# szlhl1040/Vehicles-Dispatch-Simulator

Hardware: AMD Instinct MI355X
Metric: env-steps x replicas / sec (192-cluster, 10k vehicles) (higher is better)
Workload: dtype int32

## Files before the change

include/vds_debug.h:

```cpp
#ifndef VDS_DEBUG_H
#define VDS_DEBUG_H

#include "vds.h"

#ifdef __cplusplus
extern "C" {
#endif

int vds_debug_dense(vds_handle *h, int32_t lanes_per_replica, int32_t tab, int32_t keys, int32_t force_slow);

int vds_debug_ablate(vds_handle *h, int32_t flags);

int vds_debug_read_prof(vds_handle *h, uint64_t *out32);

int vds_debug_read_span(vds_handle *h, uint64_t *out1024, int32_t reset);

int vds_debug_read_err(vds_handle *h, int32_t *out16);

int vds_debug_check_guards(vds_handle *h);

int vds_debug_poke_guard(vds_handle *h);

int vds_debug_graph_pool_size(void);

int vds_debug_tick_forms(vds_handle *h, uint8_t *out, int32_t cap, int32_t *n_out);

int vds_selftest_dpp(vds_handle *h, const int32_t *in, int32_t *out_wave, int32_t *out_rowmin, int32_t *out_rowsum,
                     int32_t *out_rowscan, int32_t nwaves);

#ifdef __cplusplus
}
#endif
#endif
```

vehicles_dispatch_simulator_amd/_lib.py:

```python
from __future__ import annotations

import ctypes as C
import os
import sys
import subprocess

_HERE = os.path.dirname(os.path.abspath(__file__))
def _lib_path():
    name = os.environ.get("VDS_LIB", "libvds.so")
    if os.path.isabs(name):
        return name
    for d in (_HERE, os.path.join(os.path.dirname(_HERE), "build")):
        if os.path.exists(os.path.join(d, name)):
            return os.path.join(d, name)
    return os.path.join(_HERE, name)


LIB_PATH = _lib_path()
CSRC = os.path.join(_HERE, "csrc")

NUM_COUNTERS = 8
COUNTER_NAMES = ("order_num", "reject_num", "matched", "wait_sum", "dispatch_num", "dispatch_cost", "sum_order_value", "evals")


class VdsConfig(C.Structure):
    _fields_ = [
        ("struct_size", C.c_int32), ("device", C.c_int32), ("replicas", C.c_int32), ("vehicles", C.c_int32),
        ("tick_minutes", C.c_int32), ("neighbor_can_server", C.c_int32), ("pickup_reject_threshold", C.c_int64),
        ("idle_cap", C.c_int32), ("ring_cap", C.c_int32), ("ring_ticks", C.c_int32), ("far_cap", C.c_int32),
        ("force_generic", C.c_int32),
    ]


_VP, _I32, _I64 = C.c_void_p, C.c_int32, C.c_int64
SYMBOLS = {
    "vds_version": (_I32, []),
    "vds_build_id": (C.c_char_p, []),
    "vds_config_init": (None, [C.POINTER(VdsConfig)]),
    "vds_create": (C.c_int, [C.POINTER(VdsConfig), C.POINTER(_VP)]),
    "vds_destroy": (C.c_int, [_VP]),
    "vds_last_error": (C.c_char_p, [_VP]),
    "vds_set_stream": (C.c_int, [_VP, _VP]),
    "vds_load_static": (C.c_int, [_VP, _VP, _I32, _VP, _I32, _VP, _VP, _I32]),
    "vds_load_orders": (C.c_int, [_VP, _VP, _VP, _VP, _I32]),
    "vds_load_order_days": (C.c_int, [_VP, _I32, _VP, _VP, _VP, _VP, _VP]),
    "vds_load_orders_strided": (C.c_int, [_VP, _VP, _VP, _VP, _I32, _I64]),
    "vds_replica_ticks": (C.c_int, [_VP, _I32, C.POINTER(_I32), C.POINTER(_I32)]),
    "vds_set_idle_cap": (C.c_int, [_VP, _I32]),
    "vds_idle_cap": (C.c_int, [_VP]),
    "vds_num_ticks": (C.c_int, [_VP, C.POINTER(_I32)]),
    "vds_reset": (C.c_int, [_VP, _VP]),
    "vds_reset_again": (C.c_int, [_VP]),
    "vds_reset_random": (C.c_int, [_VP, _VP]),
    "vds_step": (C.c_int, [_VP]),
    "vds_apply_dispatch": (C.c_int, [_VP, _I32, _VP, _VP, _VP, _VP]),
    "vds_apply_dispatch_ex": (C.c_int, [_VP, _I32, _VP, _VP, _VP, _VP, _VP, _VP]),
    "vds_apply_dispatch_device": (C.c_int, [_VP, _I32, _VP]),
    "vds_advance": (C.c_int, [_VP]),
    "vds_run": (C.c_int, [_VP, _I32]),
    "vds_set_run_groups": (C.c_int, [_VP, _I32, _I32]),
    "vds_get_run_groups": (C.c_int, [_VP]),
    "vds_sync": (C.c_int, [_VP]),
    "vds_clock": (C.c_int, [_VP, C.POINTER(_I32), C.POINTER(_I32)]),
    "vds_read_obs": (C.c_int, [_VP, _VP, _VP, _VP, _VP, _VP]),
    "vds_obs_device": (C.c_int, [_VP, C.POINTER(_VP)]),
    "vds_obs_device_planes": (C.c_int, [_VP, _I32, C.POINTER(_VP)]),
    "vds_obs_inplace": (C.c_int, [_VP, _I32, C.POINTER(_VP), C.POINTER(C.c_int64), C.POINTER(C.c_int64)]),
    "vds_run_hooked_invalidate": (C.c_int, [_VP]),
    "vds_supply_inplace": (C.c_int, [_VP, C.POINTER(_VP), C.POINTER(C.c_int64), C.POINTER(C.c_int64), C.POINTER(C.c_int64), C.POINTER(_VP), C.POINTER(_I32)]),
    "vds_counters_device": (C.c_int, [_VP, C.POINTER(_VP)]),
    "vds_outcomes_device": (C.c_int, [_VP, C.POINTER(_VP)]),
    "vds_read_outcomes": (C.c_int, [_VP, _VP, _VP, _VP, _VP]),
    "vds_read_counters": (C.c_int, [_VP, _VP]),
    "vds_reduce_counters": (C.c_int, [_VP, _VP, C.POINTER(_VP)]),
    "vds_reduce_counters_into": (C.c_int, [_VP, _VP]),
    "vds_profile_enable": (C.c_int, [_VP, _I32]),
    "vds_run_hooked": (C.c_int, [_VP, _I32, _I32, _I32, _VP, _VP]),
    "vds_set_replica_days": (C.c_int, [_VP, _VP]),
    "vds_profile_read": (C.c_int, [_VP, _VP, _I32, C.POINTER(_I32)]),
    "vds_read_orders": (C.c_int, [_VP, _I32, _I32, _VP, _VP, _VP]),
    "vds_read_lists": (C.c_int, [_VP, _I32] + [_VP] * 8),
    "vds_read_vehicles": (C.c_int, [_VP, _I32] + [_VP] * 5),
    "vds_read_work": (C.c_int, [_VP, _VP]),
    "vds_py_random_nodes": (C.c_int, [C.c_uint64, _I32, _I32, _VP, _VP]),
    "vds_cluster_cost_sums": (C.c_int, [_I32, _VP, _I32, _VP, _I32, _VP, _VP]),
    "vds_cluster_cost_sums_error": (C.c_char_p, []),
    "vds_main_kernel": (C.c_char_p, [_VP]),
    "vds_dfs_sequences": (C.c_int, [_VP, _VP, _I32, _I32, _VP, _VP, C.c_int64]),
}
TEST_SYMBOLS = {"vds_debug_read_span": (C.c_int, [_VP, _VP, _I32]), "vds_debug_read_err": (C.c_int, [_VP, _VP]), "vds_debug_graph_pool_size": (C.c_int, []), "vds_debug_tick_forms": (C.c_int, [_VP, _VP, _I32, _VP]), "vds_debug_check_guards": (C.c_int, [_VP]), "vds_debug_poke_guard": (C.c_int, [_VP]), "vds_debug_dense": (C.c_int, [_VP, _I32, _I32, _I32, _I32]), "vds_debug_ablate": (C.c_int, [_VP, _I32]), "vds_debug_read_prof": (C.c_int, [_VP, _VP]), "vds_selftest_dpp": (C.c_int, [_VP, _VP, _VP, _VP, _VP, _VP, _I32])}

_lib = None


def build(force: bool = False) -> str:
    srcs = [os.path.join(CSRC, f) for f in os.listdir(CSRC) if f.endswith((".hip", ".h"))]
    srcs.append(os.path.join(os.path.dirname(_HERE), "include", "vds.h"))
    srcs.append(os.path.join(os.path.dirname(_HERE), "include", "vds_debug.h"))
    stale = (not os.path.exists(LIB_PATH)) or any(os.path.getmtime(s) > os.path.getmtime(LIB_PATH) for s in srcs)
    if force or stale:
        subprocess.check_call(["make", "-s", "-C", CSRC])
    return LIB_PATH


def load():
    global _lib
    if _lib is None:
        if not os.path.exists(LIB_PATH):
            try:
                build(force=True)
            except Exception as e:
                raise RuntimeError("libvds.so is not built (%s) and building it failed (%s): run "
                                   "`make -C vehicles_dispatch_simulator_amd/csrc`; there is no CPU fallback" % (LIB_PATH, e))
        if "torch" not in sys.modules and not os.environ.get("VDS_NO_TORCH_PRELOAD"):
            try:
                import torch
            except ImportError:
                pass
        lib = C.CDLL(LIB_PATH)
        for name, (res, args) in {**SYMBOLS, **TEST_SYMBOLS}.items():
            if os.environ.get("VDS_LIB") and not hasattr(lib, name):
                print("vehicles_dispatch_simulator_amd: %s (VDS_LIB) does not export %s" % (LIB_PATH, name), file=sys.stderr)
                continue
            fn = getattr(lib, name)
            fn.restype = res
            fn.argtypes = args
        _lib = lib
    return _lib
```

vehicles_dispatch_simulator_amd/csrc/vds_api.hip:

```cpp
#include "../../include/vds.h"
#include "../../include/vds_debug.h"
#include "vds_device.h"

#include <algorithm>
#include <unordered_map>
#include <atomic>
#include <chrono>
#include <thread>
#include <cstdarg>
#include <cstdio>
#include <cstdlib>
#include <cstring>
#include <exception>
#include <map>
#include <mutex>
#include <new>
#include <string>
#include <vector>
#include <execinfo.h>
#include <signal.h>
#include <unistd.h>

namespace vds {
void launch_reset(const Static &, const State &, const int *, hipStream_t);
bool reset_uses_image(const Static &);
void launch_reset_capture(const Static &, const State &, unsigned *, int *, hipStream_t);
void launch_reset_image(const Static &, const State &, const unsigned *, const int *, hipStream_t);
void launch_py_random_nodes(const unsigned long long *, int, int, int, int, const int *, int *, int *, hipStream_t);
void launch_start_nodes_check(const int *, int, int, int, int, const int *, int *, unsigned long long *, hipStream_t);
void launch_tick_main(const Static &, const State &, int, int, hipStream_t);
void launch_tick_work(const Static &, const State &, int, hipStream_t);
void launch_update_only(const Static &, const State &, int, hipStream_t);
void launch_match_dfs(const Static &, const State &, int, hipStream_t);
void launch_tick_replica2(const Static &, const State &, int, hipStream_t);
void launch_tick_hybrid(const Static &, const State &, int, int, hipStream_t);
void emit_tick_rows(const Emit &, const Static &, const State &, int, int, int, int);
void emit_hybrid_rows(const Emit &, const Static &, const State &, int, int, int, int);
void emit_hybrid_walk(const Emit &, const Static &, const State &, int, int, int);
void launch_build_vis(const Static &, const int *, unsigned *, unsigned char *, long long, hipStream_t);
size_t dfs_walk_lds(const Static &);
int dfs_walk_pool(const Static &);
void launch_dispatch(const Static &, const State &, int, int, const int *, const int *, const int *, const int *,
                     const int *, const int *, const int *, const int *, hipStream_t);
void launch_dispatch_dense(const Static &, const State &, int, int, const int *, int, hipStream_t);
void launch_pack_obs(const Static &, const State &, int, int, int, int *, hipStream_t);
void launch_reduce_counters(const Static &, const State &, long long *, long long *, hipStream_t);
void launch_selftest_dpp(const int *, int *, int *, int *, int *, int, hipStream_t);
void set_ablate_tick(int, hipStream_t);
void read_prof_tick(unsigned long long *, hipStream_t);
void set_ablate_dfs(int, hipStream_t);
void read_prof_dfs(unsigned long long *, hipStream_t);
void set_ablate_dense(int, hipStream_t);
void read_prof_dense(unsigned long long *, hipStream_t);
void read_span_dense(unsigned long long *, int, hipStream_t);
void emit_tick_dense(const Emit &, const Static &, const State &, int, int, int);
void emit_dense_flush(const Emit &, const Static &, const State &, int, int);
void emit_pack_obs(const Emit &, const Static &, const State &, int, int, int, int *, int, int);
void emit_dispatch_dense(const Emit &, const Static &, const State &, int, int, const int *, int, int, int);
void emit_slot_outcomes(const Emit &, const Static &, const State &, int, int, long long *, int, int);
void launch_slot_outcomes(const Static &, const State &, int, int, long long *, hipStream_t);
}

using namespace vds;

static thread_local std::string g_create_error;

struct DayHost {
    int O = 0;
    int T = 0, now0 = 0, q_base = 0, Oq = 0;
    std::vector<int> so_id;
    std::vector<int> q_value;
    std::vector<int> q_of;
    std::vector<int> o_tick;
    std::vector<long long> value_upto;
    long long value_all = 0;
};

template <typename T>
struct NoInitAlloc {
    using value_type = T;
    NoInitAlloc() = default;
    template <class U> NoInitAlloc(const NoInitAlloc<U> &) {}
    T *allocate(size_t n) { return static_cast<T *>(::operator new(n * sizeof(T))); }
    void deallocate(T *p, size_t) { ::operator delete(p); }
    template <class U, class... A> void construct(U *p, A &&...a) {
        if constexpr (sizeof...(A) == 0) ::new ((void *)p) U; else ::new ((void *)p) U(std::forward<A>(a)...);
    }
    bool operator==(const NoInitAlloc &) const { return true; }
    bool operator!=(const NoInitAlloc &) const { return false; }
};
template <typename T> using hvec = std::vector<T, NoInitAlloc<T>>;

struct PinnedPool {
    std::mutex mu;
    std::vector<std::pair<void *, size_t>> idle;
    std::unordered_map<void *, std::pair<size_t, bool>> live;
    size_t idle_bytes = 0;
    void *get(size_t bytes) {
        bytes = (bytes + 65535) & ~(size_t)65535;
        std::lock_guard<std::mutex> lk(mu);
        int best = -1;
        for (int i = 0; i < (int)idle.size(); ++i)
            if (idle[i].second >= bytes && idle[i].second <= bytes + bytes / 2 + (1u << 20) && (best < 0 || idle[i].second < idle[best].second)) best = i;
        if (best >= 0) {
            void *p = idle[best].first; const size_t b = idle[best].second;
            idle.erase(idle.begin() + best); idle_bytes -= b;
            live[p] = {b, true};
            return p;
        }
        void *p = nullptr;
        if (hipHostMalloc(&p, bytes, hipHostMallocDefault) == hipSuccess && p) { live[p] = {bytes, true}; return p; }
        (void)hipGetLastError();
        p = ::operator new(bytes);
        live[p] = {bytes, false};
        return p;
    }
    void put(void *p) {
        std::lock_guard<std::mutex> lk(mu);
        auto it = live.find(p);
        if (it == live.end()) return;
        const size_t b = it->second.first; const bool pinned = it->second.second;
        live.erase(it);
        if (!pinned) { ::operator delete(p); return; }
        idle.emplace_back(p, b); idle_bytes += b;
        while (idle_bytes > ((size_t)1 << 30) && !idle.empty()) {
            (void)hipHostFree(idle.front().first); idle_bytes -= idle.front().second; idle.erase(idle.begin());
        }
    }
};
static PinnedPool &pinned_pool() { static PinnedPool *pool = new PinnedPool(); return *pool; }
template <typename T>
struct PinnedAlloc {
    using value_type = T;
    PinnedAlloc() = default;
    template <class U> PinnedAlloc(const PinnedAlloc<U> &) {}
    T *allocate(size_t n) { return static_cast<T *>(pinned_pool().get(n * sizeof(T))); }
    void deallocate(T *p, size_t) { pinned_pool().put(p); }
    template <class U, class... A> void construct(U *p, A &&...a) {
        if constexpr (sizeof...(A) == 0) ::new ((void *)p) U; else ::new ((void *)p) U(std::forward<A>(a)...);
    }
    bool operator==(const PinnedAlloc &) const { return true; }
    bool operator!=(const PinnedAlloc &) const { return false; }
};
template <typename T> using pvec = std::vector<T, PinnedAlloc<T>>;


struct vds_handle {
    vds_config cfg{};
    Static S{};
    State D{};
    hipStream_t own_stream = nullptr, stream = nullptr;
    std::string err;
    bool have_static = false, have_orders = false, have_reset = false;
    bool dfs_mode = false;
    bool dfs2_ok = false;
    bool hybrid_ok = false;
    long long blk_ints = 0;
    bool dense_static_ok = false;
    bool dense_dfs_static_ok = false;
    bool want_sup = false;
    bool nodes_valid = false;
    int alloc_dense = -1, alloc_st = -1;
    int seq_tick0 = 0;
    int seq_tick = -1;
    Static *d_S = nullptr;
    State *d_D = nullptr;
    Static S_up{};
    State D_up{};
    bool have_up = false;
    pvec<int2> pull_drec;
    std::vector<int> pull_slot_q;
    std::vector<int4> pull_desc;
    int pull_Od_max = 0;
    std::vector<int> cl_cmax;
    int dbg_dense_lpr = 0, dbg_dense_tab = 0, dbg_dense_keys = 0, dbg_dense_slow = 0;
    int cost_min = 0, cost_max = 0;
    int max_seq = 0;
    std::vector<unsigned char> lbc_host;
    std::vector<int> dfs_off_host, dfs_seq_host;
    int depth_limit = 0;
    int t = 0;
    int last_stepped = -1;
    int dispatch_seq = 0;
    int O = 0;
    int lds_ints = 0;
    std::vector<int> node2cluster, node_local, cl_off, cl_nodes, cost_host, corder_host;
    std::vector<DayHost> days;
    std::vector<int> replica_day;
    int R_ext = 0;
    std::vector<int> int2ext, ext2int;
    int alloc_R = 0;
    std::vector<void *> dev_allocs;
    std::vector<void *> order_allocs;
    std::unordered_map<void *, size_t> order_bytes;
    std::vector<std::pair<void *, size_t>> order_cache;
    std::vector<void *> map_allocs;
    std::vector<void *> result_allocs;
    std::vector<DayDesc> ddesc_host;
    size_t res_cap_out = 0, res_cap_arr = 0, res_cap_slog = 0;
    int alloc_O = 0;
    int Oqmax = 0;
    std::vector<void *> state_allocs;
    std::vector<void *> idle_allocs;
    int idle_cap_grown = 0;
    std::vector<void *> *alloc_sink = nullptr;
    int *d_veh_node = nullptr;
    unsigned long long *d_seeds = nullptr;
    int *d_fullest = nullptr;
    unsigned *d_reset_img = nullptr; int *d_reset_base = nullptr;
    size_t reset_img_words = 0, reset_base_words = 0;
    unsigned veh_gen = 0, img_veh_gen = 0, img_tables_gen = 0; bool img_valid = false;
    int *d_veh_stage = nullptr;
    unsigned long long *d_bad = nullptr;
    int *d_obs = nullptr;
    long long *d_outc = nullptr;
    long long *d_cnt_per = nullptr, *d_cnt_tot = nullptr;
    int *d_actions = nullptr;
    size_t actions_cap = 0;
    int *d_selftest = nullptr;
    bool profiling = false;
    hipGraphExec_t run_exec = nullptr;
    int run_t0 = -1, run_n = 0, run_G = 1;
    int *pin_slow = nullptr;
    hipEvent_t pin_ev = nullptr;
    long long pin_bucket_ticks = 0;
    int *pin_slow_tick = nullptr; int pin_slow_cap = 0;
    bool pin_ticks_valid = false;
    int slow_tick_cap = 1;
    int tick_mode = 1, tick_lim = -1;
    std::vector<unsigned char> tick_form;
    Static S_alt;
    int dense_adapt = 0;
    unsigned tables_gen = 0;
    bool run_stale = false;
    hipStream_t run_stream = nullptr;
    int use_graph = -1;
    std::vector<hipEvent_t> ev_pool;
    size_t ev_used = 0;
    int run_groups = -1;
    int run_stagger = -1;
    hipGraphExec_t hook_exec = nullptr;
    hipGraphExec_t hook_policy_exec = nullptr;
    void *hook_policy_inst = nullptr;
    int hook_t0 = -1, hook_n = 0, hook_G = 1, hook_planes = 0, hook_K = 0;
    unsigned hook_gen = 0;
    const long long *hook_outc = nullptr;
    const void *hook_actions = nullptr;
    void *hook_policy = nullptr;
    hipStream_t hook_stream = nullptr;
};

static int fail(vds_handle *h, int code, const char *fmt, ...) {
    char buf[512];
    va_list ap;
    va_start(ap, fmt);
    vsnprintf(buf, sizeof(buf), fmt, ap);
    va_end(ap);
    if (h) h->err = buf;
    else g_create_error = buf;
    return code;
}

#define HIPCHK(h, call)                                                                          \
    do {                                                                                         \
        hipError_t e_ = (call);                                                                  \
        if (e_ != hipSuccess) return fail(h, VDS_EHIP, "%s failed: %s", #call, hipGetErrorString(e_)); \
    } while (0)

#ifdef VDS_CANARY
static const size_t GUARD_FRONT = 64u << 10, GUARD_BACK = 256u << 10;
static const bool GUARDED = true;
#else
static const size_t GUARD_FRONT = 0, GUARD_BACK = 0;
static const bool GUARDED = false;
#endif
struct GuardRec { void *base; size_t bytes; };
static std::map<void *, GuardRec> g_guards;
static std::mutex g_guards_mu;

static void dev_free(void *p) {
    if (!p) return;
    if (GUARDED) {
        std::lock_guard<std::mutex> lk(g_guards_mu);
        auto it = g_guards.find(p);
        if (it != g_guards.end()) { (void)hipFree(it->second.base); g_guards.erase(it); return; }
    }
    (void)hipFree(p);
}

template <typename T>
static int dev_alloc(vds_handle *h, T **p, size_t n) {
    *p = nullptr;
    if (n == 0) n = 1;
    const size_t bytes = n * sizeof(T);
    if (!GUARDED && h->alloc_sink == &h->order_allocs) {
        int best = -1;
        for (int i = 0; i < (int)h->order_cache.size(); ++i) {
            const size_t cb = h->order_cache[i].second;
            if (cb >= bytes && cb <= bytes + bytes / 2 + 65536 && (best < 0 || cb < h->order_cache[best].second)) best = i;
        }
        if (best >= 0) {
            *p = reinterpret_cast<T *>(h->order_cache[best].first);
            h->order_bytes[(void *)*p] = h->order_cache[best].second;
            h->order_cache.erase(h->order_cache.begin() + best);
            h->order_allocs.push_back((void *)*p);
            return VDS_OK;
        }
    }
    char *base = nullptr;
    hipError_t e = hipMalloc((void **)&base, bytes + GUARD_FRONT + GUARD_BACK);
    if (e != hipSuccess) return fail(h, VDS_ENOMEM, "hipMalloc(%zu bytes) failed: %s", bytes, hipGetErrorString(e));
    if (GUARDED) {
        (void)hipMemset(base, 0xA5, GUARD_FRONT);
        (void)hipMemset(base + GUARD_FRONT + bytes, 0xA5, GUARD_BACK);
        std::lock_guard<std::mutex> lk(g_guards_mu);
        g_guards[(void *)(base + GUARD_FRONT)] = GuardRec{(void *)base, bytes};
    }
    *p = reinterpret_cast<T *>(base + GUARD_FRONT);
    (h->alloc_sink ? *h->alloc_sink : h->dev_allocs).push_back((void *)*p);
    if (!GUARDED && h->alloc_sink == &h->order_allocs) h->order_bytes[(void *)*p] = bytes;
    return VDS_OK;
}

template <typename T, typename A>
static int upload(vds_handle *h, T **p, const std::vector<T, A> &v) {
    int rc = dev_alloc(h, p, v.size());
    if (rc) return rc;
    if (!v.empty()) HIPCHK(h, hipMemcpy(*p, v.data(), v.size() * sizeof(T), hipMemcpyHostToDevice));
    return VDS_OK;
}

template <typename F>
static int guarded(vds_handle *h, const char *name, F &&body) {
    try {
        return body();
    } catch (const std::bad_alloc &) {
        return fail(h, VDS_ENOMEM, "%s: out of host memory", name);
    } catch (const std::exception &e) {
        return fail(h, VDS_EINVAL, "%s: %s", name, e.what());
    } catch (...) {
        return fail(h, VDS_EINVAL, "%s: unknown C++ exception", name);
    }
}

#define RUN_GROUPS_MAX 16

extern "C" int vds_debug_tick_forms(vds_handle *h, uint8_t *out, int32_t cap, int32_t *n_out) {
    if (!h || !out || !n_out || cap < 0) return VDS_EINVAL;
    const int n = (int)std::min<size_t>(h->tick_form.size(), (size_t)cap);
    for (int i = 0; i < n; ++i) out[i] = h->tick_form[i];
    *n_out = n;
    return VDS_OK;
}
extern "C" int vds_debug_graph_pool_size() {
    return 0;
}

static void drop_hook_graph(vds_handle *h) {
    if (h->hook_exec) {
        (void)hipStreamSynchronize(h->hook_stream);
        (void)hipGraphExecDestroy(h->hook_exec);
        h->hook_exec = nullptr;
    }
    if (h->hook_policy_exec) { (void)hipStreamSynchronize(h->stream); (void)hipGraphExecDestroy(h->hook_policy_exec); h->hook_policy_exec = nullptr; h->hook_policy_inst = nullptr; }
    h->hook_t0 = -1; h->hook_n = 0;
}

static void drop_run_graph(vds_handle *h) {
    drop_hook_graph(h);
    if (h->run_exec) {
        (void)hipStreamSynchronize(h->run_stream);
        (void)hipGraphExecDestroy(h->run_exec);
        h->run_exec = nullptr;
    }
    h->run_t0 = -1; h->run_n = 0; h->run_G = 1; h->run_stale = false;
}

#ifndef DENSE_LPR_DEFAULT
#define DENSE_LPR_DEFAULT 8
#endif

static int dev_copy_sync(vds_handle *h) {
    if (!h->S.dense) return VDS_OK;
    if (!h->d_S) {
        HIPCHK(h, hipMalloc((void **)&h->d_S, sizeof(Static)));
        HIPCHK(h, hipMalloc((void **)&h->d_D, sizeof(State)));
    }
    h->S.self_dev = h->d_S; h->S.state_dev = h->d_D;
    Static want = h->S;
    want.r_lo = 0;
    if (h->have_up && memcmp(&want, &h->S_up, sizeof(Static)) == 0 && memcmp(&h->D, &h->D_up, sizeof(State)) == 0) return VDS_OK;
    HIPCHK(h, hipMemcpyAsync(h->d_S, &want, sizeof(Static), hipMemcpyHostToDevice, h->stream));
    HIPCHK(h, hipMemcpyAsync(h->d_D, &h->D, sizeof(State), hipMemcpyHostToDevice, h->stream));
    memcpy(&h->S_up, &want, sizeof(Static));
    memcpy(&h->D_up, &h->D, sizeof(State));
    h->have_up = true;
    return VDS_OK;
}

static int round_up(int x, int m) { return (x + m - 1) / m * m; }

template <typename F>
static void for_each_day(int n_days, F &&fn) {
    int nt = (int)std::thread::hardware_concurrency();
    if (const char *v = getenv("VDS_LOAD_THREADS")) { if (*v) nt = atoi(v); }
    nt = std::max(1, std::min(std::min(nt, 16), n_days));
    if (nt <= 1) { for (int d = 0; d < n_days; ++d) fn(d); return; }
    std::atomic<int> next{0};
    auto work = [&] { for (int d = next.fetch_add(1); d < n_days; d = next.fetch_add(1)) fn(d); };
    std::vector<std::thread> th;
    th.reserve((size_t)nt);
    try { for (int i = 1; i < nt; ++i) th.emplace_back(work); } catch (...) { }
    work();
    for (auto &t : th) t.join();
}
struct LoadTimer {
    bool on; std::chrono::steady_clock::time_point t0;
    LoadTimer() { const char *v = getenv("VDS_LOAD_TIMING"); on = v && *v == '1'; t0 = std::chrono::steady_clock::now(); }
    void lap(const char *what) {
        if (!on) return;
        const auto t1 = std::chrono::steady_clock::now();
        fprintf(stderr, "vds_load_orders: %-34s %8.2f ms\n", what, std::chrono::duration<double, std::milli>(t1 - t0).count());
        t0 = t1;
    }
};

extern "C" {

int32_t vds_version(void) { return (1 << 16) | 0; }

#ifndef VDS_SRC_HASH
#define VDS_SRC_HASH "unknown"
#endif
const char *vds_build_id(void) {
#ifdef VDS_PROF
    return "src:" VDS_SRC_HASH "+prof";
#elif defined(WKDEBUG)
    return "src:" VDS_SRC_HASH "+dbg";
#elif defined(VDS_CANARY)
    return "src:" VDS_SRC_HASH "+canary";
#else
    return "src:" VDS_SRC_HASH;
#endif
}

namespace {
struct Mt19937 {
    uint32_t mt[624];
    int idx;
    void init_genrand(uint32_t s) {
        mt[0] = s;
        for (int i = 1; i < 624; ++i) mt[i] = 1812433253u * (mt[i - 1] ^ (mt[i - 1] >> 30)) + (uint32_t)i;
        idx = 624;
    }
    void init_by_array(const uint32_t *key, int len) {
        init_genrand(19650218u);
        int i = 1, j = 0;
        for (int k = std::max(624, len); k; --k) {
            mt[i] = (mt[i] ^ ((mt[i - 1] ^ (mt[i - 1] >> 30)) * 1664525u)) + key[j] + (uint32_t)j;
            if (++i >= 624) { mt[0] = mt[623]; i = 1; }
            if (++j >= len) j = 0;
        }
        for (int k = 623; k; --k) {
            mt[i] = (mt[i] ^ ((mt[i - 1] ^ (mt[i - 1] >> 30)) * 1566083941u)) - (uint32_t)i;
            if (++i >= 624) { mt[0] = mt[623]; i = 1; }
        }
        mt[0] = 0x80000000u;
    }
    uint32_t next() {
        if (idx >= 624) {
            for (int k = 0; k < 624; ++k) {
                uint32_t y = (mt[k] & 0x80000000u) | (mt[(k + 1) % 624] & 0x7fffffffu);
                mt[k] = mt[(k + 397) % 624] ^ (y >> 1) ^ ((y & 1u) ? 0x9908b0dfu : 0u);
            }
            idx = 0;
        }
        uint32_t y = mt[idx++];
        y ^= y >> 11; y ^= (y << 7) & 0x9d2c5680u; y ^= (y << 15) & 0xefc60000u; y ^= y >> 18;
        return y;
    }
};
}

int vds_py_random_nodes(uint64_t seed, int32_t N, int32_t count, const uint8_t *valid, int32_t *out) {
    if (N < 1 || count < 0 || (count > 0 && !out)) return VDS_EINVAL;
    if (valid) {
        bool any = false;
        for (int i = 0; i < N && !any; ++i) any = valid[i] != 0;
        if (!any) return VDS_ESTATE;
    }
    Mt19937 g;
    uint32_t key[2] = {(uint32_t)(seed & 0xffffffffu), (uint32_t)(seed >> 32)};
    g.init_by_array(key, key[1] ? 2 : 1);
    int k = 0;
    for (uint32_t n = (uint32_t)N; n; n >>= 1) ++k;
    for (int v = 0; v < count; ++v) {
        for (;;) {
            uint32_t r;
            do { r = g.next() >> (32 - k); } while (r >= (uint32_t)N);
            if (!valid || valid[r]) { out[v] = (int32_t)r; break; }
        }
    }
    return VDS_OK;
}
// ... 182 lines not shown
        std::vector<int> seq;
        for (int c = 0; c < C; ++c) {
            seq.clear();
            if (nbr_off[c + 1] > nbr_off[c]) {
                std::fill(seen.begin(), seen.end(), 0);
                dfs_visit(c, depth_limit, nbr_off, nbr_idx, seen, seq);
            }
            for (size_t i = 1; i < seq.size(); ++i) dfs_seq.push_back(seq[i]);
            dfs_off[c + 1] = (int)dfs_seq.size();
            if (seq.size() > 1) any_seq = true;
        }
    }
    h->dfs_mode = any_seq;
    int rc;
    h->cost_host.assign(cost, cost + (size_t)N * N);
    int *d;
    long long *dl;
    std::vector<int> costp_host;
    {
        std::vector<int> &costp = costp_host;
        costp.assign((size_t)N * N, 0);
        const int ncol = h->cl_off[C];
        for (int i = 0; i < N; ++i) {
            const int *src = cost + (size_t)i * N;
            int *dst = costp.data() + (size_t)i * N;
            for (int j = 0; j < ncol; ++j) dst[j] = src[h->cl_nodes[j]];
        }
        if ((rc = upload(h, &d, costp))) return rc; S.cost = d;
    }
    if ((rc = upload(h, &d, h->node2cluster))) return rc; S.node2cluster = d;
    if ((rc = upload(h, &d, h->node_local))) return rc; S.node_local = d;
    if ((rc = upload(h, &d, h->cl_off))) return rc; S.cl_off = d;
    if ((rc = upload(h, &d, h->cl_nodes))) return rc; S.cl_nodes = d;
    if ((rc = upload(h, &dl, blk_off))) return rc; S.blk_off = dl;
    if ((rc = upload(h, &d, blk))) return rc; S.blk = d;
    {
        std::vector<int> corder(C);
        for (int c = 0; c < C; ++c) corder[c] = c;
        std::stable_sort(corder.begin(), corder.end(), [&](int a, int b) { return cdesc[a].x > cdesc[b].x; });
        if ((rc = upload(h, &d, corder))) return rc; S.corder = d;
        h->corder_host = corder;
        std::vector<int4> cdo(C);
        std::vector<long long> b8off(C + 1, 0);
        for (int c = 0; c < C; ++c) { long long nc = cdesc[c].x; b8off[c + 1] = b8off[c] + (nc * nc + 15) / 16 * 16; }
        bool u8 = b8off[C] < (1ll << 31);
        for (size_t i = 0; i < blk.size() && u8; ++i) u8 = blk[i] >= 0 && blk[i] <= 255;
        S.u8_ok = u8 ? 1 : 0;
        std::vector<unsigned char> blk8(u8 ? (size_t)b8off[C] : 1, 0);
        if (u8)
            for (int c = 0; c < C; ++c) {
                const long long nc = cdesc[c].x;
                for (long long e = 0; e < nc * nc; ++e) blk8[(size_t)b8off[c] + e] = (unsigned char)blk[(size_t)cdesc[c].y + e];
            }
        { unsigned char *d8; if ((rc = upload(h, &d8, blk8))) return rc; S.blk8 = d8; }
        for (int i = 0; i < C; ++i) cdo[i] = make_int4(cdesc[corder[i]].x, cdesc[corder[i]].y, corder[i], u8 ? (int)b8off[corder[i]] : 0);
        for (int c = 0; c < C; ++c) cdesc[c].z = u8 ? (int)b8off[c] : 0;
        { int4 *d4c; if ((rc = upload(h, &d4c, cdesc))) return rc; S.cdesc = d4c; }
        S.cost8 = nullptr;
        if (u8) {
            std::vector<unsigned char> c8((size_t)N * N + 16, 0);
            bool fits = true;
            for (size_t i = 0; i < (size_t)N * N && fits; ++i) { fits = costp_host[i] >= 0 && costp_host[i] <= 255; c8[i] = (unsigned char)costp_host[i]; }
            if (fits) { unsigned char *d8; if ((rc = upload(h, &d8, c8))) return rc; S.cost8 = d8; }
            else S.u8_ok = 0;
            S.lbc = nullptr;
            h->lbc_host.clear();
            if (fits && any_seq && (long long)N * C <= (256ll << 20)) {
                std::vector<unsigned char> lb((size_t)N * C, 255);
                for (int pn = 0; pn < N; ++pn) {
                    const unsigned char *row = c8.data() + (size_t)pn * N;
                    for (int c = 0; c < C; ++c) {
                        unsigned char m = 255;
                        for (int col = h->cl_off[c]; col < h->cl_off[c + 1]; ++col) m = std::min(m, row[col]);
                        lb[(size_t)pn * C + c] = m;
                    }
                }
                unsigned char *dlb; if ((rc = upload(h, &dlb, lb))) return rc; S.lbc = dlb;
                h->lbc_host.swap(lb);
            }
        }
        { int4 *d4o; if ((rc = upload(h, &d4o, cdo))) return rc; S.cdesc_ord = d4o; }
        S.blk8s = nullptr; S.blk32s = nullptr; S.cdesc_dense = nullptr;
        bool d_ok = max_nc <= 255;
        bool d8 = d_ok && S.u8_ok;
        for (size_t i = 0; i < blk.size() && d8; ++i) d8 = blk[i] <= 254;
        if (d_ok) {
            std::vector<long long> doff(C, 0);
            long long tot = 0;
            const long long esz = d8 ? 1 : 4;
            for (int c = 0; c < C; ++c) { const long long nc = cdesc[c].x; doff[c] = tot; tot += (nc * (nc + 1) * esz + 15) / 16 * 16; }
            d_ok = tot < (1ll << 31);
            if (d_ok) {
                std::vector<unsigned char> bs((size_t)std::max<long long>(tot, 16), 0);
                for (int c = 0; c < C; ++c) {
                    const long long nc = cdesc[c].x;
                    for (long long pp = 0; pp < nc; ++pp) {
                        for (long long l = 0; l <= nc; ++l) {
                            const int v = l < nc ? blk[(size_t)cdesc[c].y + pp * nc + l] : (d8 ? 0xFF : DENSE_DEAD_COST);
                            if (d8) bs[(size_t)(doff[c] + pp * (nc + 1) + l)] = (unsigned char)v;
                            else memcpy(bs.data() + (size_t)(doff[c] + (pp * (nc + 1) + l) * 4), &v, 4);
                        }
                    }
                }
                unsigned char *db; if ((rc = upload(h, &db, bs))) return rc;
                if (d8) S.blk8s = db; else S.blk32s = reinterpret_cast<const int *>(db);
                std::vector<int4> cdd(C);
                for (int i = 0; i < C; ++i) cdd[i] = make_int4(cdesc[corder[i]].x, (int)doff[corder[i]], corder[i], dfs_off[corder[i] + 1] > dfs_off[corder[i]] ? 1 : 0);
                int4 *d4d; if ((rc = upload(h, &d4d, cdd))) return rc; S.cdesc_dense = d4d;
            }
        }
        h->dense_static_ok = d_ok;
        h->cl_cmax.assign(C, 0);
        for (int c = 0; c < C; ++c) {
            const long long nc = cdesc[c].x;
            int mx = 0;
            for (long long e = 0; e < nc * nc; ++e) mx = std::max(mx, blk[(size_t)cdesc[c].y + e]);
            h->cl_cmax[c] = mx;
        }
    }
    h->max_seq = 0;
    for (int c = 0; c < C; ++c) h->max_seq = std::max(h->max_seq, dfs_off[c + 1] - dfs_off[c]);
    S.seq_pad = h->max_seq <= 64 ? 64 : h->max_seq <= 128 ? 128 : 256;
    h->dfs_off_host = dfs_off; h->dfs_seq_host = dfs_seq;
    if ((rc = upload(h, &d, dfs_off))) return rc; S.dfs_off = d;
    if ((rc = upload(h, &d, dfs_seq))) return rc; S.dfs_seq = d;
    {
        const int bmw = (C + 31) / 32;
        std::vector<unsigned> vb((size_t)C * bmw, 0u);
        for (int c = 0; c < C; ++c)
            for (int j = dfs_off[c]; j < dfs_off[c + 1]; ++j) vb[(size_t)c * bmw + (dfs_seq[j] >> 5)] |= 1u << (dfs_seq[j] & 31);
        unsigned *dv; if ((rc = upload(h, &dv, vb))) return rc; S.vis_bits = dv;
    }
    {
        int cmin = 0x7FFFFFFF, cmax = -0x7FFFFFFF - 1;
        for (size_t i = 0; i < (size_t)N * N; ++i) { cmin = std::min(cmin, cost[i]); cmax = std::max(cmax, cost[i]); }
        S.fast_ok = (cmin >= 0 && cmax < (1 << 23) && (long long)cmax <= S.reject_threshold) ? 1 : 0;
        S.window_live = ((long long)cmax > S.reject_threshold) ? 1 : 0;
        if (h->cfg.force_generic == 1) S.fast_ok = 0;
        h->cost_min = cmin; h->cost_max = cmax;
    }
    const int lds_budget_ints = (64 * 1024) / 4;
    h->lds_ints = std::min((max_nc * max_nc + 3) / 4 * 4, lds_budget_ints);
    {
        const long long esz = S.blk8s ? 1 : 4;
        const bool common = h->dense_static_ok && S.fast_ok && S.V < (1 << 24) && (long long)max_nc * (max_nc + 1) * esz <= 64 * 1024 && h->cfg.force_generic == 0;
        h->dense_static_ok = common && !h->dfs_mode;
        h->dense_dfs_static_ok = common && h->dfs_mode && S.blk8s != nullptr && S.u8_ok && S.cost8 != nullptr && S.V <= 16384 && h->max_seq <= 256 &&
                                 !(getenv("VDS_DENSE_DFS") && getenv("VDS_DENSE_DFS")[0] == '0');
    }
    h->have_static = true;
    return VDS_OK;
}

static int alloc_state(vds_handle *h, int O) {
    Static &S = h->S;
    State &D = h->D;
    const int V = S.V, R = S.R, C = S.C;
    const int per = (V + C - 1) / C;
    int idle_cap = h->cfg.idle_cap > 0 ? h->cfg.idle_cap : std::min(round_up(std::max(V, 1), 64), round_up(4 * per + 64, 64));
    if (h->idle_cap_grown > idle_cap) idle_cap = h->idle_cap_grown;
    idle_cap = round_up(idle_cap, 64);
    if (idle_cap > (1 << 24)) return fail(h, VDS_EINVAL, "idle_cap=%d > 2^24 slots per (replica, cluster) unsupported", idle_cap);
    int H = h->cfg.ring_ticks > 0 ? h->cfg.ring_ticks : 32;
    if (H < 2 || (H & (H - 1))) return fail(h, VDS_EINVAL, "ring_ticks=%d must be a power of two >= 2", H);
    const long long per_tick = ((long long)O + (long long)std::max(S.T, 1) * C - 1) / ((long long)std::max(S.T, 1) * C);
    int ring_cap = h->cfg.ring_cap > 0 ? h->cfg.ring_cap : (int)std::min<long long>(round_up(std::max(V, 16), 16), round_up((int)std::min<long long>(10 * per_tick + 32, 60000), 16));
    ring_cap = round_up(ring_cap, 16);
    if (ring_cap > 65520) return fail(h, VDS_EINVAL, "ring_cap=%d > 65520 unsupported", ring_cap);
    int far_cap = h->cfg.far_cap > 0 ? round_up(h->cfg.far_cap, 64) : std::min(round_up(std::max(V, 1), 64), 256);
    if (S.dense && H > 32) { S.dense = 0; S.pull = 0; }
    if (!h->state_allocs.empty() && S.idle_cap >= idle_cap && S.fl_cap == far_cap && S.H == H && S.ring_cap >= ring_cap && h->alloc_dense == S.dense && h->alloc_st == S.dense_st && h->alloc_R == R)
        return VDS_OK;
    for (void *p : h->state_allocs) dev_free(p);
    h->state_allocs.clear();
    h->d_outc = nullptr;
    S.idle_cap = idle_cap; S.fl_cap = far_cap; S.in_cap = far_cap; S.H = H; S.ring_cap = ring_cap;
    const size_t B = (size_t)C * R;
    h->alloc_dense = S.dense; h->alloc_st = S.dense_st;
    h->alloc_R = R;
    h->nodes_valid = false;
    int rc;
    struct Sink { vds_handle *h; std::vector<void *> *old; ~Sink() { h->alloc_sink = old; } } sink{h, h->alloc_sink};
    h->alloc_sink = &h->state_allocs;
    if ((rc = dev_alloc(h, &D.hdr, B * HDR_WORDS))) return rc;
    if ((rc = dev_alloc(h, &D.cnt, B * CNT_WORDS))) return rc;
    {
        std::vector<void *> *keep = h->alloc_sink;
        h->alloc_sink = &h->idle_allocs;
        for (void *p : h->idle_allocs) dev_free(p);
        h->idle_allocs.clear();
        rc = dev_alloc(h, &D.idle, S.dense ? (B * idle_cap + 1) / 2 : B * idle_cap);
        D.stamp = nullptr;
        if (!rc && S.dense_st) rc = dev_alloc(h, &D.stamp, B * idle_cap);
        h->alloc_sink = keep;
        if (rc) return rc;
    }
    D.slow_tick = nullptr;
    {
        int tcap = std::max(S.T, 1);
        for (const auto &d : h->days) tcap = std::max(tcap, d.T);
        h->slow_tick_cap = tcap;
        if (S.dense && (rc = dev_alloc(h, &D.slow_tick, (size_t)tcap))) return rc;
    }
    D.dry = nullptr;
    if (S.dense_st && (rc = dev_alloc(h, &D.dry, (size_t)R))) return rc;
    D.sup = nullptr; D.sup_slot = nullptr;
    if (getenv("VDS_SUPPLY_INPLACE") && getenv("VDS_SUPPLY_INPLACE")[0] == '1') h->want_sup = true;
    if (S.dense && h->want_sup && ((rc = dev_alloc(h, &D.sup, (size_t)VDS_SUP_PLANES * B)) || (rc = dev_alloc(h, &D.sup_slot, (size_t)1)))) return rc;
    if ((rc = dev_alloc(h, &D.ring, S.dense ? ((size_t)H * B * ring_cap + 1) / 2 : (size_t)H * B * ring_cap))) return rc;
    D.ring_min = nullptr;
    if (S.dense && (rc = dev_alloc(h, &D.ring_min, (size_t)H * B * ring_cap))) return rc;
    S.ring_min_on = D.ring_min != nullptr;
    if ((rc = dev_alloc(h, &D.ring_cnt, (size_t)H * B))) return rc;
    if ((rc = dev_alloc(h, &D.fl, B * far_cap))) return rc;
    if ((rc = dev_alloc(h, &D.inbox, 2 * B * far_cap))) return rc;
    if ((rc = dev_alloc(h, &D.err, 16))) return rc;
    if ((rc = dev_alloc(h, &D.work, 2 + 2 * B))) return rc;
    if ((rc = dev_alloc(h, &h->d_veh_node, (size_t)R * V))) return rc;
    if ((rc = dev_alloc(h, &h->d_obs, 5 * (size_t)R * C))) return rc;
    if ((rc = dev_alloc(h, &h->d_cnt_per, (size_t)R * CNT_WORDS))) return rc;
    if ((rc = dev_alloc(h, &h->d_cnt_tot, CNT_WORDS))) return rc;
    HIPCHK(h, hipMemset(D.err, 0, 16 * sizeof(int)));
    HIPCHK(h, hipMemset(D.work, 0, 2 * sizeof(int)));
    return VDS_OK;
}

static int alloc_state(vds_handle *h, int O);

static int apply_replica_map(vds_handle *h) {
    Static &S = h->S;
    const int RX = h->R_ext, n_days = S.n_days;
    const std::vector<DayDesc> &ddesc = h->ddesc_host;
    int Tmax = 0;
    for (int r = 0; r < RX; ++r) Tmax = std::max(Tmax, h->days[h->replica_day[r]].T);
    S.T = Tmax;
    S.R = RX; h->int2ext.clear(); h->ext2int.clear();
    const bool gran8_ok = S.dense && S.dense_lpr == 16 && h->cfg.force_generic == 0 && !(getenv("VDS_ROW_GRAN8") && getenv("VDS_ROW_GRAN8")[0] == '0');
    S.row_gran = 16;
    S.chunk_days = n_days > 1 ? 1 : 0;
    for (int r = 0; r < RX && S.chunk_days; ++r)
        if (h->replica_day[r] != h->replica_day[r & ~15]) S.chunk_days = 0;
    for (int gr = 8; gr >= 4 && n_days > 1 && !S.chunk_days && gran8_ok; gr >>= 1) {
        bool okg = true;
        for (int r = 0; r < RX && okg; ++r) okg = h->replica_day[r] == h->replica_day[r & ~(gr - 1)];
        if (okg) { S.chunk_days = 1; S.row_gran = gr; }
    }
    std::vector<int> rperm;
    std::vector<int> day_of_internal;
    if (n_days > 1 && !S.chunk_days && h->cfg.force_generic == 0) {
        std::vector<std::vector<int>> by_day(n_days);
        for (int r = 0; r < RX; ++r) by_day[h->replica_day[r]].push_back(r);
        std::vector<int> i2e;
        int gran = 16;
        for (int pass = 0; pass < 3; ++pass, gran >>= 1) {
            i2e.clear(); day_of_internal.clear();
            for (int dd = 0; dd < n_days; ++dd) {
                for (int r : by_day[dd]) { i2e.push_back(r); day_of_internal.push_back(dd); }
                while (i2e.size() % gran) { i2e.push_back(-1); day_of_internal.push_back(n_days); }
            }
            if (i2e.size() * 4 <= (size_t)RX * 5 || !gran8_ok) break;
        }
        while (i2e.size() % 16) { i2e.push_back(-1); day_of_internal.push_back(n_days); }
        if (i2e.size() * 4 <= (size_t)RX * 5) {
            S.row_gran = gran >= 16 ? 16 : (gran >= 8 ? 8 : 4);
            if (h->alloc_R > (int)i2e.size() && (size_t)h->alloc_R * 4 <= (size_t)RX * 5 && !h->state_allocs.empty())
                while ((int)i2e.size() < h->alloc_R) { i2e.push_back(-1); day_of_internal.push_back(n_days); }
            S.chunk_days = 1;
            S.R = (int)i2e.size();
            h->int2ext = i2e;
            h->ext2int.assign(RX, -1);
            for (int i = 0; i < S.R; ++i) if (i2e[i] >= 0) h->ext2int[i2e[i]] = i;
            rperm.resize(S.R);
            for (int i = 0; i < S.R; ++i) rperm[i] = i2e[i] >= 0 ? i : -1;
        } else {
            day_of_internal.clear();
        }
    }
    if (day_of_internal.empty()) day_of_internal = h->replica_day;
    for (void *p : h->map_allocs) dev_free(p);
    h->map_allocs.clear();
    struct Sink { vds_handle *h; std::vector<void *> *old; ~Sink() { h->alloc_sink = old; } } sink{h, h->alloc_sink};
    h->alloc_sink = &h->map_allocs;
    int rc;
    int *d;
    S.rperm = nullptr; S.rslots = 0; S.int2ext = nullptr;
    if (!rperm.empty()) { if ((rc = upload(h, &d, rperm))) return rc; S.rperm = d; S.rslots = (int)rperm.size(); }
    if ((rc = upload(h, &d, day_of_internal))) return rc; S.replica_day = d;
    if (!h->int2ext.empty()) { if ((rc = upload(h, &d, h->int2ext))) return rc; S.int2ext = d; }
    {
        std::vector<int4> rdesc(S.R);
        for (int r = 0; r < S.R; ++r) { const DayDesc &dd = ddesc[day_of_internal[r]]; rdesc[r] = make_int4(dd.bkt_base, dd.now0, dd.T, dd.q_base); }
        int4 *dr; if ((rc = upload(h, &dr, rdesc))) return rc; S.replica_desc = dr;
    }
    S.replica_desc2 = nullptr;
    if (S.pull) {
        std::vector<int4> rd2(S.R);
        for (int r = 0; r < S.R; ++r) rd2[r] = day_of_internal[r] < n_days ? h->pull_desc[day_of_internal[r]] : make_int4(0, 0, 0, 0);
        int4 *d4r; if ((rc = upload(h, &d4r, rd2))) return rc; S.replica_desc2 = d4r;
    }
    return VDS_OK;
}

static int alloc_results(vds_handle *h) {
    Static &S = h->S;
    S.arr_slots = std::max(h->pull_Od_max, 1);
    const size_t need_out = (size_t)S.R * std::max(h->Oqmax, 1);
    const size_t need_arr = S.pull ? (size_t)S.R * S.arr_slots : 0;
    const size_t need_slog = h->hybrid_ok ? (size_t)S.R * std::max(S.max_tick_orders, 1) : 0;
    auto fits = [](size_t need, size_t cap) { return need <= cap && (need == 0 ? cap == 0 : cap <= 4 * need + (1u << 20)); };
    if (h->D.out != nullptr && fits(need_out, h->res_cap_out) && fits(need_arr, h->res_cap_arr) && fits(need_slog, h->res_cap_slog)) return VDS_OK;
    for (void *p : h->result_allocs) dev_free(p);
    h->result_allocs.clear();
    h->D.out = nullptr; h->D.arr = nullptr; h->D.slog = nullptr;
    h->res_cap_out = h->res_cap_arr = h->res_cap_slog = 0;
    struct Sink { vds_handle *h; std::vector<void *> *old; ~Sink() { h->alloc_sink = old; } } sink{h, h->alloc_sink};
    h->alloc_sink = &h->result_allocs;
    int rc = dev_alloc(h, &h->D.out, need_out);
    if (!rc && need_arr) rc = dev_alloc(h, &h->D.arr, need_arr);
    if (!rc && need_slog) rc = dev_alloc(h, &h->D.slog, need_slog);
    if (!rc) { h->res_cap_out = need_out; h->res_cap_arr = need_arr; h->res_cap_slog = need_slog; }
    return rc;
}

static int set_replica_days_impl(vds_handle *h, const int32_t *replica_day) {
    if (!h || !h->have_orders) return fail(h, VDS_EINVAL, "vds_set_replica_days: load order days first");
    if (!replica_day) return fail(h, VDS_EINVAL, "vds_set_replica_days: null map");
    const int n_days = h->S.n_days;
    for (int r = 0; r < h->R_ext; ++r)
        if (replica_day[r] < 0 || replica_day[r] >= n_days) return fail(h, VDS_EINVAL, "vds_set_replica_days: replica %d is mapped to day %d of %d", r, replica_day[r], n_days);
    HIPCHK(h, hipSetDevice(h->cfg.device));
    HIPCHK(h, hipStreamSynchronize(h->stream));
    h->replica_day.assign(replica_day, replica_day + h->R_ext);
    const int R_before = h->S.R;
    int rc = apply_replica_map(h);
    if (rc) return rc;
    if (h->S.R != R_before) {
        if ((rc = alloc_state(h, h->alloc_O))) return rc;
        if ((rc = alloc_results(h))) return rc;
        if (h->d_veh_stage) {  }
    }
    { h->run_stale = true; h->tables_gen++; }
    h->have_reset = false;
    h->t = 0; h->last_stepped = -1; h->dispatch_seq = 0; h->seq_tick = -1;
    return VDS_OK;
}

static int load_days_body(vds_handle *h, int32_t n_days, const int64_t *day_off, const int32_t *release_min, const int32_t *pickup,
                          const int32_t *delivery, const int32_t *replica_day) {
    LoadTimer lt;
    if (!h || !h->have_static) return fail(h, VDS_EINVAL, "vds_load_orders: call vds_load_static first");
    if (n_days < 1 || !day_off || !release_min || !pickup || !delivery) return fail(h, VDS_EINVAL, "vds_load_orders: bad argument");
    for (int d = 0; d < n_days; ++d)
        if (day_off[d + 1] - day_off[d] < 1 || day_off[d + 1] - day_off[d] > 0x7fffffff) return fail(h, VDS_EINVAL, "vds_load_orders: day %d has no orders (or more than 2^31)", d);
    HIPCHK(h, hipSetDevice(h->cfg.device));
    if (h->have_orders) {
// ... 46 lines not shown
                const std::vector<int> &costh = h->cost_host;
                for (int i = 0; i < O; ++i) {
                    if (pk[i] < 0 || pk[i] >= N || dl[i] < 0 || dl[i] >= N) { day_fail(l, VDS_EINVAL, "vds_load_orders: order %lld has a node outside [0,%lld)", i, N); return; }
                    l.value[i] = costh[(size_t)dl[i] * N + pk[i]];
                }
                H.o_tick.assign(O, -1);
                l.cnt.assign((size_t)T * C + 1, 0);
                long long run = 0;
                int n_proc = 0;
                H.value_all = 0;
                for (int i = 0; i < O; ++i) {
                    H.value_all += l.value[i];
                    long long x = (long long)rel[i] - now0;
                    long long ti = x < 0 ? 0 : x / tick;
                    run = std::max(run, ti);
                    if (i == O - 1 || run >= T) continue;
                    int pc = h->node2cluster[pk[i]], dc = h->node2cluster[dl[i]];
                    if (pc < 0 || dc < 0) { day_fail(l, VDS_ESTATE, "vds_load_orders: order %lld touches a node outside every cluster (KeyError in the reference, :918/:960)", i, 0); return; }
                    H.o_tick[i] = (int)run;
                    l.cnt[(size_t)run * C + pc + 1]++;
                    n_proc++;
                }
                for (size_t i = 1; i < l.cnt.size(); ++i) l.cnt[i] += l.cnt[i - 1];
                l.n_proc = n_proc;
            } catch (...) { l.code = VDS_ENOMEM; l.msg = "vds_load_orders: out of host memory"; }
        });
        std::vector<size_t> rec0(n_days + 1, 0), bk0(n_days + 1, 0), tk0(n_days + 1, 0);
        for (int d = 0; d < n_days; ++d) {
            if (L[d].code) return fail(h, L[d].code, "%s", L[d].msg.c_str());
            rec0[d + 1] = rec0[d] + (size_t)L[d].n_proc;
            bk0[d + 1] = bk0[d] + L[d].cnt.size();
            tk0[d + 1] = tk0[d] + (size_t)L[d].T + 1;
            if (rec0[d + 1] >= (1ull << 31)) return fail(h, VDS_EINVAL, "vds_load_orders: more than 2^31 processed orders on one handle");
            if (bk0[d + 1] >= (1ull << 31)) return fail(h, VDS_EINVAL, "vds_load_orders: bucket table exceeds 2^31 entries");
        }
        so_rec.resize(rec0[n_days]); so_pnode.resize(rec0[n_days]); ord_q.resize(rec0[n_days]);
        bkt_off.resize(bk0[n_days]); tick_off.resize(tk0[n_days]);
        for_each_day(n_days, [&](int d) {
            DayLocal &l = L[d];
            try {
                DayHost &H = h->days[d];
                const int32_t *pk = pickup + day_off[d], *dl = delivery + day_off[d];
                const int O = l.O, T = l.T, n_proc = l.n_proc;
                const size_t r0 = rec0[d];
                H.q_base = (int)r0; H.Oq = n_proc;
                H.so_id.assign(n_proc, 0);
                H.q_value.assign(n_proc, 0);
                H.value_upto.assign(T + 1, 0);
                l.toff.assign(T + 1, 0);
                std::vector<int> fill(l.cnt.begin(), l.cnt.end() - 1);
                int k = 0;
                for (int i = 0; i < O; ++i) {
                    int ti = H.o_tick[i];
                    if (ti < 0) continue;
                    int pc = h->node2cluster[pk[i]], dc = h->node2cluster[dl[i]];
                    int q = fill[(size_t)ti * C + pc]++;
                    so_rec[r0 + q] = make_int4(i, h->node_local[pk[i]] | (h->node_local[dl[i]] << 16), dc | (pc << 16), l.value[i]);
                    H.so_id[q] = i;
                    H.q_value[q] = l.value[i];
                    so_pnode[r0 + q] = pk[i];
                    ord_q[r0 + k++] = (int)r0 + q;
                    l.toff[ti + 1]++;
                    H.value_upto[ti + 1] += l.value[i];
                }
                for (int t = 0; t < T; ++t) { l.toff[t + 1] += l.toff[t]; H.value_upto[t + 1] += H.value_upto[t]; }
                int day_mto = 0;
                for (int t = 0; t < T; ++t) day_mto = std::max(day_mto, l.toff[t + 1] - l.toff[t]);
                l.day_mto = day_mto;
                ddesc[d].bkt_base = (int)bk0[d];
                ddesc[d].tick_base = (int)tk0[d];
                ddesc[d].now0 = H.now0; ddesc[d].T = T; ddesc[d].q_base = H.q_base; ddesc[d].Oq = n_proc;
                ddesc[d].max_tick_orders = day_mto; ddesc[d].pad = 0;
                for (size_t i = 0; i < l.cnt.size(); ++i) bkt_off[bk0[d] + i] = l.cnt[i] + (int)r0;
                for (int t = 0; t <= T; ++t) tick_off[tk0[d] + t] = l.toff[t] + (int)r0;
                std::vector<int>().swap(l.value); std::vector<int>().swap(l.cnt);
            } catch (...) { l.code = VDS_ENOMEM; l.msg = "vds_load_orders: out of host memory"; }
        });
        for (int d = 0; d < n_days; ++d) {
            if (L[d].code) return fail(h, L[d].code, "%s", L[d].msg.c_str());
            Tmax = std::max(Tmax, L[d].T); Oqmax = std::max(Oqmax, L[d].n_proc); Omax = std::max(Omax, L[d].O); mto = std::max(mto, L[d].day_mto);
            Ototal += L[d].O;
        }
    }
    lt.lap("cursor, buckets, sorted records");
    S.now0 = h->days[0].now0; S.Oq = Oqmax; h->O = Omax; h->Oqmax = Oqmax;
    S.n_days = n_days;
    (void)Tmax;
    {
        DayDesc e{}; e.bkt_base = 0; e.tick_base = 0; e.now0 = h->days[0].now0; e.T = 0; e.q_base = 0; e.Oq = 0; e.max_tick_orders = 0; e.pad = 0;
        ddesc.push_back(e);
    }
    h->ddesc_host = ddesc;
    S.max_tick_orders = mto;
    int rc;
    int *d;
    int4 *d4;
    struct Sink { vds_handle *h; ~Sink() { h->alloc_sink = nullptr; } } sink{h};
    h->alloc_sink = &h->order_allocs;
    if ((rc = upload(h, &d4, so_rec))) return rc; S.so_rec = d4;
    if ((rc = upload(h, &d, bkt_off))) return rc; S.bkt_off = d;
    if ((rc = upload(h, &d, tick_off))) return rc; S.tick_off = d;
    if ((rc = upload(h, &d, so_pnode))) return rc; S.so_pnode = d;
    if ((rc = upload(h, &d, ord_q))) return rc; S.ord_q = d;
    {
        std::vector<int> so_rank(so_rec.size(), 0);
        for_each_day(n_days, [&](int dd) {
            const DayDesc &de = ddesc[dd];
            for (int t = 0; t < de.T; ++t) {
                const int a = tick_off[de.tick_base + t], b = tick_off[de.tick_base + t + 1];
                for (int i = a; i < b; ++i) so_rank[ord_q[i]] = i - a;
            }
        });
        if ((rc = upload(h, &d, so_rank))) return rc; S.so_rank = d;
    }
    lt.lap("upload records, ranks");
    S.so_lb = nullptr; S.so_vis = nullptr;
    if (h->dfs_mode && h->cfg.force_generic == 0 && h->max_seq <= 256 && mto < 65535 && (long long)so_rec.size() * S.seq_pad * 5 <= (6ll << 30)) {
        std::vector<int> so_bkt0(so_rec.size(), 0);
        for_each_day(n_days, [&](int dd) {
            const DayDesc &de = ddesc[dd];
            for (int t = 0; t < de.T; ++t) {
                const int b0 = de.bkt_base + t * C;
                for (int q = bkt_off[b0]; q < bkt_off[b0 + C]; ++q) so_bkt0[q] = b0;
            }
        });
        int *d_b0;
        if ((rc = upload(h, &d_b0, so_bkt0))) return rc;
        unsigned *dv;
        if ((rc = dev_alloc(h, &dv, so_rec.size() * (size_t)S.seq_pad))) return rc;
        unsigned char *dl = nullptr;
        if (!h->lbc_host.empty() && (rc = dev_alloc(h, &dl, so_rec.size() * (size_t)S.seq_pad))) return rc;
        launch_build_vis(S, d_b0, dv, dl, (long long)so_rec.size(), h->stream);
        HIPCHK(h, hipGetLastError());
        S.so_vis = dv; S.so_lb = dl;
    }
    lt.lap("visit rows + bounds per order");
    { DayDesc *dd; if ((rc = upload(h, &dd, ddesc))) return rc; S.day = dd; }
    const int ring_H = h->cfg.ring_ticks > 0 ? h->cfg.ring_ticks : 32;
    S.dense = (h->dense_static_ok && Omax < (1 << DENSE_ID_BITS) && ring_H <= 32) ? 1 : 0;
    S.dense_st = 0;
    if (h->dense_dfs_static_ok && n_days == 1 && Omax < (1 << DENSE_ID_BITS) && ring_H <= 32 && mto < 65535 && S.so_vis != nullptr &&
        S.max_nc * S.max_nc <= h->lds_ints && S.N <= 65534 && h->cost_max < (1 << 15) && h->cfg.idle_cap <= 16384) {
        Static Z = S;
        Z.dense_st = 1; Z.walk_pool = 0;
        if (dfs_walk_lds(Z) + 1024 <= 64 * 1024) { S.dense = 1; S.dense_st = 1; }
    }
    {
        auto env_int = [](const char *name, int dflt) { const char *v = getenv(name); return v && *v ? atoi(v) : dflt; };
        if (env_int("VDS_DENSE", 1) == 0) S.dense = 0;
        const int lpr = h->dbg_dense_lpr > 0 ? h->dbg_dense_lpr : env_int("VDS_DENSE_LPR", n_days > 1 ? 16 : DENSE_LPR_DEFAULT);
        S.dense_lpr = (lpr == 8 || lpr == 16) ? lpr : DENSE_LPR_DEFAULT;
        const int tab_max = (S.dense_lpr == 16 && S.blk8s != nullptr && env_int("VDS_DENSE_TAB256", 1) != 0) ? 256 : 128;
        h->dense_adapt = (h->dbg_dense_lpr > 0 || h->dbg_dense_tab > 0 || getenv("VDS_DENSE_LPR") || env_int("VDS_DENSE_ADAPT", 1) == 0) ? -1 : 0;
        h->pin_bucket_ticks = 0; h->pin_ticks_valid = false; h->tick_form.clear();
        { const char *v = getenv("VDS_DENSE_TICK_FORMS"); h->tick_mode = !v || !*v ? 1 : (*v == '0' ? 0 : (*v == 'a' ? 2 : 1)); h->tick_lim = env_int("VDS_DENSE_TICK_LIM", -1); }
        S.dense_tab = h->dbg_dense_tab > 0 ? std::min(h->dbg_dense_tab, tab_max) : tab_max;
        S.dense_keys = h->dbg_dense_keys > 0 ? std::min(h->dbg_dense_keys, 64) : 64;
        S.dense_force_slow = h->dbg_dense_slow & 1;
        S.pull = (S.dense && S.V < (1 << 24) - 1 && !(h->dbg_dense_slow & 2) && env_int("VDS_DENSE_PULL", 1) != 0) ? 1 : 0;
        if (S.dense_st && !S.pull) { S.dense = 0; S.dense_st = 0; }
    }
    S.so_slot = nullptr; S.d_rec = nullptr; S.d_first = nullptr; S.replica_desc2 = nullptr; S.pull_W = 0; S.pull_hmax = 0;
    int Od_max = 0;
    std::vector<int> d_first_keep;
    if (S.pull) {
        const int Hc = h->cfg.ring_ticks > 0 ? h->cfg.ring_ticks : 32;
        const int tk = S.tick_minutes;
        auto slots_of = [&](long long rel) -> int { return rel <= 0 ? 1 : (int)((rel + tk - 1) / tk); };
        pvec<int> so_slot(so_rec.size(), -1);
        pvec<int2> d_rec;
        std::vector<int> d_first;
        std::vector<int4> ddesc2(ddesc.size(), make_int4(0, 0, 0, 0));
        int W = 0, hmax = 0;
        bool ok = true;
        struct PullDay { std::vector<int> start; int npull = 0, W = 0, hmax = 0, TA = 0, code = 0; };
        std::vector<PullDay> PD(n_days);
        auto for_pull = [&](const DayDesc &de, auto &&fn) {
            for (int t = 0; t < de.T; ++t)
                for (int ix = tick_off[de.tick_base + t]; ix < tick_off[de.tick_base + t + 1]; ++ix) {
                    const int q = ord_q[ix];
                    const int4 &rr = so_rec[q];
                    const int c = (int)((unsigned)rr.z >> 16);
                    const int dmin = slots_of(rr.w), dmax = slots_of((long long)rr.w + h->cl_cmax[c]);
                    if (dmax >= Hc) continue;
                    fn(q, rr, t, dmin, dmax);
                }
        };
        for (int dd = 0; dd < n_days; ++dd) { PD[dd].TA = ddesc[dd].T + Hc; if (PD[dd].TA >= 65535) ok = false; }
        if (ok) for_each_day(n_days, [&](int dd) {
            PullDay &P = PD[dd];
            try {
                const int TA = P.TA;
                P.start.assign((size_t)C * (TA + 1) + 1, 0);
                for_pull(ddesc[dd], [&](int, const int4 &rr, int t, int dmin, int dmax) {
                    P.W = std::max(P.W, dmax - dmin);
                    P.hmax = std::max(P.hmax, dmin);
                    P.start[(size_t)(rr.z & 0xFFFF) * (TA + 1) + (t + dmin) + 1]++;
                    ++P.npull;
                });
                for (size_t kx = 0; kx + 1 < P.start.size(); ++kx) P.start[kx + 1] += P.start[kx];
            } catch (...) { P.code = VDS_ENOMEM; }
        });
        std::vector<size_t> rbase(n_days + 1, 0), fbase(n_days + 1, 0);
        for (int dd = 0; dd < n_days && ok; ++dd) {
            if (PD[dd].code) return fail(h, VDS_ENOMEM, "vds_load_orders: out of host memory");
            rbase[dd + 1] = rbase[dd] + (size_t)PD[dd].npull;
            fbase[dd + 1] = fbase[dd] + (size_t)(PD[dd].TA + 1) * C;
            W = std::max(W, PD[dd].W); hmax = std::max(hmax, PD[dd].hmax); Od_max = std::max(Od_max, PD[dd].npull);
            ddesc2[dd] = make_int4((int)fbase[dd], (int)rbase[dd], PD[dd].TA, PD[dd].npull);
        }
        if (fbase[n_days] >= (1ull << 31) || rbase[n_days] >= (1ull << 31)) ok = false;
        if (ok) {
            d_rec.resize(rbase[n_days]);
            d_first.resize(fbase[n_days]);
            for_each_day(n_days, [&](int dd) {
                PullDay &P = PD[dd];
                const int TA = P.TA, base = (int)rbase[dd];
                int *first = d_first.data() + fbase[dd];
                for (int c = 0; c < C; ++c)
                    for (int a = 0; a <= TA; ++a) first[(size_t)a * C + c] = base + P.start[(size_t)c * (TA + 1) + a];
                for_pull(ddesc[dd], [&](int q, const int4 &rr, int t, int dmin, int) {
                    const int a0 = t + dmin;
                    const int i = P.start[(size_t)(rr.z & 0xFFFF) * (TA + 1) + a0]++;
                    d_rec[(size_t)base + i] = make_int2((int)dense_key(t, 0, rr.x), a0 | ((int)((unsigned)rr.y >> 16) << 16) | (dmin << 24));
                    so_slot[q] = i;
                });
            });
        }
        if ((long long)d_first.size() >= (1ll << 31) || W > DENSE_PULL_WMAX) ok = false;
        if (ok && S.dense_st)
            for (int dd = 0; dd < n_days; ++dd) ok = ok && PD[dd].npull == ddesc[dd].Oq;
        if (!ok && S.dense_st) { S.dense = 0; S.dense_st = 0; }
        if (!ok) S.pull = 0;
        else {
            struct Sink2 { vds_handle *h; ~Sink2() { h->alloc_sink = nullptr; } } sink2{h};
            h->alloc_sink = &h->order_allocs;
            S.pull_W = W; S.pull_hmax = hmax;
            if ((rc = upload(h, &d, so_slot))) return rc; S.so_slot = d;
            int2 *d2; if ((rc = upload(h, &d2, d_rec))) return rc; S.d_rec = d2;
            if ((rc = upload(h, &d, d_first))) return rc; S.d_first = d;
            h->pull_desc = ddesc2;
            d_first_keep = d_first;
            h->pull_drec = std::move(d_rec);
            h->pull_slot_q.assign(h->pull_drec.size(), 0);
            for_each_day(n_days, [&](int dd) {
                const int qb = ddesc[dd].q_base;
                for (int q = qb; q < qb + ddesc[dd].Oq; ++q)
                    if (so_slot[q] >= 0) h->pull_slot_q[(size_t)ddesc2[dd].y + so_slot[q]] = q - qb;
            });
        }
    }
    h->pull_Od_max = Od_max;
    lt.lap("static arrival slots");
    S.tdesc = nullptr;
    if (S.dense && n_days == 1 && (int)h->corder_host.size() == C) {
        const DayDesc &de = ddesc[0];
        std::vector<int4> td((size_t)std::max(de.T, 1) * C * 2, make_int4(0, 0, 0, 0));
        std::vector<int4> cdd((size_t)C);
        HIPCHK(h, hipMemcpy(cdd.data(), S.cdesc_dense, (size_t)C * sizeof(int4), hipMemcpyDeviceToHost));
        for (int t = 0; t < de.T; ++t)
            for (int ci = 0; ci < C; ++ci) {
                const int c = h->corder_host[ci];
                const int q0 = bkt_off[de.bkt_base + (size_t)t * C + c], k = bkt_off[de.bkt_base + (size_t)t * C + c + 1] - q0;
                int clo = 0, n = 0;
                if (S.pull) {
                    clo = d_first_keep[(size_t)std::max(t - S.pull_W, 0) * C + c];
                    n = d_first_keep[(size_t)(t + 1) * C + c] - clo;
                }
                td[2 * ((size_t)t * C + ci)] = make_int4(q0, k, clo, n);
                td[2 * ((size_t)t * C + ci) + 1] = cdd[ci];
            }
        struct Sink3 { vds_handle *h; ~Sink3() { h->alloc_sink = nullptr; } } sink3{h};
        h->alloc_sink = &h->order_allocs;
        int4 *dtd; if ((rc = upload(h, &dtd, td))) return rc; S.tdesc = dtd;
    }
    h->alloc_sink = nullptr;
    lt.lap("bucket descriptors");
    if ((rc = apply_replica_map(h))) return rc;
    h->alloc_sink = nullptr;
    h->alloc_O = (int)std::min<long long>(Ototal / n_days, 0x7fffffff);
    if ((rc = alloc_state(h, h->alloc_O))) return rc;
    lt.lap("state tables");
    {
        const Static &Z = h->S;
        const int ids2 = std::max(Z.max_tick_orders, 4 * Z.C);
        const size_t lds2 = ((size_t)9 * Z.C + 1 + ids2 + ((size_t)Z.V + 2) / 2) * sizeof(int) + 2048;
        h->dfs2_ok = h->dfs_mode && Omax <= (1 << 20) && Z.max_nc <= 2047 && h->cost_min >= 0 && h->cost_max < (1 << 15) &&
                     Z.V <= 20480 && Z.N <= 65534 && Z.C <= 3072 && h->blk_ints < (1ll << 29) && Z.idle_cap <= 32767 && Z.max_tick_orders < 32768 &&
                     lds2 <= 64 * 1024;
        h->S.walk_pool = 0; h->S.walk_pool = dfs_walk_pool(h->S);
        h->hybrid_ok = h->dfs_mode && h->cfg.force_generic == 0 && Z.fast_ok && Z.max_nc * Z.max_nc <= h->lds_ints &&
                       Z.max_tick_orders < 65535 && Z.V < 65536 && Z.max_nc <= 2047 &&
                       Z.N <= 65534 && Z.C <= 65535 && Z.idle_cap <= 16384 && h->cost_max < (1 << 15) && h->max_seq <= 256 &&
                       dfs_walk_lds(Z) + 1024 <= 64 * 1024 && Z.so_vis != nullptr;
        if (Z.dense_st && !h->hybrid_ok)
            return fail(h, VDS_ECAPACITY, "vds_load_orders: neighbour search on the dense layout needs the walk's tables (idle_cap %d <= 16384, %zu bytes of LDS <= 64 KB); VDS_DENSE_DFS=0 keeps the wide layout",
                        Z.idle_cap, dfs_walk_lds(Z) + 1024);
    }
    if ((rc = alloc_results(h))) return rc;
    lt.lap("results, arrival slots, steal log");
    h->have_orders = true;
    return VDS_OK;
}

static void drop_order_cache(vds_handle *h) {
    for (auto &b : h->order_cache) dev_free(b.first);
    h->order_cache.clear();
}

static int load_days_impl(vds_handle *h, int32_t n_days, const int64_t *day_off, const int32_t *release_min, const int32_t *pickup,
                          const int32_t *delivery, const int32_t *replica_day) {
    const int rc = load_days_body(h, n_days, day_off, release_min, pickup, delivery, replica_day);
    drop_order_cache(h);
    return rc;
}

static int load_orders_impl(vds_handle *h, const int32_t *release_min, const int32_t *pickup, const int32_t *delivery, int32_t O) {
    if (O < 1) return fail(h, VDS_EINVAL, "vds_load_orders: bad argument");
    const int64_t off[2] = {0, O};
    return load_days_impl(h, 1, off, release_min, pickup, delivery, nullptr);
}

static int load_orders_strided_impl(vds_handle *h, const int32_t *release_min, const int32_t *pickup, const int32_t *delivery, int32_t O,
                                    int64_t replica_stride) {
    if (!h) return VDS_EINVAL;
    if (replica_stride == 0) return load_orders_impl(h, release_min, pickup, delivery, O);
    if (O < 1 || replica_stride < O) return fail(h, VDS_EINVAL, "vds_load_orders_strided: replica_stride must be 0 (shared day) or >= O");
    const int R = h->cfg.replicas;
    if (replica_stride == O) {
        std::vector<int64_t> off(R + 1);
        for (int r = 0; r <= R; ++r) off[r] = (int64_t)r * O;
        return load_days_impl(h, R, off.data(), release_min, pickup, delivery, nullptr);
    }
    std::vector<int32_t> a((size_t)R * O), b((size_t)R * O), c((size_t)R * O);
    std::vector<int64_t> off(R + 1);
    for (int r = 0; r < R; ++r) {
        memcpy(a.data() + (size_t)r * O, release_min + (size_t)r * replica_stride, (size_t)O * 4);
        memcpy(b.data() + (size_t)r * O, pickup + (size_t)r * replica_stride, (size_t)O * 4);
        memcpy(c.data() + (size_t)r * O, delivery + (size_t)r * replica_stride, (size_t)O * 4);
        off[r] = (int64_t)r * O;
    }
    off[R] = (int64_t)R * O;
    return load_days_impl(h, R, off.data(), a.data(), b.data(), c.data(), nullptr);
}

int vds_num_ticks(const vds_handle *h, int32_t *T) {
    if (!h || !T || !h->have_orders) return VDS_EINVAL;
    *T = h->S.T;
    return VDS_OK;
}

#ifndef DENSE_ADAPT_RATE
#define DENSE_ADAPT_RATE 0.001
#endif
#ifndef DENSE_TICK_RATE
#define DENSE_TICK_RATE 0.00025
#endif
static const Static &tick_static(vds_handle *h, int t) {
    if (t < 0 || (size_t)t >= h->tick_form.size() || !h->tick_form[t]) return h->S;
    h->S_alt = h->S;
    h->S_alt.dense_lpr = 16; h->S_alt.dense_tab = 256;
    return h->S_alt;
}
static void adapt_dense(vds_handle *h) {
    Static &S = h->S;
    if (!S.dense || (h->dfs_mode && !S.dense_st) || S.n_days > 1 || !S.blk8s) return;
    if (h->tick_mode == 2) {
        if (S.dense_lpr == 8 && h->tick_form.empty()) {
            h->tick_form.assign((size_t)std::max(S.T, 1), 0);
            for (size_t t = 1; t < h->tick_form.size(); t += 2) h->tick_form[t] = 1;
            h->run_stale = true; h->tables_gen++;
        }
        return;
    }
    if (h->dense_adapt != 0) return;
    if (!h->pin_slow) {
        if (hipHostMalloc((void **)&h->pin_slow, sizeof(int)) != hipSuccess || hipEventCreateWithFlags(&h->pin_ev, hipEventDisableTiming) != hipSuccess) {
            (void)hipGetLastError(); h->dense_adapt = -1; return;
        }
        *h->pin_slow = 0;
    }
    if (h->pin_bucket_ticks > 0 && hipEventQuery(h->pin_ev) == hipSuccess) {
        if (h->tick_mode == 1 && h->pin_ticks_valid && S.dense_lpr == 8) {
            const double lim = h->tick_lim >= 0 ? (double)h->tick_lim : DENSE_TICK_RATE * (double)S.R * (double)S.C;
            size_t n16 = 0;
            h->tick_form.assign((size_t)S.T, 0);
            for (int t = 0; t < S.T; ++t) if ((double)h->pin_slow_tick[t] > lim) { h->tick_form[t] = 1; ++n16; }
            h->dense_adapt = 1;
            if (n16 * 100 >= (size_t)S.T * 85) { std::fill(h->tick_form.begin(), h->tick_form.end(), (unsigned char)1); n16 = (size_t)S.T; }
            if (n16 > 0) { h->run_stale = true; h->tables_gen++; }
            else h->tick_form.clear();
            return;
        }
        if ((double)*h->pin_slow > DENSE_ADAPT_RATE * (double)h->pin_bucket_ticks) {
            const char *t256 = getenv("VDS_DENSE_TAB256");
            S.dense_lpr = 16; S.dense_tab = (t256 && *t256 == '0') ? 128 : 256;
            h->dense_adapt = 1;
            { h->run_stale = true; h->tables_gen++; }
            return;
        }
    }
    (void)hipGetLastError();
    if (h->have_reset && h->t > 0) {
        h->pin_ticks_valid = false;
        bool ok = hipMemcpyAsync(h->pin_slow, h->D.err + 2, sizeof(int), hipMemcpyDeviceToHost, h->stream) == hipSuccess;
        if (ok && h->tick_mode == 1 && h->D.slow_tick && h->t == S.T && S.T > 0) {
            if (h->pin_slow_cap < S.T) {
                if (h->pin_slow_tick) { (void)hipStreamSynchronize(h->stream); (void)hipHostFree(h->pin_slow_tick); h->pin_slow_tick = nullptr; h->pin_slow_cap = 0; }
                if (hipHostMalloc((void **)&h->pin_slow_tick, (size_t)S.T * sizeof(int)) == hipSuccess) h->pin_slow_cap = S.T;
                else { (void)hipGetLastError(); h->pin_slow_tick = nullptr; }
            }
            if (h->pin_slow_tick && hipMemcpyAsync(h->pin_slow_tick, h->D.slow_tick, (size_t)S.T * sizeof(int), hipMemcpyDeviceToHost, h->stream) == hipSuccess)
                h->pin_ticks_valid = true;
        }
        if (ok && hipEventRecord(h->pin_ev, h->stream) == hipSuccess)
            h->pin_bucket_ticks = (long long)h->t * S.R * S.C;
        else { (void)hipGetLastError(); h->pin_bucket_ticks = 0; h->pin_ticks_valid = false; }
    }
}

static int reset_device(vds_handle *h) {
    adapt_dense(h);
    const Static &S = h->S;
    HIPCHK(h, hipMemsetAsync(h->D.err, 0, 16 * sizeof(int), h->stream));
    HIPCHK(h, hipMemsetAsync(h->D.work, 0, 2 * sizeof(int), h->stream));
    if (h->D.slow_tick) HIPCHK(h, hipMemsetAsync(h->D.slow_tick, 0, (size_t)h->slow_tick_cap * sizeof(int), h->stream));
    HIPCHK(h, hipMemsetAsync(h->D.ring_cnt, 0, (size_t)S.H * S.C * S.R * sizeof(int), h->stream));
    if (h->D.sup) {
        HIPCHK(h, hipMemsetAsync(h->D.sup, 0, (size_t)VDS_SUP_PLANES * S.C * S.R * sizeof(int), h->stream));
        HIPCHK(h, hipMemsetAsync(h->D.sup_slot, 0, sizeof(int), h->stream));
    }
    if (S.dense_st) {
        HIPCHK(h, hipMemsetAsync(h->D.stamp, 0xFF, (size_t)S.C * S.R * S.idle_cap * sizeof(unsigned short), h->stream));
        HIPCHK(h, hipMemsetAsync(h->D.dry, 0, (size_t)S.R * sizeof(int), h->stream));
    }
    if (reset_uses_image(S)) {
        const size_t iw = (size_t)S.R * S.V, bw = (size_t)S.R * (S.C + 1);
        if (h->reset_img_words < iw || h->reset_base_words < bw) {
            HIPCHK(h, hipStreamSynchronize(h->stream));
            for (void *old : {(void *)h->d_reset_img, (void *)h->d_reset_base})
                if (old) { h->dev_allocs.erase(std::remove(h->dev_allocs.begin(), h->dev_allocs.end(), old), h->dev_allocs.end()); dev_free(old); }
            h->d_reset_img = nullptr; h->d_reset_base = nullptr;
            h->reset_img_words = h->reset_base_words = 0; h->img_valid = false;
            std::vector<void *> *sink = h->alloc_sink; h->alloc_sink = nullptr;
            int rc = dev_alloc(h, &h->d_reset_img, iw);
            if (!rc) rc = dev_alloc(h, &h->d_reset_base, bw);
            h->alloc_sink = sink;
            if (rc) return rc;
            h->reset_img_words = iw; h->reset_base_words = bw;
        }
        if (h->img_valid && h->img_veh_gen == h->veh_gen && h->img_tables_gen == h->tables_gen) {
            launch_reset_image(S, h->D, h->d_reset_img, h->d_reset_base, h->stream);
        } else {
            launch_reset(S, h->D, h->d_veh_node, h->stream);
            launch_reset_capture(S, h->D, h->d_reset_img, h->d_reset_base, h->stream);
            h->img_valid = true; h->img_veh_gen = h->veh_gen; h->img_tables_gen = h->tables_gen;
        }
    } else {
        launch_reset(S, h->D, h->d_veh_node, h->stream);
    }
    HIPCHK(h, hipGetLastError());
    h->t = 0; h->last_stepped = -1; h->dispatch_seq = 0; h->seq_tick = -1;
    h->have_reset = true; h->nodes_valid = true;
    return VDS_OK;
}

static int set_idle_cap_impl(vds_handle *h, int32_t cap) {
    if (!h || !h->have_orders) return fail(h, VDS_EINVAL, "vds_set_idle_cap: load static tables and orders first");
    if (cap < 1) return fail(h, VDS_EINVAL, "vds_set_idle_cap: bad capacity %d", cap);
    HIPCHK(h, hipSetDevice(h->cfg.device));
    HIPCHK(h, hipStreamSynchronize(h->stream));
    { h->run_stale = true; h->tables_gen++; }
    cap = std::min(round_up(cap, 64), round_up(std::max(h->S.V, 1), 64));
    if (cap > (1 << 24)) return fail(h, VDS_EINVAL, "vds_set_idle_cap: %d > 2^24 unsupported", cap);
    if (cap == h->S.idle_cap) return VDS_OK;
    if (h->S.dense_st && cap > 16384) return fail(h, VDS_ECAPACITY, "vds_set_idle_cap: neighbour search on the dense layout holds at most 16384 entries per list (VDS_DENSE_DFS=0 keeps the wide layout)");
    for (void *p : h->idle_allocs) dev_free(p);
    h->idle_allocs.clear();
    h->alloc_sink = &h->idle_allocs;
    const size_t B0 = (size_t)h->S.C * h->S.R;
    int rc = dev_alloc(h, &h->D.idle, h->S.dense ? (B0 * cap + 1) / 2 : B0 * cap);
    h->D.stamp = nullptr;
    if (!rc && h->S.dense_st) rc = dev_alloc(h, &h->D.stamp, B0 * cap);
    h->alloc_sink = nullptr;
    if (rc) return rc;
    h->S.idle_cap = cap;
    h->idle_cap_grown = cap;
    if (cap > 32767) h->dfs2_ok = false;
    if (cap > 16384) h->hybrid_ok = false;
    return VDS_OK;
}

static int ensure_reset_scratch(vds_handle *h) {
    int rc;
    if (!h->d_veh_stage && (rc = dev_alloc(h, &h->d_veh_stage, std::max<size_t>((size_t)h->R_ext * h->S.V, 1)))) return rc;
    if (!h->d_fullest && (rc = dev_alloc(h, &h->d_fullest, (size_t)h->R_ext))) return rc;
    if (!h->d_bad && (rc = dev_alloc(h, &h->d_bad, (size_t)1))) return rc;
    return VDS_OK;
}

static int reset_impl(vds_handle *h, const int32_t *veh_init_node) {
    if (!h || !h->have_orders) return fail(h, VDS_EINVAL, "vds_reset: load static tables and orders first");
    if (!veh_init_node && h->S.V > 0) return fail(h, VDS_EINVAL, "vds_reset: null veh_init_node");
    HIPCHK(h, hipSetDevice(h->cfg.device));
    const Static &S = h->S;
    const size_t n = (size_t)h->R_ext * S.V;
    const bool on_device = S.V > 0 && (size_t)S.C * sizeof(int) <= 60 * 1024 && !(getenv("VDS_RESET_HOST_CHECKS") && getenv("VDS_RESET_HOST_CHECKS")[0] == '1');
    if (on_device) {
        int rc0;
        if ((rc0 = ensure_reset_scratch(h))) return rc0;
        HIPCHK(h, hipMemcpyAsync(h->d_veh_stage, veh_init_node, n * sizeof(int), hipMemcpyHostToDevice, h->stream));
        HIPCHK(h, hipMemsetAsync(h->d_bad, 0xFF, sizeof(unsigned long long), h->stream));
        launch_start_nodes_check(h->d_veh_stage, h->R_ext, S.N, S.V, S.C, S.node2cluster, h->d_fullest, h->d_bad, h->stream);
        HIPCHK(h, hipGetLastError());
        std::vector<int> full((size_t)h->R_ext);
        unsigned long long bad = 0;
        HIPCHK(h, hipMemcpyAsync(full.data(), h->d_fullest, (size_t)h->R_ext * sizeof(int), hipMemcpyDeviceToHost, h->stream));
        HIPCHK(h, hipMemcpyAsync(&bad, h->d_bad, sizeof(bad), hipMemcpyDeviceToHost, h->stream));
        HIPCHK(h, hipStreamSynchronize(h->stream));
        if (bad != ~0ull)
            return fail(h, VDS_ESTATE, "vds_reset: vehicle %zu starts on node %d which is in no cluster (:254)", (size_t)bad, veh_init_node[bad]);
        if (h->cfg.idle_cap <= 0) {
            int fullest = 0;
            for (int r = 0; r < h->R_ext; ++r) fullest = std::max(fullest, full[r]);
            const int want = std::min(round_up(std::max(S.V, 1), 64), round_up(2 * fullest + 64, 64));
            if (want > S.idle_cap && (rc0 = set_idle_cap_impl(h, want))) return rc0;
        }
        HIPCHK(h, hipMemcpyAsync(h->d_veh_node, h->d_veh_stage, n * sizeof(int), hipMemcpyDeviceToDevice, h->stream));
        h->veh_gen++;
        if ((rc0 = reset_device(h))) return rc0;
        return vds_sync(h);
    }
    for (size_t i = 0; i < n; ++i) {
        int node = veh_init_node[i];
        if (node < 0 || node >= S.N || h->node2cluster[node] < 0)
            return fail(h, VDS_ESTATE, "vds_reset: vehicle %zu starts on node %d which is in no cluster (:254)", i, node);
    }
    if (h->cfg.idle_cap <= 0 && S.V > 0) {
        std::vector<int> cnt((size_t)S.C);
        int fullest = 0;
        for (int r = 0; r < h->R_ext; ++r) {
            std::fill(cnt.begin(), cnt.end(), 0);
            const int32_t *vn = veh_init_node + (size_t)r * S.V;
            for (int v = 0; v < S.V; ++v) fullest = std::max(fullest, ++cnt[h->node2cluster[vn[v]]]);
        }
        const int want = std::min(round_up(std::max(S.V, 1), 64), round_up(2 * fullest + 64, 64));
        if (want > S.idle_cap) {
            int rc2 = set_idle_cap_impl(h, want);
            if (rc2) return rc2;
        }
    }
    HIPCHK(h, hipMemcpyAsync(h->d_veh_node, veh_init_node, n * sizeof(int), hipMemcpyHostToDevice, h->stream));
    h->veh_gen++;
    int rc = reset_device(h);
    if (rc) return rc;
    return vds_sync(h);
}

static int reset_random_impl(vds_handle *h, const uint64_t *seeds) {
    if (!h || !h->have_orders) return fail(h, VDS_EINVAL, "vds_reset_random: load static tables and orders first");
    if (!seeds) return fail(h, VDS_EINVAL, "vds_reset_random: null seeds");
    HIPCHK(h, hipSetDevice(h->cfg.device));
    const Static &S = h->S;
    bool any = false;
    for (int i = 0; i < S.N && !any; ++i) any = h->node2cluster[i] >= 0;
    if (!any && S.V > 0) return fail(h, VDS_ESTATE, "vds_reset_random: no node lies in a cluster (:254)");
    if ((size_t)(624 + S.C) * sizeof(int) > 64 * 1024) return fail(h, VDS_EINVAL, "vds_reset_random: %d clusters exceed the generator's LDS histogram", S.C);
    if (S.N < 1) return fail(h, VDS_EINVAL, "vds_reset_random: no nodes");
    int rc;
    if (!h->d_seeds && (rc = dev_alloc(h, &h->d_seeds, (size_t)h->R_ext))) return rc;
    if ((rc = ensure_reset_scratch(h))) return rc;
    HIPCHK(h, hipMemcpyAsync(h->d_seeds, seeds, (size_t)h->R_ext * sizeof(uint64_t), hipMemcpyHostToDevice, h->stream));
    launch_py_random_nodes(h->d_seeds, h->R_ext, S.N, S.V, S.C, S.node2cluster, h->d_veh_stage, h->d_fullest, h->stream);
    HIPCHK(h, hipGetLastError());
    std::vector<int> full((size_t)std::max(h->R_ext, 1));
    HIPCHK(h, hipMemcpyAsync(full.data(), h->d_fullest, (size_t)h->R_ext * sizeof(int), hipMemcpyDeviceToHost, h->stream));
    HIPCHK(h, hipStreamSynchronize(h->stream));
    int fullest = 0;
    for (int r = 0; r < h->R_ext; ++r) {
        if (full[r] < 0) return fail(h, VDS_ESTATE, "vds_reset_random: replica %d found no start nodes", r);
        fullest = std::max(fullest, full[r]);
    }
    if (h->cfg.idle_cap <= 0 && S.V > 0) {
        const int want = std::min(round_up(std::max(S.V, 1), 64), round_up(2 * fullest + 64, 64));
        if (want > S.idle_cap && (rc = set_idle_cap_impl(h, want))) return rc;
    }
    HIPCHK(h, hipMemcpyAsync(h->d_veh_node, h->d_veh_stage, (size_t)h->R_ext * S.V * sizeof(int), hipMemcpyDeviceToDevice, h->stream));
    h->veh_gen++;
    if ((rc = reset_device(h))) return rc;
    return vds_sync(h);
}

int vds_reset_again(vds_handle *h) {
    if (!h || !(h->have_reset || (h->have_orders && h->nodes_valid)))
        return fail(h, VDS_EINVAL, "vds_reset_again: needs a previous vds_reset (after a load or a map that re-allocated the state tables: vds_reset / vds_reset_random)");
    HIPCHK(h, hipSetDevice(h->cfg.device));
    return reset_device(h);
}

static int profile_enable_impl(vds_handle *h, int32_t on) {
    if (!h) return VDS_EINVAL;
    h->profiling = on != 0;
    h->ev_used = 0;
    return VDS_OK;
}

static hipEvent_t next_event(vds_handle *h) {
    if (h->ev_used == h->ev_pool.size()) {
        hipEvent_t e;
        if (hipEventCreate(&e) != hipSuccess) return nullptr;
        h->ev_pool.push_back(e);
    }
    return h->ev_pool[h->ev_used++];
}

static int profile_read_impl(vds_handle *h, float *ms, int32_t cap, int32_t *n) {
    if (!h || !ms || !n) return VDS_EINVAL;
    HIPCHK(h, hipSetDevice(h->cfg.device));
    HIPCHK(h, hipStreamSynchronize(h->stream));
    int k = 0;
    for (size_t i = 0; i + 1 < h->ev_used && k < cap; i += 2, ++k) HIPCHK(h, hipEventElapsedTime(&ms[k], h->ev_pool[i], h->ev_pool[i + 1]));
    *n = k;
    h->ev_used = 0;
    return VDS_OK;
}

static int step_impl(vds_handle *h, bool flush = true) {
    if (!h || !h->have_reset) return fail(h, VDS_EINVAL, "vds_step: call vds_reset first");
    if (h->last_stepped == h->t) return fail(h, VDS_EINVAL, "vds_step: tick %d already stepped; call vds_advance", h->t);
    HIPCHK(h, hipSetDevice(h->cfg.device));
    if (h->t >= h->S.T) return fail(h, VDS_EINVAL, "vds_step: tick %d is past the end of the day (%d ticks, :1048)", h->t, h->S.T);
    if (!h->dfs_mode) {
        hipEvent_t a = nullptr, b = nullptr;
        if (h->profiling) {
            a = next_event(h); b = next_event(h);
            if (!a || !b) return fail(h, VDS_EHIP, "vds_step: hipEventCreate failed");
            HIPCHK(h, hipEventRecord(a, h->stream));
        }
        if (h->S.dense) {
            const int rcs = dev_copy_sync(h);
            if (rcs) return rcs;
            Emit e; e.st = h->stream; emit_tick_dense(e, tick_static(h, h->t), h->D, h->t, 0, 0);
        }
        else launch_tick_main(h->S, h->D, h->t, h->lds_ints, h->stream);
        if (h->profiling) HIPCHK(h, hipEventRecord(b, h->stream));
        if (!h->S.dense && (!h->S.fast_ok || h->S.max_nc * h->S.max_nc > h->lds_ints)) launch_tick_work(h->S, h->D, h->t, h->stream);
    } else if (h->hybrid_ok && h->cfg.force_generic == 0) {
        hipEvent_t a = nullptr, b = nullptr;
        if (h->profiling) {
            a = next_event(h); b = next_event(h);
            if (!a || !b) return fail(h, VDS_EHIP, "vds_step: hipEventCreate failed");
            HIPCHK(h, hipEventRecord(a, h->stream));
        }
        if (h->S.dense_st) {
            const int rcs = dev_copy_sync(h);
            if (rcs) return rcs;
            Emit e; e.st = h->stream;
            emit_tick_dense(e, tick_static(h, h->t), h->D, h->t, 0, 0);
            emit_hybrid_walk(e, h->S, h->D, h->t, 0, 0);
            if (flush) emit_dense_flush(e, h->S, h->D, 0, 0);
        }
        else launch_tick_hybrid(h->S, h->D, h->t, h->lds_ints, h->stream);
        if (h->profiling) HIPCHK(h, hipEventRecord(b, h->stream));
    } else if (h->dfs2_ok && h->cfg.force_generic != 1) {
        hipEvent_t a = nullptr, b = nullptr;
        if (h->profiling) {
            a = next_event(h); b = next_event(h);
            if (!a || !b) return fail(h, VDS_EHIP, "vds_step: hipEventCreate failed");
            HIPCHK(h, hipEventRecord(a, h->stream));
        }
        launch_tick_replica2(h->S, h->D, h->t, h->stream);
        if (h->profiling) HIPCHK(h, hipEventRecord(b, h->stream));
    } else {
        launch_update_only(h->S, h->D, h->t, h->stream);
        launch_match_dfs(h->S, h->D, h->t, h->stream);
    }
    HIPCHK(h, hipGetLastError());
    h->last_stepped = h->t;
    return VDS_OK;
}

int vds_advance(vds_handle *h) {
    if (!h || !h->have_reset) return fail(h, VDS_EINVAL, "vds_advance: call vds_reset first");
    if (h->last_stepped != h->t) return fail(h, VDS_EINVAL, "vds_advance: tick %d has not been stepped", h->t);
    h->t++;
    return VDS_OK;
}

static int run_eager(vds_handle *h, int32_t n_ticks) {
    for (int i = 0; i < n_ticks; ++i) {
        int rc = guarded(h, "vds_run", [&] { return step_impl(h, false); });
        if (rc) return rc;
        rc = vds_advance(h);
        if (rc) return rc;
    }
    if (h->S.dense_st && n_ticks > 0) {
        Emit e; e.st = h->stream;
        emit_dense_flush(e, h->S, h->D, 0, 0);
        HIPCHK(h, hipGetLastError());
    }
    return VDS_OK;
}

static bool run_groups_hybrid(const vds_handle *h) { return h->dfs_mode && h->hybrid_ok && h->cfg.force_generic == 0; }
static bool run_groups_plain(const vds_handle *h) {
    return !h->dfs_mode && h->S.fast_ok && (h->S.dense || h->S.max_nc * h->S.max_nc <= h->lds_ints);
}
static int run_group_count(vds_handle *h) {
    if (!(run_groups_hybrid(h) || run_groups_plain(h))) return 1;
    if (h->run_groups < 0) {
        const char *v = getenv("VDS_RUN_GROUPS");
        h->run_groups = (v && *v) ? atoi(v) : 0;
    }
    if (h->run_stagger < 0) {
        const char *v = getenv("VDS_RUN_STAGGER");
        h->run_stagger = (v && *v) ? atoi(v) : 1;
    }
    if (!h->use_graph) return 1;
    int G = h->run_groups > 0 ? h->run_groups : 1;
    const int chunks = (h->S.R + 15) / 16;
    if (G > chunks) G = chunks;
    if (G > RUN_GROUPS_MAX) G = RUN_GROUPS_MAX;
    return G < 1 ? 1 : G;
}

static int build_group_graph(vds_handle *h, int32_t n_ticks, int G, hipGraph_t *out) {
    hipGraph_t g = nullptr;
    HIPCHK(h, hipGraphCreate(&g, 0));
    const int chunks = (h->S.R + 15) / 16;
    hipGraphNode_t prev = nullptr;
    hipError_t err = hipSuccess;
    for (int i = 0; i < n_ticks && err == hipSuccess; ++i) {
        const int t = h->t + i;
        for (int gi = 0; gi < G && err == hipSuccess; ++gi) {
            const int c0 = (int)((long long)chunks * gi / G), c1 = (int)((long long)chunks * (gi + 1) / G);
            const int r_lo = c0 * 16, r_n = (c1 * 16 < h->S.R ? c1 * 16 : h->S.R) - r_lo;
            if (r_n <= 0) continue;
            hipGraphNode_t node = nullptr;
            Emit e;
            e.graph = g; e.deps = prev ? &prev : nullptr; e.ndeps = prev ? 1 : 0; e.node = &node; e.err = &err;
            if (!h->dfs_mode) {
                if (h->S.dense) emit_tick_dense(e, tick_static(h, t), h->D, t, r_lo, r_n);
                else emit_tick_rows(e, h->S, h->D, t, h->lds_ints, r_lo, r_n);
                if (err != hipSuccess) break;
                prev = node;
                continue;
            }
            if (h->S.dense_st) emit_tick_dense(e, tick_static(h, t), h->D, t, r_lo, r_n);
            else emit_hybrid_rows(e, h->S, h->D, t, h->lds_ints, r_lo, r_n);
            if (err != hipSuccess) break;
            prev = node;
            e.deps = &prev; e.ndeps = 1; e.node = &node;
            emit_hybrid_walk(e, h->S, h->D, t, r_lo, r_n);
            if (err != hipSuccess) break;
            prev = node;
            if (h->S.dense_st && i == n_ticks - 1) {
                e.deps = &prev; e.ndeps = 1; e.node = &node;
                emit_dense_flush(e, h->S, h->D, r_lo, r_n);
                if (err != hipSuccess) break;
                prev = node;
            }
        }
    }
    if (err != hipSuccess) {
        (void)hipGraphDestroy(g);
        (void)hipGetLastError();
        return fail(h, VDS_EHIP, "vds_run: hipGraphAddKernelNode failed: %s", hipGetErrorString(err));
    }
    *out = g;
    return VDS_OK;
}

int vds_run(vds_handle *h, int32_t n_ticks) {
    if (!h || !h->have_reset) return fail(h, VDS_EINVAL, "vds_run: call vds_reset first");
    if (h->use_graph < 0) { const char *v = getenv("VDS_RUN_GRAPH"); h->use_graph = (v && *v == '0') ? 0 : 1; }
    if (!h->use_graph || h->profiling || n_ticks < 8 || h->last_stepped == h->t || h->t + n_ticks > h->S.T) return run_eager(h, n_ticks);
    HIPCHK(h, hipSetDevice(h->cfg.device));
    { const int rcs = dev_copy_sync(h); if (rcs) return rcs; }
    const int G = run_group_count(h);
    if (!(h->run_exec && !h->run_stale && h->run_t0 == h->t && h->run_n == n_ticks && h->run_stream == h->stream && h->run_G == G)) {
        const int t0 = h->t, ls0 = h->last_stepped;
        hipGraph_t g = nullptr;
        int rc;
        hipError_t ec = hipSuccess;
        if (G > 1) {
            rc = build_group_graph(h, n_ticks, G, &g);
        } else {
            if (hipStreamBeginCapture(h->stream, hipStreamCaptureModeThreadLocal) != hipSuccess) { (void)hipGetLastError(); return run_eager(h, n_ticks); }
            rc = run_eager(h, n_ticks);
            ec = hipStreamEndCapture(h->stream, &g);
        }
        h->t = t0; h->last_stepped = ls0;
        if (rc || ec != hipSuccess || !g) {
            if (g) (void)hipGraphDestroy(g);
            (void)hipGetLastError();
            if (rc) return rc;
            return run_eager(h, n_ticks);
        }
        bool updated = false;
        if (h->run_exec && h->run_n == n_ticks && h->run_G == G) {
            (void)hipStreamSynchronize(h->run_stream);
            hipGraphNode_t bad = nullptr;
            hipGraphExecUpdateResult res;
            updated = hipGraphExecUpdate(h->run_exec, g, &bad, &res) == hipSuccess;
            if (!updated) (void)hipGetLastError();
        }
        if (!updated) {
            drop_run_graph(h);
            const hipError_t ei = hipGraphInstantiate(&h->run_exec, g, nullptr, nullptr, 0);
            if (ei != hipSuccess) { (void)hipGraphDestroy(g); h->run_exec = nullptr; (void)hipGetLastError(); return run_eager(h, n_ticks); }
        }
        (void)hipGraphDestroy(g);
        h->run_t0 = t0; h->run_n = n_ticks; h->run_stream = h->stream; h->run_G = G; h->run_stale = false;
    }
    HIPCHK(h, hipGraphLaunch(h->run_exec, h->stream));
    h->t += n_ticks;
    h->last_stepped = h->t - 1;
    return VDS_OK;
}

int vds_get_run_groups(vds_handle *h) {
    if (!h || !h->have_static) return 1;
    if (h->use_graph < 0) { const char *v = getenv("VDS_RUN_GRAPH"); h->use_graph = (v && *v == '0') ? 0 : 1; }
    return run_group_count(h);
}

int vds_set_run_groups(vds_handle *h, int32_t groups, int32_t stagger) {
    if (!h) return VDS_EINVAL;
    if (groups > RUN_GROUPS_MAX || stagger > 2) return fail(h, VDS_EINVAL, "vds_set_run_groups: groups <= %d, stagger 0 / 1 / 2 (or negative: default)", RUN_GROUPS_MAX);
    { h->run_stale = true; h->tables_gen++; }
    h->run_groups = groups > 0 ? groups : -1;
    h->run_stagger = stagger >= 0 ? stagger : -1;
    return VDS_OK;
}

static int ensure_outcomes(vds_handle *h);

static int run_hooked_eager(vds_handle *h, int32_t n_ticks, int32_t planes, int32_t K, const void *dev_actions, void *policy_graph) {
    if (policy_graph && h->hook_policy_inst != policy_graph) {
        if (h->hook_policy_exec) { (void)hipStreamSynchronize(h->stream); (void)hipGraphExecDestroy(h->hook_policy_exec); h->hook_policy_exec = nullptr; }
        HIPCHK(h, hipGraphInstantiate(&h->hook_policy_exec, (hipGraph_t)policy_graph, nullptr, nullptr, 0));
        h->hook_policy_inst = policy_graph;
    }
    for (int i = 0; i < n_ticks; ++i) {
        int rc = vds_step(h);
        if (rc) return rc;
        if ((planes & 31) && (rc = vds_obs_device_planes(h, planes & 31, nullptr))) return rc;
        if ((planes & VDS_PLANE_OUTCOMES) && (rc = vds_outcomes_device(h, nullptr))) return rc;
        if (policy_graph) HIPCHK(h, hipGraphLaunch(h->hook_policy_exec, h->stream));
        if (K > 0 && dev_actions && (rc = vds_apply_dispatch_device(h, K, dev_actions))) return rc;
        if ((rc = vds_advance(h))) return rc;
    }
    return VDS_OK;
}

static int run_hooked_impl(vds_handle *h, int32_t n_ticks, int32_t planes, int32_t K, const void *dev_actions, void *policy_graph) {
    if (!h || !h->have_reset) return fail(h, VDS_EINVAL, "vds_run_hooked: call vds_reset first");
    if (n_ticks < 0 || planes < 0 || planes > 63 || K < 0 || K > 64 || (K > 0 && !dev_actions))
        return fail(h, VDS_EINVAL, "vds_run_hooked: planes is a mask of the five observation planes and VDS_PLANE_OUTCOMES (0 .. 63), K in [0, 64] with a non-null action tensor");
    if (h->last_stepped == h->t) return fail(h, VDS_EINVAL, "vds_run_hooked: tick %d already stepped; call vds_advance", h->t);
    if (h->t + n_ticks > h->S.T) return fail(h, VDS_EINVAL, "vds_run_hooked: %d slots from slot %d on run past the end of the day (%d slots, :1048)", n_ticks, h->t, h->S.T);
    if (n_ticks == 0) return VDS_OK;
    HIPCHK(h, hipSetDevice(h->cfg.device));
    if (planes & VDS_PLANE_OUTCOMES) { const int rco = ensure_outcomes(h); if (rco) return rco; }
    if (h->use_graph < 0) { const char *v = getenv("VDS_RUN_GRAPH"); h->use_graph = (v && *v == '0') ? 0 : 1; }
    const bool groupable = run_groups_hybrid(h) || run_groups_plain(h);
    if (!h->use_graph || h->profiling || !groupable) return run_hooked_eager(h, n_ticks, planes, K, dev_actions, policy_graph);
    { const int rcs = dev_copy_sync(h); if (rcs) return rcs; }
    (void)run_group_count(h);
    const int G = h->run_groups > 0 ? std::min(run_group_count(h), RUN_GROUPS_MAX) : 1;
    const bool same = h->hook_exec && h->hook_gen == h->tables_gen && h->hook_t0 == h->t && h->hook_n == n_ticks && h->hook_G == G && h->hook_planes == planes && h->hook_K == K &&
                      h->hook_actions == dev_actions && h->hook_policy == policy_graph && h->hook_stream == h->stream && h->hook_outc == h->d_outc;
    if (!same) {
        hipGraph_t g = nullptr;
        HIPCHK(h, hipGraphCreate(&g, 0));
        const int chunks = (h->S.R + 15) / 16;
        hipGraphNode_t chain = nullptr;
        hipError_t err = hipSuccess;
        for (int i = 0; i < n_ticks && err == hipSuccess; ++i) {
            const int t = h->t + i;
            for (int gi = 0; gi < G && err == hipSuccess; ++gi) {
                const int c0 = (int)((long long)chunks * gi / G), c1 = (int)((long long)chunks * (gi + 1) / G);
                const int r_lo = c0 * 16, r_n = (c1 * 16 < h->S.R ? c1 * 16 : h->S.R) - r_lo;
                if (r_n <= 0) continue;
                hipGraphNode_t n1 = nullptr, n2 = nullptr, n3 = nullptr;
                Emit e;
                e.graph = g; e.deps = chain ? &chain : nullptr; e.ndeps = chain ? 1 : 0; e.node = &n1; e.err = &err;
                if (!h->dfs_mode) {
                    if (h->S.dense) emit_tick_dense(e, tick_static(h, t), h->D, t, r_lo, r_n);
                    else emit_tick_rows(e, h->S, h->D, t, h->lds_ints, r_lo, r_n);
                } else {
                    if (h->S.dense_st) emit_tick_dense(e, tick_static(h, t), h->D, t, r_lo, r_n);
                    else emit_hybrid_rows(e, h->S, h->D, t, h->lds_ints, r_lo, r_n);
                    if (err != hipSuccess) break;
                    e.deps = &n1; e.ndeps = 1; e.node = &n2;
                    emit_hybrid_walk(e, h->S, h->D, t, r_lo, r_n);
                    n1 = n2;
                    if (h->S.dense_st && err == hipSuccess) {
                        hipGraphNode_t nf = nullptr;
                        e.deps = &n1; e.ndeps = 1; e.node = &nf;
                        emit_dense_flush(e, h->S, h->D, r_lo, r_n);
                        n1 = nf;
                    }
                }
                if (err != hipSuccess) break;
                chain = n1;
                if (planes & 31) {
                    e.deps = &chain; e.ndeps = 1; e.node = &n3;
                    emit_pack_obs(e, h->S, h->D, t, 1, planes & 31, h->d_obs, r_lo, r_n);
                    if (err != hipSuccess) break;
                    chain = n3;
                }
                if (planes & VDS_PLANE_OUTCOMES) {
                    hipGraphNode_t n4 = nullptr;
                    e.deps = &chain; e.ndeps = 1; e.node = &n4;
                    emit_slot_outcomes(e, h->S, h->D, t, 1, h->d_outc, r_lo, r_n);
                    if (err != hipSuccess) break;
                    chain = n4;
                }
            }
            if (err != hipSuccess) break;
            if (policy_graph) {
                hipGraphNode_t join = nullptr, pol = nullptr, fork = nullptr;
                err = hipGraphAddEmptyNode(&join, g, chain ? &chain : nullptr, chain ? 1 : 0);
                if (err != hipSuccess) break;
                err = hipGraphAddChildGraphNode(&pol, g, &join, 1, (hipGraph_t)policy_graph);
                if (err != hipSuccess) break;
                err = hipGraphAddEmptyNode(&fork, g, &pol, 1);
                if (err != hipSuccess) break;
                chain = fork;
            }
            for (int gi = 0; gi < G && err == hipSuccess && K > 0; ++gi) {
                const int c0 = (int)((long long)chunks * gi / G), c1 = (int)((long long)chunks * (gi + 1) / G);
                const int r_lo = c0 * 16, r_n = (c1 * 16 < h->S.R ? c1 * 16 : h->S.R) - r_lo;
                if (r_n <= 0) continue;
                hipGraphNode_t nd = nullptr;
                Emit e;
                e.graph = g; e.deps = chain ? &chain : nullptr; e.ndeps = chain ? 1 : 0; e.node = &nd; e.err = &err;
                emit_dispatch_dense(e, h->S, h->D, t, K, (const int *)dev_actions, 0, r_lo, r_n);
                if (err != hipSuccess) break;
                chain = nd;
            }
        }
        if (err != hipSuccess) {
            (void)hipGraphDestroy(g);
            (void)hipGetLastError();
            return fail(h, VDS_EHIP, "vds_run_hooked: building the day graph failed: %s", hipGetErrorString(err));
        }
        bool updated = false;
        if (h->hook_exec && h->hook_n == n_ticks && h->hook_G == G && ((h->hook_planes & 31) != 0) == ((planes & 31) != 0) && (h->hook_planes & VDS_PLANE_OUTCOMES) == (planes & VDS_PLANE_OUTCOMES) && (h->hook_K > 0) == (K > 0) && (h->hook_policy != nullptr) == (policy_graph != nullptr)) {
            (void)hipStreamSynchronize(h->hook_stream);
            hipGraphNode_t bad = nullptr;
            hipGraphExecUpdateResult res;
            updated = hipGraphExecUpdate(h->hook_exec, g, &bad, &res) == hipSuccess;
            if (!updated) (void)hipGetLastError();
        }
        if (!updated) {
            drop_hook_graph(h);
            const hipError_t ei = hipGraphInstantiate(&h->hook_exec, g, nullptr, nullptr, 0);
            if (ei != hipSuccess) {
                (void)hipGraphDestroy(g); h->hook_exec = nullptr; (void)hipGetLastError();
                return run_hooked_eager(h, n_ticks, planes, K, dev_actions, policy_graph);
            }
        }
        (void)hipGraphDestroy(g);
        h->hook_t0 = h->t; h->hook_n = n_ticks; h->hook_G = G; h->hook_planes = planes; h->hook_K = K; h->hook_actions = dev_actions;
        h->hook_policy = policy_graph; h->hook_stream = h->stream; h->hook_gen = h->tables_gen; h->hook_outc = h->d_outc;
    }
    HIPCHK(h, hipGraphLaunch(h->hook_exec, h->stream));
    h->t += n_ticks;
    h->last_stepped = h->t - 1;
    if (K > 0) { h->dispatch_seq += K * n_ticks; h->seq_tick = -1; }
    return VDS_OK;
}

int vds_run_hooked(vds_handle *h, int32_t n_ticks, int32_t planes, int32_t K, const void *dev_actions, void *policy_graph) {
    return guarded(h, "vds_run_hooked", [&] { return run_hooked_impl(h, n_ticks, planes, K, dev_actions, policy_graph); });
}

int vds_run_hooked_invalidate(vds_handle *h) {
    if (!h) return VDS_EINVAL;
    HIPCHK(h, hipSetDevice(h->cfg.device));
    drop_hook_graph(h);
    return VDS_OK;
}

int vds_sync(vds_handle *h) {
    if (!h) return VDS_EINVAL;
    HIPCHK(h, hipSetDevice(h->cfg.device));
    HIPCHK(h, hipStreamSynchronize(h->stream));
    if (!h->have_static) return VDS_OK;
    int err[4] = {0, 0, 0, 0};
    HIPCHK(h, hipMemcpy(err, h->D.err, sizeof(err), hipMemcpyDeviceToHost));
    if (err[0] & ERR_IDLE_CAP) return fail(h, VDS_ECAPACITY, "idle table overflow: more than idle_cap=%d idle vehicles in one (replica, cluster); raise it: vds_config.idle_cap / vds_set_idle_cap + vds_reset_again (Simulation(..., idle_cap=N), BatchedDispatchEnv.set_idle_cap)", h->S.idle_cap);
    if (err[0] & ERR_FL_CAP) return fail(h, VDS_ECAPACITY, "far-arrival table overflow: more than far_cap=%d vehicles on trips longer than the ring horizon to one (replica, cluster); raise vds_config.far_cap", h->S.fl_cap);
    if (err[0] & ERR_INBOX_CAP) return fail(h, VDS_ECAPACITY, "far-arrival inbox overflow: more than far_cap=%d long trips sent to one (replica, cluster) in one tick; raise vds_config.far_cap", h->S.in_cap);
    if (err[0] & ERR_RING_CAP) return fail(h, VDS_ECAPACITY, "arrival ring overflow: more than ring_cap=%d vehicles due in one (replica, cluster) in one tick; raise vds_config.ring_cap", h->S.ring_cap);
    if (err[0] & ERR_DISPATCH) {
        const int keep = err[0] & ~ERR_DISPATCH;
        HIPCHK(h, hipMemcpy(h->D.err, &keep, sizeof(int), hipMemcpyHostToDevice));
        return fail(h, VDS_ESTATE, "dispatch of an idle position that does not exist (or listed twice); the action was skipped");
    }
    return VDS_OK;
}

int vds_clock(const vds_handle *h, int32_t *step, int32_t *now_min) {
    if (!h || !h->have_orders) return VDS_EINVAL;
    if (step) *step = h->t;
    if (now_min) *now_min = h->S.now0 + h->t * h->S.tick_minutes;
    return VDS_OK;
}

static int apply_dispatch_impl(vds_handle *h, int32_t n, const int32_t *replica, const int32_t *from_cluster,
                       const int32_t *idle_pos, const int32_t *target_node, const int32_t *arrive_min = nullptr,
                       const int32_t *counted = nullptr) {
    if (!h || !h->have_reset) return fail(h, VDS_EINVAL, "vds_apply_dispatch: call vds_reset first");
    if (h->last_stepped != h->t) return fail(h, VDS_EINVAL, "vds_apply_dispatch: must follow vds_step of the current tick (the hook runs after Match, :1083)");
    if (n == 0) return VDS_OK;
    if (n < 0 || !replica || !from_cluster || !idle_pos || !target_node) return fail(h, VDS_EINVAL, "vds_apply_dispatch: bad argument");
    HIPCHK(h, hipSetDevice(h->cfg.device));
    const Static &S = h->S;
    if (h->seq_tick != h->t) { h->seq_tick = h->t; h->seq_tick0 = h->dispatch_seq; }
    if (S.dense && (long long)(h->dispatch_seq - h->seq_tick0) + n >= (1 << DENSE_ID_BITS))
        return fail(h, VDS_ECAPACITY, "vds_apply_dispatch: more than 2^%d dispatch actions in one slot (the dense arrival keys carry a %d-bit sequence number); vds_config.force_generic = 5 selects the wide layout", DENSE_ID_BITS, DENSE_ID_BITS);
    std::vector<int> order(n);
    for (int i = 0; i < n; ++i) {
        order[i] = i;
        if (replica[i] < 0 || replica[i] >= h->R_ext || from_cluster[i] < 0 || from_cluster[i] >= S.C)
            return fail(h, VDS_EINVAL, "vds_apply_dispatch: action %d: replica/cluster out of range", i);
        if (target_node[i] < 0 || target_node[i] >= S.N || h->node2cluster[target_node[i]] < 0)
            return fail(h, VDS_ESTATE, "vds_apply_dispatch: action %d: target node %d is in no cluster", i, target_node[i]);
        if (h->t >= h->days[h->replica_day[replica[i]]].T)
            return fail(h, VDS_ESTATE, "vds_apply_dispatch: action %d: the day of replica %d is over (%d ticks), its city stands still", i, replica[i], h->days[h->replica_day[replica[i]]].T);
    }
    std::stable_sort(order.begin(), order.end(), [&](int a, int b) {
        if (replica[a] != replica[b]) return replica[a] < replica[b];
        return from_cluster[a] < from_cluster[b];
    });
    for (int k = 1; k < n; ++k) {
        const int a = order[k - 1], b = order[k];
        if (replica[a] == replica[b] && from_cluster[a] == from_cluster[b]) {
            for (int j = k - 1; j >= 0 && replica[order[j]] == replica[b] && from_cluster[order[j]] == from_cluster[b]; --j)
                if (idle_pos[order[j]] == idle_pos[b])
                    return fail(h, VDS_ESTATE, "vds_apply_dispatch: actions %d and %d name the same idle position %d of cluster %d, replica %d",
                                order[j], b, idle_pos[b], from_cluster[b], replica[b]);
// ... 660 lines not shown
```

vehicles_dispatch_simulator_amd/csrc/vds_device.h:

```cpp
#pragma once
#include <hip/hip_runtime.h>
#include <stdint.h>

namespace vds {

enum {
    HDR_IDLE = 0,
    HDR_IDLE_PRE = 1,
    HDR_ORDERS = 2,
    HDR_FL = 3,
    HDR_INBOX0 = 4,
    HDR_INBOX1 = 5,
    HDR_RAW = 6,
    HDR_CNT32 = 8,
    HDR_WORDS = 16
};

enum {
    CNT_ORDERS = 0, CNT_REJECTS = 1, CNT_WAIT = 2, CNT_VALUE = 3,
    CNT_EVALS = 4, CNT_ARRIVALS = 5, CNT_DISPATCH = 6, CNT_DISPATCH_COST = 7, CNT_WORDS = 8
};

enum { ERR_IDLE_CAP = 1, ERR_FL_CAP = 2, ERR_INBOX_CAP = 4, ERR_DISPATCH = 8, ERR_RING_CAP = 16 };

__host__ __device__ inline int meta_pack(int tick, int is_dispatch, int dest_local) {
    return (tick << 16) | (is_dispatch << 15) | dest_local;
}
__host__ __device__ inline int meta_dest(int w) { return w & 0x7FFF; }
__host__ __device__ inline int meta_is_dispatch(int w) { return (w >> 15) & 1; }
__host__ __device__ inline unsigned long long entry_key(int id, int w) {
    return ((unsigned long long)((unsigned)w >> 15) << 32) | (unsigned)id;
}

struct DayDesc {
    int bkt_base;
    int tick_base;
    int now0;
    int T;
    int q_base;
    int Oq;
    int max_tick_orders;
    int pad;
};
struct DayView { const int *bkt_off; const int *tick_off; int now0, T, q_base; };

struct State;
struct Static {
    int N, C, V, R, Oq, T;
    int R_ext;
    const int *int2ext;
    int n_days;
    const int *rperm;
    int rslots;
    int chunk_days;
    int row_gran;
    const DayDesc *day;
    const int *replica_day;
    const int4 *replica_desc;
    int tick_minutes, now0;
    unsigned tick_magic;
    int tick_div_limit;
    long long reject_threshold;
    int idle_cap, fl_cap, in_cap;
    int H, ring_cap;
    int fast_ok;
    int window_live;
    int max_nc;
    const int *cost;
    const int *node2cluster;
    const int *node_local;
    const int *cl_off;
    const int *cl_nodes;
    const long long *blk_off;
    const int *blk;
    const int4 *cdesc;
    const int *corder;
    const int4 *cdesc_ord;
    const unsigned char *blk8;
    const unsigned char *cost8;
    int u8_ok;
    const unsigned char *lbc;
    const int *dfs_off;
    const int *dfs_seq;
    const unsigned *vis_bits;
    const int4 *so_rec;
    const int *bkt_off;
    const int *tick_off;
    const int *ord_q;
    const int *so_pnode;
    int walk_pool;
    const unsigned *so_vis;
    const unsigned char *so_lb;
    int seq_pad;
    const int *so_rank;
    int max_tick_orders;
    int r_lo;
    int dense;
    int dense_lpr;
    int dense_tab, dense_keys;
    int dense_force_slow;
    const Static *self_dev;
    const struct State *state_dev;
    int pull, pull_W, pull_hmax;
    int arr_slots;
    const int *so_slot;
    const int2 *d_rec;
    const int *d_first;
    const int4 *replica_desc2;
    int ring_min_on;
    const int *blk32s;
    const unsigned char *blk8s;
    const int4 *cdesc_dense;
    int dense_st;
    const int4 *tdesc;
};

struct Emit {
    hipStream_t st = nullptr;
    hipGraph_t graph = nullptr;
    const hipGraphNode_t *deps = nullptr;
    size_t ndeps = 0;
    hipGraphNode_t *node = nullptr;
    hipError_t *err = nullptr;
};

struct State {
    int *hdr;
    long long *cnt;
    uint2 *idle;
    int4 *ring;
    int *ring_cnt;
    int4 *fl;
    int4 *inbox;
    int4 *slog;
    int2 *out;
    int *err;
    int *work;
    unsigned *arr;
    unsigned short *stamp;
    int *slow_tick;
    int *dry;
    int *sup;
    int *sup_slot;
    int *ring_min;
};

#define DENSE_PULL_WMAX 3
#define VDS_SUP_PLANES 32
__host__ __device__ inline size_t sup_index(int C, int R, int slot, int c, int r) { return ((size_t)(slot & (VDS_SUP_PLANES - 1)) * C + c) * R + r; }
__host__ __device__ inline size_t arr_index(int R, int slot, int r) { return (size_t)slot * (size_t)R + (size_t)r; }
__host__ __device__ inline unsigned pull_entry(int veh, int arrival_slot) { return ((unsigned)veh << 8) | ((unsigned)arrival_slot & 0xFFu); }
__host__ __device__ inline unsigned pull_reject(int t) { return 0xFFFFFF00u | ((unsigned)(t + 128) & 0xFFu); }
__host__ __device__ inline bool pull_is_reject(unsigned e) { return (e >> 8) == 0xFFFFFFu; }
__host__ __device__ inline int pull_slots_ahead(unsigned e, int now_slot) { return (int)(signed char)((e & 0xFFu) - ((unsigned)now_slot & 0xFFu)); }
#define DENSE_DEAD_COST 0x00FFFFFF
#define DENSE_ID_BITS 25
__host__ __device__ inline unsigned dense_pack(unsigned veh, unsigned loc) { return (veh << 8) | (loc & 0xFFu); }
__host__ __device__ inline unsigned dense_key(int tick, int is_dispatch, int id) {
    return ((unsigned)(tick & 63) << 26) | ((unsigned)(is_dispatch & 1) << 25) | ((unsigned)id & ((1u << DENSE_ID_BITS) - 1));
}
__host__ __device__ inline unsigned dense_key_rel(unsigned key, int t) { return key - ((unsigned)((t - 32) & 63) << 26); }
__host__ __device__ inline int dense_key_is_dispatch(unsigned key) { return (int)((key >> 25) & 1u); }
__host__ __device__ inline int dense_key_id(unsigned key) { return (int)(key & ((1u << DENSE_ID_BITS) - 1)); }
__host__ __device__ inline int dense_key_tick(unsigned key, int t_now) { return t_now - (int)(((unsigned)t_now - (key >> 26)) & 63u); }

struct IdleRef {
    uint2 *p;
    unsigned *q;
    __device__ __forceinline__ uint2 get(int e) const {
        if (!q) return p[e];
        const unsigned v = q[e];
        return make_uint2(v >> 8, v & 0xFFu);
    }
    __device__ __forceinline__ void set(int e, uint2 v) const {
        if (!q) p[e] = v;
        else q[e] = dense_pack(v.x, v.y);
    }
};
__device__ __forceinline__ IdleRef idle_ref(const Static &S, const State &D, int c, int r) {
    IdleRef f;
    const size_t off = ((size_t)c * S.R + r) * S.idle_cap;
    if (S.dense) { f.p = nullptr; f.q = reinterpret_cast<unsigned *>(D.idle) + off; }
    else { f.p = D.idle + off; f.q = nullptr; }
    return f;
}
__device__ __forceinline__ uint2 *ring2(const State &D) { return reinterpret_cast<uint2 *>(D.ring); }

__device__ __forceinline__ DayView day_view(const Static &S, int r) {
    if (S.n_days <= 1) return DayView{S.bkt_off, S.tick_off, S.now0, S.T, 0};
    const DayDesc d = S.day[S.replica_day[r]];
    return DayView{S.bkt_off + d.bkt_base, S.tick_off + d.tick_base, d.now0, d.T, d.q_base};
}
__device__ __forceinline__ int2 *out_row(const Static &S, const State &D, int r) {
    const int qb = S.n_days <= 1 ? 0 : S.day[S.replica_day[r]].q_base;
    return D.out + (size_t)r * S.Oq - qb;
}

}
```

vehicles_dispatch_simulator_amd/csrc/vds_tick_dense.hip:

```cpp
#include "vds_kernels_common.h"
#include <algorithm>

namespace vds {

VDS_PROF_ACCESSORS(dense)

#define SPAN_TICKS 256
#ifdef VDS_PROF
#define SPAN_WAYS 64
static __device__ unsigned long long g_span[2 * SPAN_TICKS * SPAN_WAYS * 2];
void read_span_dense(unsigned long long *out, int reset, hipStream_t st) {
    (void)hipStreamSynchronize(st);
    static unsigned long long host[2 * SPAN_TICKS * SPAN_WAYS * 2];
    if (out) {
        (void)hipMemcpyFromSymbol(host, HIP_SYMBOL(g_span), sizeof(host));
        for (int i = 0; i < 2 * SPAN_TICKS; ++i) {
            unsigned long long lo = ~0ull, hi = 0ull;
            for (int w = 0; w < SPAN_WAYS; ++w) { lo = std::min(lo, host[(i * SPAN_WAYS + w) * 2]); hi = std::max(hi, host[(i * SPAN_WAYS + w) * 2 + 1]); }
            out[2 * i] = lo; out[2 * i + 1] = hi;
        }
    }
    if (reset) {
        for (int i = 0; i < 2 * SPAN_TICKS * SPAN_WAYS; ++i) { host[2 * i] = ~0ull; host[2 * i + 1] = 0ull; }
        (void)hipMemcpyToSymbol(HIP_SYMBOL(g_span), host, sizeof(host));
    }
}
#else
void read_span_dense(unsigned long long *, int, hipStream_t) { }
#endif

#define DN_ROWS 16
#define DN_TAB 128
#define DN_KEYS 64
#define DN_ORDERS 64
#ifndef DN_ROWS32
#define DN_ROWS32 1
#endif
#define DN_TPAD 4

struct DenseArgs {
    int *hdr; long long *cnt; unsigned *idle; uint2 *ring; int *ring_cnt; int4 *inbox; int2 *out; int *err;
    const int4 *cdesc_dense; const char *blk; const int4 *so_rec; const int *bkt_off; const int4 *replica_desc; const int *rperm;
    int R, C, H, idle_cap, ring_cap, in_cap, Oq, arr_slots;
    int tick_minutes, now0, tick_div_limit; unsigned tick_magic;
    int r_lo, r_hi, dense_tab, dense_keys, dense_force_slow;
    int *ring_min;
    unsigned *arr; const int *so_slot; const int2 *d_rec; const int *d_first; const int4 *replica_desc2; int pull_W;
    const int4 *tdesc;
    unsigned short *stamp; int *dry; int *slow_tick; const int *so_rank;
    int *sup, *sup_slot;
    const Static *Sdev; const State *Ddev;
};
__device__ __forceinline__ uint2 *ring2(const DenseArgs &D) { return D.ring; }
__device__ __forceinline__ int ticks_until_fast(const DenseArgs &S, int rel) {
    const int n = rel + S.tick_minutes - 1;
    if (S.tick_div_limit > (1 << 26)) return (int)__umulhi((unsigned)n, S.tick_magic);
    return n / S.tick_minutes;
}

template <int LPR>
__device__ __forceinline__ int grp_min(int v) {
    v = min(v, dpp_mov<0xB1, 0xF>(v, v));
    v = min(v, dpp_mov<0x4E, 0xF>(v, v));
    if (LPR >= 8) v = min(v, dpp_mov<0x141, 0xF>(v, v));
    if (LPR >= 16) v = min(v, dpp_mov<0x140, 0xF>(v, v));
    return v;
}
template <int LPR>
__device__ __forceinline__ int grp_max(int v) {
    v = max(v, dpp_mov<0xB1, 0xF>(v, v));
    v = max(v, dpp_mov<0x4E, 0xF>(v, v));
    if (LPR >= 8) v = max(v, dpp_mov<0x141, 0xF>(v, v));
    if (LPR >= 16) v = max(v, dpp_mov<0x140, 0xF>(v, v));
    return v;
}
template <int LPR>
__device__ __forceinline__ int grp_sum(int v) {
    v += dpp_mov<0xB1, 0xF>(v, v);
    v += dpp_mov<0x4E, 0xF>(v, v);
    if (LPR >= 8) v += dpp_mov<0x141, 0xF>(v, v);
    if (LPR >= 16) v += dpp_mov<0x140, 0xF>(v, v);
    return v;
}
template <int LPR>
__device__ __forceinline__ int grp_incl_scan(int v, int lg) {
    int t;
    t = dpp_zero<0x111>(v); v += (LPR >= 16 || lg >= 1) ? t : 0;
    t = dpp_zero<0x112>(v); v += (LPR >= 16 || lg >= 2) ? t : 0;
    if (LPR >= 8) { t = dpp_zero<0x114>(v); v += (LPR >= 16 || lg >= 4) ? t : 0; }
    if (LPR >= 16) { t = dpp_zero<0x118>(v); v += t; }
    return v;
}
template <int LPR>
__device__ __forceinline__ int wave_max_of_groups(int v) {
    if (LPR == 16) return max(max(rdlane(v, 0), rdlane(v, 16)), max(rdlane(v, 32), rdlane(v, 48)));
    v = max(v, dpp_mov<0x141, 0xF>(v, v));
    if (LPR == 4) v = max(v, dpp_mov<0x4E, 0xF>(v, v));
    v = max(v, dpp_mov<0x140, 0xF>(v, v));
    return max(max(rdlane(v, 0), rdlane(v, 16)), max(rdlane(v, 32), rdlane(v, 48)));
}
__device__ __forceinline__ unsigned loc_bytes4(unsigned e0, unsigned e1, unsigned e2, unsigned e3) {
    const unsigned t01 = __builtin_amdgcn_perm(e1, e0, 0x0c0c0400u);
    const unsigned t23 = __builtin_amdgcn_perm(e3, e2, 0x0c0c0400u);
    return __builtin_amdgcn_perm(t23, t01, 0x05040100u);
}

__device__ __forceinline__ unsigned bfi(unsigned mask, unsigned a, unsigned b) { return (mask & a) | (~mask & b); }
__device__ __forceinline__ unsigned byte_of(unsigned v, int i) { return (v >> (8 * i)) & 0xFFu; }

__device__ __forceinline__ int wave_incl_scan_i32(int v) {
    v = row_incl_scan_i32(v);
    v += __builtin_amdgcn_update_dpp(0, v, 0x142, 0xA, 0xF, false);
    v += __builtin_amdgcn_update_dpp(0, v, 0x143, 0xC, 0xF, false);
    return v;
}
__device__ __forceinline__ int wave_sum_i32(int v) {
    for (int o = 32; o > 0; o >>= 1) v += __shfl_xor(v, o, WAVE);
    return v;
}

template <int J, bool ST = false>
__device__ int dense_match_wave(const Static &S, const State &D, int r, int t, int now, int m, int q0, int k, const unsigned char *lds_blk, int nc,
                                unsigned *idle, int &wait_sum, int &value_sum, long long &evals, int &rejects, unsigned short *stamp = nullptr) {
    constexpr int NL = J / 4;
    const int lane = lane_id();
    const int lbase = lane * J;
    unsigned e[J];
#pragma unroll
    for (int s = 0; s < J; ++s) e[s] = 0u;
    if (lbase < m) {
#pragma unroll
        for (int s = 0; s < J; s += 4) {
            const uint4 v = *reinterpret_cast<const uint4 *>(idle + lbase + s);
            e[s] = v.x; e[s + 1] = v.y; e[s + 2] = v.z; e[s + 3] = v.w;
        }
    }
    const unsigned ncrep = (unsigned)nc * 0x01010101u;
    unsigned L[NL];
#pragma unroll
    for (int i = 0; i < NL; ++i) {
        const unsigned v = loc_bytes4(e[4 * i], e[4 * i + 1], e[4 * i + 2], e[4 * i + 3]);
        const int nv = min(max(m - lbase - 4 * i, 0), 4);
        L[i] = bfi((unsigned)(0xFFFFFFFFull << (8 * nv)), ncrep, v);
    }
    int navail = m;
    int2 *out_r = out_row(S, D, r);
    for (int base = 0; base < k; base += WAVE) {
        const int kk = min(WAVE, k - base);
        int4 rec = make_int4(0, 0, 0, 0);
        int slot = -1, rank = 0;
        if (lane < kk) { rec = S.so_rec[q0 + base + lane]; if (S.pull) slot = S.so_slot[q0 + base + lane]; if (ST) rank = S.so_rank[q0 + base + lane]; }
        int res = IMAX;
        for (int j = 0; j < kk; ++j) {
            const int p = rdlane(rec.y, j) & 0xFFFF;
            const unsigned char *row = lds_blk + p * (nc + 1);
            int best = IMAX;
#pragma unroll
            for (int s = 0; s < J; ++s) best = min(best, (int)(((unsigned)row[byte_of(L[s >> 2], s & 3)] << 10) | (unsigned)s));
            best += lbase;
            const int rmin = wave_min_i32(best);
            const int wrel = (rmin & 1023) - lbase;
            const unsigned bm = 0xFFu << ((wrel & 3) << 3);
            const int hi = wrel >> 2;
#pragma unroll
            for (int i = 0; i < NL; ++i) L[i] = bfi(hi == i ? bm : 0u, ncrep, L[i]);
            res = lane == j ? rmin : res;
            evals += navail;
            navail -= (rmin >> 10) != 0xFF ? 1 : 0;
        }
        const bool has = lane < kk;
        const bool matched = has && (res >> 10) != 0xFF;
        const int wait = res >> 10, wpos = res & 1023;
        unsigned went = 0;
#pragma unroll
        for (int s = 0; s < J; ++s) {
            const unsigned got = (unsigned)__builtin_amdgcn_ds_bpermute((wpos / J) << 2, (int)e[s]);
            went = (wpos % J) == s ? got : went;
        }
        const int vid = matched ? (int)(went >> 8) : -1;
        if (ST && matched) stamp[wpos] = (unsigned short)rank;
        if (has) {
            out_r[q0 + base + lane] = make_int2(vid, matched ? wait : -1);
            if (slot >= 0) {
                const int rel = wait + rec.w;
                const int d = rel <= 0 ? 1 : ticks_until<true>(S, rel);
                D.arr[arr_index(S.R, slot, r)] = matched ? pull_entry(vid, t + d) : pull_reject(t);
                if (D.sup != nullptr && matched) atomicAdd(&D.sup[sup_index(S.C, S.R, t + d, rec.z & 0xFFFF, r)], 1);
            } else if (matched) post_arrival<true, true>(S, D, rec.z & 0xFFFF, r, t, now, vid, rec.x, now + wait + rec.w, 0, (int)((unsigned)rec.y >> 16));
        }
        wait_sum += wave_sum_i32(matched ? wait : 0);
        value_sum += wave_sum_i32(matched ? rec.w : 0);
        rejects += wave_sum_i32((has && !matched) ? 1 : 0);
    }
    if (ST) return navail;
    int alive = 0, firstdead = IMAX;
#pragma unroll
    for (int s = J - 1; s >= 0; --s) {
        const bool dead = byte_of(L[s >> 2], s & 3) == (unsigned)nc;
        alive += dead ? 0 : 1;
        firstdead = dead ? lbase + s : firstdead;
    }
    const int incl = wave_incl_scan_i32(alive);
// ... 601 lines not shown
            }
        }
        wave_order();
        if (J >= 4) {
#pragma unroll
            for (int s = 0; s < J; s += 4) *reinterpret_cast<uint4 *>(tab + lbase + s) = make_uint4(0xFFFFu, 0xFFFFu, 0xFFFFu, 0xFFFFu);
        } else {
            *reinterpret_cast<uint2 *>(tab + lbase) = make_uint2(0xFFFFu, 0xFFFFu);
        }
        wave_order();
    } else {
    int alive = 0, firstdead = IMAX;
#pragma unroll
    for (int s = J - 1; s >= 0; --s) {
        const bool dead = byte_of(L[s >> 2], s & 3) == (unsigned)nc;
        alive += dead ? 0 : 1;
        firstdead = dead ? lbase + s : firstdead;
    }
    const int incl = grp_incl_scan<LPR>(alive, lg);
    mfin = grp_sum<LPR>(alive);
    int fc = grp_min<LPR>(firstdead);
    fc = A > 0 ? min(fc, m) : fc;
    wave_order();
    {
        int wp = incl - alive;
#pragma unroll
        for (int s = 0; s < J; ++s) {
            if (byte_of(L[s >> 2], s & 3) != (unsigned)nc) { tab[wp] = e[s]; wp++; }
        }
    }
    wave_order();
    if (rowvalid && lbase < mfin && lbase + J > fc && !(abl & 2)) {
        if (J >= 4) {
#pragma unroll
            for (int s = 0; s < J; s += 4) {
                if (lbase + s < mfin && lbase + s + 4 > fc) *reinterpret_cast<uint4 *>(idle + lbase + s) = *reinterpret_cast<const uint4 *>(tab + lbase + s);
            }
        } else {
            *reinterpret_cast<uint2 *>(idle + lbase) = *reinterpret_cast<const uint2 *>(tab + lbase);
        }
    }
    }
    PROF_STAMP(7);
    int wsum = 0, vsum = 0, rej = 0;
    int2 *out_r = D.out + (size_t)r * S.Oq + (q0 - qb);
#pragma unroll
    for (int jj = 0; jj < NG; ++jj) {
        if (jj * LPR >= kmax) break;
        const int j = jj * LPR + lg;
        const bool has = rowvalid && j < k;
        int4 rr;
        if (DM == 2) { rr = make_int4(0, 0, 0, 0); if (has) rr = S.so_rec[q0 + j]; }
        else rr = lds_rec[j < k ? j : 0];
        const int rv = res[jj];
        const bool matched = has && (rv >> PB) != DEAD;
        const int wait = rv >> PB;
        const int wpos = rv & PM;
        const int src = (gbase + (wpos / J)) << 2;
        unsigned went = 0;
#pragma unroll
        for (int s = 0; s < J; ++s) {
            const unsigned got = (unsigned)__builtin_amdgcn_ds_bpermute(src, (int)e[s]);
            went = (wpos % J) == s ? got : went;
        }
        const int vid = matched ? (int)(went >> 8) : -1;
        if (has && !(abl & 8)) out_r[j] = make_int2(vid, matched ? wait : -1);
        if (ST && matched) tab[wpos] = (unsigned)lds_rank[j];
        int slot = -1;
        if (PULL) { if (DM == 2) { if (has) slot = S.so_slot[q0 + j]; } else slot = lds_slot[j < k ? j : 0]; }
        if (PULL && slot >= 0) {
            const int rel = wait + rr.w;
            const int d = rel <= 0 ? 1 : ticks_until_fast(S, rel);
            if (has && !(abl & 1)) D.arr[arr_index(S.R, slot, r)] = matched ? pull_entry(vid, t + d) : pull_reject(t);
            if (D.sup != nullptr && matched && !(abl & 1)) atomicAdd(&D.sup[sup_index(S.C, S.R, t + d, rr.z & 0xFFFF, r)], 1);
#ifdef VDS_PROF
            if (has && (abl & 65536)) reinterpret_cast<unsigned *>(D.ring_min)[arr_index(S.R, slot, r)] = (unsigned)vid;
#endif
        } else if (matched && !(abl & 1)) {
            const int rel = wait + rr.w;
            const int d = rel <= 0 ? 1 : ticks_until_fast(S, rel);
            const int dc = rr.z & 0xFFFF;
            if (d < S.H) {
                const size_t i = ((size_t)(((t + d) & (S.H - 1)) * S.C + dc)) * S.R + r;
                int pos = (rr.x & 7);
                if (D.sup != nullptr) atomicAdd(&D.sup[sup_index(S.C, S.R, t + d, dc, r)], 1);
                if (!(abl & 64)) pos = atomicAdd(&D.ring_cnt[i], (abl & 32) ? 0 : 0x10001) & 0xFFFF;
                if (pos >= S.ring_cap) atomicOr(&D.err[0], ERR_RING_CAP);
                else if (!(abl & 32)) ring2(D)[i * S.ring_cap + pos] = make_uint2(dense_pack((unsigned)vid, (unsigned)rr.y >> 16), dense_key(t, 0, rr.x));
#ifdef VDS_PROF
                if (abl & (4096 | 8192 | 16384)) {
                    int *sh = D.ring_min + i * S.ring_cap;
                    int p2 = pos & 3;
                    if (abl & (4096 | 8192)) p2 = atomicAdd(&sh[0], 0x10001) & 3;
                    if (abl & (4096 | 16384)) *reinterpret_cast<uint2 *>(sh + 2 + 2 * p2) = make_uint2((unsigned)vid, (unsigned)rr.x);
                }
#endif
            } else {
                const size_t db = (size_t)dc * S.R + r;
                const int np = (t + 1) & 1;
                const int slot = atomicAdd(&D.hdr[db * HDR_WORDS + HDR_INBOX0 + np], 1);
                if (slot < S.in_cap) D.inbox[((size_t)np * S.C * S.R + db) * S.in_cap + slot] = make_int4(vid, rr.x, now + rel, meta_pack(t, 0, (int)((unsigned)rr.y >> 16)));
                else atomicOr(&D.err[0], ERR_INBOX_CAP);
            }
        }
        wsum += matched ? wait : 0;
        vsum += matched ? rr.w : 0;
        rej += (has && !matched) ? 1 : 0;
    }
    wsum = grp_sum<LPR>(wsum);
    vsum = grp_sum<LPR>(vsum);
    rej = grp_sum<LPR>(rej);
    if (ST) {
        wave_order();
        if (rowvalid && lbase < max(mnew, m_raw)) {
            unsigned pk[(J + 1) / 2];
#pragma unroll
            for (int s = 0; s < J; s += 2) pk[s >> 1] = (tab[lbase + s] & 0xFFFFu) | (tab[lbase + s + 1] << 16);
            unsigned *sp = reinterpret_cast<unsigned *>(D.stamp + b * S.idle_cap + lbase);
            if (J >= 8) {
#pragma unroll
                for (int s = 0; s < J / 2; s += 4) *reinterpret_cast<uint4 *>(sp + s) = make_uint4(pk[s], pk[s + 1], pk[s + 2], pk[s + 3]);
            } else if (J == 4) *reinterpret_cast<uint2 *>(sp) = make_uint2(pk[0], pk[1]);
            else sp[0] = pk[0];
        }
        if (rowvalid && lg == 0 && capable && k > mnew) atomicAdd(&D.dry[r], 1);
    }
    if (rowvalid && lg == 2 && D.sup != nullptr) D.sup[(size_t)(t & (VDS_SUP_PLANES - 1)) * S.C * S.R + b] = 0;
    if (rowvalid && !(abl & 16)) {
        if (REC && ST) store_record<true>(D.hdr + b * HDR_WORDS, lg, hw, mfin, mnew, k, rej, wsum, vsum, evals, A, mfin != mnew ? mnew + 1 : 0);
        else if (REC) store_record(D.hdr + b * HDR_WORDS, lg, hw, mfin, mnew, k, rej, wsum, vsum, evals, A);
        else {
            if (lg < 3) D.hdr[b * HDR_WORDS + lg] = lg == HDR_IDLE ? mfin : (lg == HDR_IDLE_PRE ? mnew : k);
            if (!(abl & 32768)) store_counters<LPR>(D.cnt + b * CNT_WORDS, lg, cntv, k, rej, wsum, vsum, evals, A);
        }
    }
    PROF_STAMP(8);
}

#ifndef DN_MIN_WAVES16
#define DN_MIN_WAVES16 8
#endif
#ifndef DN_MIN_WAVES8
#define DN_MIN_WAVES8 6
#endif
#ifndef DN_MIN_WAVES4
#define DN_MIN_WAVES4 4
#endif
#ifndef DN_MIN_WAVES256
#define DN_MIN_WAVES256 7
#endif

#define DN_CAND 128

template <bool U8, int DM, int LPR, bool PULL, int TABMAX = DN_TAB, int ROWS = DN_ROWS, bool ST = false>
__global__ __launch_bounds__(ROWS * LPR, TABMAX > 128 ? DN_MIN_WAVES256 : (LPR == 16 ? DN_MIN_WAVES16 : (LPR == 8 ? DN_MIN_WAVES8 : DN_MIN_WAVES4))) void k_tick_dense(DenseArgs P, int t) {
    static_assert(TABMAX == 128 || (TABMAX == 256 && LPR == 16 && U8), "256-entry tables: 16 lanes per replica, byte costs");
    static_assert(!ST || (U8 && DM == 0 && PULL), "stamp form: byte costs, one shared day, static arrival slots");
    static_assert(ROWS == DN_ROWS || (ROWS == 32 && DM == 0 && LPR == 8) || ((ROWS == 8 || ROWS == 4) && DM == 1 && LPR == 16),
                  "32-row workgroups: one shared day, 8 lanes per replica; 8- / 4-row workgroups: one day per workgroup, 16 lanes per replica");
    const DenseArgs &S = P, &D = P;
#ifdef VDS_PROF
    const int span_i = (((P.r_lo != 0 ? 1 : 0) * SPAN_TICKS + (t & (SPAN_TICKS - 1))) * SPAN_WAYS + (int)(blockIdx.x & (SPAN_WAYS - 1))) * 2;
    if ((g_ablate & 1048576) && threadIdx.x == 0) atomicMin(&g_span[span_i], (unsigned long long)__builtin_amdgcn_s_memrealtime());
    struct SpanEnd { int i; __device__ ~SpanEnd() { if ((g_ablate & 1048576) && threadIdx.x == 0) atomicMax(&g_span[i + 1], (unsigned long long)__builtin_amdgcn_s_memrealtime()); } } span_end{span_i};
#endif
    if (DN_ABL & 512) return;
    if (blockIdx.x == 0 && threadIdx.x == 0 && P.sup_slot != nullptr) P.sup_slot[0] = (t + 1) & (VDS_SUP_PLANES - 1);
    typedef typename std::conditional<U8, unsigned char, int>::type CT;
    constexpr int RPW = WAVE / LPR;
    constexpr int NTHR = ROWS * LPR;
    extern __shared__ int lds_dyn[];
    int4 *lds_rec = reinterpret_cast<int4 *>(lds_dyn);
    int *lds_slot = reinterpret_cast<int *>(lds_rec + (DM == 2 ? DN_ROWS * DN_ORDERS * 2 / 16 : DN_ORDERS));
    int *lds_rank = lds_slot + (PULL ? DN_ORDERS : 0);
    int2 *lds_drec = reinterpret_cast<int2 *>(lds_rank + (ST ? DN_ORDERS : 0));
    unsigned *tab_all = reinterpret_cast<unsigned *>(lds_drec + (PULL ? DN_CAND : 0));
    CT *lds_blk = reinterpret_cast<CT *>(tab_all + ROWS * (TABMAX + DN_TPAD));
    const int nchunks = gridDim.x / S.C;
    int4 cd, td0 = make_int4(0, 0, 0, 0);
    if (DM == 0) {
        const int4 *tp = S.tdesc + 2 * ((size_t)t * S.C + blockIdx.x / nchunks);
        td0 = tp[0]; cd = tp[1];
    } else cd = S.cdesc_dense[blockIdx.x / nchunks];
    const int c = cd.z, nc = cd.x;
    const int row0 = S.r_lo + (int)(blockIdx.x % nchunks) * ROWS;
    const int wave = __builtin_amdgcn_readfirstlane((int)(threadIdx.x >> 6));
    const int lane = lane_id();
    const int g = lane / LPR, lg = lane & (LPR - 1);
    const int p = t & 1;
    const int rslot = row0 + wave * RPW + g;
    const int r = (DM == 1 && S.rperm != nullptr) ? S.rperm[rslot < S.r_hi ? rslot : S.r_lo] : rslot;
    bool rowvalid = rslot < S.r_hi && r >= 0 && r < S.R;
    unsigned short *pick = reinterpret_cast<unsigned short *>(lds_rec) + (wave * RPW + g) * DN_ORDERS;
#ifdef VDS_PROF
    const bool prof = (g_ablate & 128) != 0;
    unsigned long long tprev = prof ? __builtin_amdgcn_s_memtime() : 0ull;
#else
    const bool prof = false;
    unsigned long long tprev = 0ull;
#endif
    const int pwave = (int)((blockIdx.x * (NTHR / WAVE) + wave) & (PROF_WAVES - 1));
    int q0, k, now, qb = 0;
    int clo = 0, n = 0, qdb = 0;
    const int2 *drec_row = nullptr;
    if (DM == 2) {
        q0 = 0; k = 0; now = S.now0 + t * S.tick_minutes;
        if (rowvalid) {
            const int4 dd = S.replica_desc[r];
            rowvalid = t < dd.z;
            now = dd.y + t * S.tick_minutes;
            qb = dd.w;
            if (rowvalid) {
                const int *bo = S.bkt_off + dd.x + (size_t)t * S.C + c;
                q0 = bo[0]; k = bo[1] - q0;
                if (PULL) {
                    const int4 d2 = S.replica_desc2[r];
                    const int *df = S.d_first + d2.x;
                    clo = df[(size_t)max(t - S.pull_W, 0) * S.C + c];
                    n = df[(size_t)(t + 1) * S.C + c] - clo;
                    qdb = d2.y;
                    drec_row = S.d_rec + clo;
                }
            }
        }
    } else if (DM == 1) {
        const int r0 = row0;
        const int rd = S.rperm != nullptr ? S.rperm[r0] : min(r0, S.R - 1);
        if (rd < 0) return;
        const int4 dd = S.replica_desc[rd];
        rowvalid = rowvalid && t < dd.z;
        q0 = 0; k = 0;
        if (t < dd.z) {
            const int *bo = S.bkt_off + dd.x + (size_t)t * S.C + c;
            q0 = bo[0]; k = bo[1] - q0;
            if (PULL) {
                const int4 d2 = S.replica_desc2[rd];
                const int *df = S.d_first + d2.x;
                clo = df[(size_t)max(t - S.pull_W, 0) * S.C + c];
                n = df[(size_t)(t + 1) * S.C + c] - clo;
                qdb = d2.y;
            }
        }
        now = dd.y + t * S.tick_minutes;
        qb = dd.w;
    } else {
        const int4 td = td0;
        q0 = td.x; k = td.y;
        now = S.now0 + t * S.tick_minutes;
        if (PULL) { clo = td.z; n = td.w; }
    }
    const size_t b = (size_t)c * S.R + (rowvalid ? r : 0);
    const size_t si = (size_t)(t & (S.H - 1)) * S.C * S.R + b;
    const bool wg_ok = k <= DN_ORDERS && n <= DN_CAND;
    unsigned *tab = tab_all + (wave * RPW + g) * (TABMAX + DN_TPAD);
    int m = 0, far = 0, A = 0;
    long long cntv = 0;
    int4 h0 = make_int4(0, 0, 0, 0);
    int hin = 0, rcw = 0;
    int2 hw = make_int2(0, 0);
    if (rowvalid) {
        if (U8) { if (lg < 8) hw = *reinterpret_cast<const int2 *>(D.hdr + b * HDR_WORDS + 2 * lg); }
        else {
            h0 = *reinterpret_cast<const int4 *>(D.hdr + b * HDR_WORDS);
            hin = D.hdr[b * HDR_WORDS + HDR_INBOX0 + p];
            if (LPR >= CNT_WORDS && lg < CNT_WORDS && !(DN_ABL & 131072)) cntv = D.cnt[b * CNT_WORDS + lg];
        }
        rcw = D.ring_cnt[si];
    }
    const char *blk_g = S.blk + cd.y;
    const int4 *blk4 = reinterpret_cast<const int4 *>(blk_g);
    const int n4 = (nc * (nc + 1) * (int)sizeof(CT) + 15) >> 4;
    const bool stage = DM != 2 && k > 0;
    const bool mine = stage && (int)threadIdx.x < min(k, DN_ORDERS);
    const bool dmine = PULL && DM != 2 && wg_ok && (int)threadIdx.x < n;
    int4 sblk = make_int4(0, 0, 0, 0), srec = make_int4(0, 0, 0, 0);
    int sslot = -1, srank = 0;
    int2 sdrec = make_int2(0, 0);
    if (stage && (int)threadIdx.x < n4 && !(DN_ABL & 1024)) sblk = blk4[threadIdx.x];
    if (mine) { srec = S.so_rec[q0 + threadIdx.x]; if (PULL) sslot = S.so_slot[q0 + threadIdx.x]; if (ST) srank = S.so_rank[q0 + threadIdx.x]; }
    if (dmine) sdrec = S.d_rec[clo + threadIdx.x];
    int Ac = 0;
    if (PULL && wg_ok) {
        const unsigned *ar = D.arr + arr_index(S.R, clo - qdb, rowvalid ? r : 0);
        const unsigned never = pull_reject(t - 1);
        const int gsh = lane & ~(LPR - 1);
        constexpr int NIF = 4;
        for (int i0 = 0; i0 < n; i0 += NIF * LPR) {
            unsigned v[NIF];
#pragma unroll
            for (int u = 0; u < NIF; ++u) {
                const int idx = i0 + u * LPR + lg;
                v[u] = never;
                if (idx < n && rowvalid) v[u] = ar[(size_t)idx * S.R];
            }
#pragma unroll
            for (int u = 0; u < NIF; ++u) {
                const int idx = i0 + u * LPR + lg;
                const bool now_ = (v[u] & 0xFFu) == ((unsigned)t & 0xFFu);
                const unsigned gm = (unsigned)(ballot(now_) >> gsh) & ((1u << LPR) - 1u);
                const int pos = Ac + __popc(gm & ((1u << lg) - 1u));
                if (now_ && pos < DN_TH) { tab[pos] = v[u]; tab[DN_TH + pos] = (unsigned)idx; }
                Ac += __popc(gm);
            }
        }
    }
    asm volatile("" : "+v"(rcw));
    int Aring = rcw & 0xFFFF;
    A = Aring + Ac;
    int m_raw = 0;
    if (U8) {
        const int gb = (lane & ~(LPR - 1)) << 2;
        m = __builtin_amdgcn_ds_bpermute(gb, hw.x);
        far = __builtin_amdgcn_ds_bpermute(gb + 4, hw.y) | __builtin_amdgcn_ds_bpermute(gb + 8, p ? hw.y : hw.x);
        if (ST) { const int rw = __builtin_amdgcn_ds_bpermute(gb + 12, hw.x); m_raw = rw ? rw - 1 : m; }
    } else {
        m = h0.x;
        far = h0.w | hin;
    }
    if (DN_ABL & 256) { if (m + far + A + (int)cntv == 0x7FFFFFF1) D.err[1] = 1; return; }
    if (DM == 2) {
        int4 *lds4 = reinterpret_cast<int4 *>(lds_blk);
        for (int i = threadIdx.x; i < n4; i += NTHR) lds4[i] = blk4[i];
        if (wg_ok)
            for (int j = lg; j < k; j += LPR) pick[j] = (unsigned short)((S.so_rec[q0 + j].y & 0xFFFF) * (nc + 1));
    } else if (k > 0) {
        int4 *lds4 = reinterpret_cast<int4 *>(lds_blk);
        if (!(DN_ABL & 1024)) {
            if ((int)threadIdx.x < n4) lds4[threadIdx.x] = sblk;
            for (int i = threadIdx.x + NTHR; i < n4; i += NTHR) lds4[i] = blk4[i];
        }
        if (mine) { lds_rec[threadIdx.x] = srec; if (PULL) lds_slot[threadIdx.x] = sslot; if (ST) lds_rank[threadIdx.x] = srank; }
    }
    if (dmine) lds_drec[threadIdx.x] = sdrec;
    if (NTHR < DN_CAND && PULL && DM != 2 && wg_ok)
        for (int i = threadIdx.x + NTHR; i < n; i += NTHR) lds_drec[i] = S.d_rec[clo + i];
    PROF_STAMP(0);
    __syncthreads();
    PROF_STAMP_NW(1);
    const int mnew0 = ST ? max(m + A, m_raw) : m + A;
    const bool bad = rowvalid && (!wg_ok || far != 0 || Aring > S.dense_keys || Aring > S.ring_cap || A > DN_TAB || mnew0 > min(S.dense_tab, TABMAX) || mnew0 > S.idle_cap || S.dense_force_slow ||
                                  (PULL && (A - Aring > S.dense_keys * 2 || A > DN_TH)));
#ifdef VDS_PROF
    if (bad && lg == 0) {
        const int why = k > DN_ORDERS ? 4 : (n > DN_CAND ? 5 : (far != 0 ? 6 : ((Aring > S.dense_keys || Aring > S.ring_cap) ? 7 : (A > DN_TAB ? 8 : ((mnew0 > min(S.dense_tab, TABMAX) || mnew0 > S.idle_cap) ? 9 :
                        ((PULL && A - Aring > S.dense_keys * 2) ? 10 : 11))))));
        atomicAdd(&D.err[why], 1);
    }
#endif
    const unsigned long long badrows = ballot(bad && lg == 0);
    if (badrows != 0ull && lane == 0) {
        atomicAdd(&D.err[2], popc64(badrows));
        if (D.slow_tick != nullptr) atomicAdd(&D.slow_tick[t], popc64(badrows));
    }
    if (bad) { rowvalid = false; m = 0; A = 0; Aring = 0; }
    if (!rowvalid) m_raw = 0;
    const bool any = ballot(rowvalid) != 0;
    const int mmax = wave_max_of_groups<LPR>(ST ? max(m + A, m_raw) : m + A);
    PROF_STAMP_NW(2);
    if (any) {
        const int nn = (wg_ok && rowvalid) ? n : 0;
        const int kr = (DM == 2 && !rowvalid) ? 0 : k;
        const int kmax = DM == 2 ? wave_max_of_groups<LPR>(kr) : k;
        const int2 *drec = DM == 2 ? drec_row : lds_drec;
        const bool capable = ST && cd.w != 0;
        if (mmax <= 32) dense_body<LPR, 32, CT, DM, PULL, ST>(S, D, t, now, q0, kr, kmax, qb, lds_blk, nc, lds_rec, pick, tab, r, rowvalid, b, si, m, A, cntv, hw, nn, Aring, drec, lds_slot, prof, tprev, pwave, m_raw, capable, lds_rank);
        else if (mmax <= 64) dense_body<LPR, 64, CT, DM, PULL, ST>(S, D, t, now, q0, kr, kmax, qb, lds_blk, nc, lds_rec, pick, tab, r, rowvalid, b, si, m, A, cntv, hw, nn, Aring, drec, lds_slot, prof, tprev, pwave, m_raw, capable, lds_rank);
        else if (TABMAX <= 128 || mmax <= 128) dense_body<LPR, 128, CT, DM, PULL, ST>(S, D, t, now, q0, kr, kmax, qb, lds_blk, nc, lds_rec, pick, tab, r, rowvalid, b, si, m, A, cntv, hw, nn, Aring, drec, lds_slot, prof, tprev, pwave, m_raw, capable, lds_rank);
        else dense_body<LPR, (TABMAX > 128 ? 256 : 128), CT, DM, PULL, ST>(S, D, t, now, q0, kr, kmax, qb, lds_blk, nc, lds_rec, pick, tab, r, rowvalid, b, si, m, A, cntv, hw, nn, Aring, drec, lds_slot, prof, tprev, pwave, m_raw, capable, lds_rank);
    }
    for (unsigned long long rest = badrows; rest; rest &= rest - 1) {
        const int l0 = __ffsll((long long)rest) - 1;
        dense_bucket_slow<CT, ST>(*P.Sdev, *P.Ddev, c, rdlane(r, l0), t, reinterpret_cast<const CT *>(blk_g), nc, (DM == 2 || k > 0) ? lds_blk : (const CT *)nullptr);
    }
}

__global__ __launch_bounds__(256) void k_dense_flush(int *hdr, unsigned *idle_all, unsigned short *stamp_all, int R, int C, int idle_cap, int r_lo, int r_n) {
    const int wave = (int)(threadIdx.x >> 6), lane = lane_id();
    const long long bi = (long long)blockIdx.x * 4 + wave;
    if (bi >= (long long)C * r_n) return;
    const int c = (int)(bi / r_n), r = r_lo + (int)(bi % r_n);
    const size_t b = (size_t)c * R + r;
    const int rw = hdr[b * HDR_WORDS + HDR_RAW];
    if (rw == 0) return;
    const int raw = rw - 1;
    unsigned *idle = idle_all + b * idle_cap;
    unsigned short *stamp = stamp_all + b * idle_cap;
    int newm = 0;
    for (int base = 0; base < raw; base += WAVE) {
        const int i = base + lane;
        const unsigned e = i < raw ? idle[i] : 0u;
        const bool keep = i < raw && stamp[i] == 0xFFFFu;
        const unsigned long long kb = ballot(keep);
        wave_fence();
        if (keep) idle[newm + popc64(kb & lanemask_lt())] = e;
        if (i < raw) stamp[i] = (unsigned short)0xFFFFu;
        newm += popc64(kb);
        wave_fence();
    }
    if (lane == 0) hdr[b * HDR_WORDS + HDR_RAW] = 0;
}

void emit_dense_flush(const Emit &e, const Static &S, const State &D, int r_lo, int r_n) {
    if (r_n <= 0) r_n = S.R - r_lo;
    const long long nb = (long long)S.C * r_n;
    const dim3 grid((unsigned)((nb + 3) / 4)), block(256);
    int *hdr = D.hdr; unsigned *idle = reinterpret_cast<unsigned *>(D.idle); unsigned short *stamp = D.stamp;
    int R = S.R, C = S.C, cap = S.idle_cap;
    if (!e.graph) { hipLaunchKernelGGL(k_dense_flush, grid, block, 0, e.st, hdr, idle, stamp, R, C, cap, r_lo, r_n); return; }
    void *args[8] = {&hdr, &idle, &stamp, &R, &C, &cap, &r_lo, &r_n};
    hipKernelNodeParams p{};
    p.func = reinterpret_cast<void *>(k_dense_flush); p.gridDim = grid; p.blockDim = block; p.sharedMemBytes = 0; p.kernelParams = args; p.extra = nullptr;
    *e.err = hipGraphAddKernelNode(e.node, e.graph, e.deps, e.ndeps, &p);
}


static void emit_dense(const Emit &e, void (*k)(DenseArgs, int), dim3 grid, dim3 block, size_t lds, DenseArgs P, int t) {
    if (!e.graph) { hipLaunchKernelGGL(k, grid, block, lds, e.st, P, t); return; }
    void *args[2] = {&P, &t};
    hipKernelNodeParams p{};
    p.func = reinterpret_cast<void *>(k); p.gridDim = grid; p.blockDim = block; p.sharedMemBytes = (unsigned)lds; p.kernelParams = args; p.extra = nullptr;
    *e.err = hipGraphAddKernelNode(e.node, e.graph, e.deps, e.ndeps, &p);
}

static bool dense_tab256(const Static &S) { return S.dense_lpr == 16 && S.blk8s != nullptr && S.dense_tab > 128; }

template <bool PULL>
static void emit_dense_256(const Emit &e, const Static &S, const DenseArgs &P, int t, dim3 grid, size_t lds) {
    const dim3 block(DN_ROWS * 16);
    if (S.n_days > 1 && S.chunk_days && S.row_gran == 8) { emit_dense(e, k_tick_dense<true, 1, 16, PULL, 256, 8>, grid, dim3(8 * 16), lds, P, t); return; }
    if (S.n_days > 1 && S.chunk_days && S.row_gran == 4) { emit_dense(e, k_tick_dense<true, 1, 16, PULL, 256, 4>, grid, dim3(4 * 16), lds, P, t); return; }
    if (S.n_days <= 1) emit_dense(e, k_tick_dense<true, 0, 16, PULL, 256>, grid, block, lds, P, t);
    else if (S.chunk_days) emit_dense(e, k_tick_dense<true, 1, 16, PULL, 256>, grid, block, lds, P, t);
    else emit_dense(e, k_tick_dense<true, 2, 16, PULL, 256>, grid, block, lds, P, t);
}

template <int LPR, bool PULL>
static void emit_dense_lpr(const Emit &e, const Static &S, const DenseArgs &P, int t, dim3 grid, size_t lds) {
    const int dm = S.n_days <= 1 ? 0 : (S.chunk_days ? 1 : 2);
    const dim3 block(DN_ROWS * LPR);
    if (LPR == 16 && dm == 1 && S.row_gran == 8) {
        if (S.blk8s) emit_dense(e, k_tick_dense<true, 1, 16, PULL, DN_TAB, 8>, grid, dim3(8 * 16), lds, P, t);
        else emit_dense(e, k_tick_dense<false, 1, 16, PULL, DN_TAB, 8>, grid, dim3(8 * 16), lds, P, t);
        return;
    }
    if (LPR == 16 && dm == 1 && S.row_gran == 4) {
        if (S.blk8s) emit_dense(e, k_tick_dense<true, 1, 16, PULL, DN_TAB, 4>, grid, dim3(4 * 16), lds, P, t);
        else emit_dense(e, k_tick_dense<false, 1, 16, PULL, DN_TAB, 4>, grid, dim3(4 * 16), lds, P, t);
        return;
    }
    if (S.blk8s) emit_dense(e, dm == 2 ? k_tick_dense<true, 2, LPR, PULL> : (dm ? k_tick_dense<true, 1, LPR, PULL> : k_tick_dense<true, 0, LPR, PULL>), grid, block, lds, P, t);
    else emit_dense(e, dm == 2 ? k_tick_dense<false, 2, LPR, PULL> : (dm ? k_tick_dense<false, 1, LPR, PULL> : k_tick_dense<false, 0, LPR, PULL>), grid, block, lds, P, t);
}

void emit_tick_dense(const Emit &e, const Static &S, const State &D, int t, int r_lo, int r_n) {
    DenseArgs P;
    P.hdr = D.hdr; P.cnt = D.cnt; P.idle = reinterpret_cast<unsigned *>(D.idle); P.ring = reinterpret_cast<uint2 *>(D.ring);
    P.ring_cnt = D.ring_cnt; P.inbox = D.inbox; P.out = D.out; P.err = D.err;
    P.cdesc_dense = S.cdesc_dense; P.blk = S.blk8s ? reinterpret_cast<const char *>(S.blk8s) : reinterpret_cast<const char *>(S.blk32s);
    P.so_rec = S.so_rec; P.bkt_off = S.bkt_off; P.replica_desc = S.replica_desc; P.rperm = S.rperm;
    P.arr_slots = S.arr_slots; P.R = S.R; P.C = S.C; P.H = S.H; P.idle_cap = S.idle_cap; P.ring_cap = S.ring_cap; P.in_cap = S.in_cap; P.Oq = S.Oq;
    P.tick_minutes = S.tick_minutes; P.now0 = S.now0; P.tick_div_limit = S.tick_div_limit; P.tick_magic = S.tick_magic;
    P.r_lo = r_lo; P.r_hi = r_lo + (r_n > 0 ? r_n : (S.rperm != nullptr ? S.rslots : S.R) - r_lo); P.dense_tab = S.dense_tab; P.dense_keys = S.dense_keys; P.dense_force_slow = S.dense_force_slow;
    P.Sdev = S.self_dev; P.Ddev = S.state_dev; P.ring_min = D.ring_min;
    P.tdesc = S.tdesc;
    P.stamp = D.stamp; P.dry = D.dry; P.slow_tick = D.slow_tick; P.so_rank = S.so_rank; P.sup = D.sup; P.sup_slot = D.sup_slot;
    P.arr = D.arr; P.so_slot = S.so_slot; P.d_rec = S.d_rec; P.d_first = S.d_first; P.replica_desc2 = S.replica_desc2; P.pull_W = S.pull_W;
    const int slots = r_n > 0 ? r_n : (S.rperm != nullptr ? S.rslots : S.R) - r_lo;
    const bool t256 = dense_tab256(S);
    const bool rows32 = S.n_days <= 1 && S.dense_lpr == 8 && !t256 && S.blk8s != nullptr && S.pull && slots >= 64 && DN_ROWS32;
    const bool rows8 = S.n_days > 1 && S.chunk_days && S.row_gran < 16 && S.dense_lpr == 16;
    const int rows = rows32 ? 32 : (rows8 ? S.row_gran : DN_ROWS);
    const int rchunks = (slots + rows - 1) / rows;
    const dim3 grid(S.C * rchunks);
    const int bb = (S.max_nc * (S.max_nc + 1) * (S.blk8s ? 1 : 4) + 15) / 16 * 16;
    const size_t lds = (S.n_days > 1 && !S.chunk_days ? DN_ROWS * DN_ORDERS * 2 : DN_ORDERS * 16) + (S.pull ? DN_ORDERS * 8 + DN_CAND * 8 : 0) + (S.dense_st ? DN_ORDERS * 4 : 0) +
                       rows * ((t256 ? 256 : DN_TAB) + DN_TPAD) * 4 + bb;
    if (S.dense_st) {
        if (t256) emit_dense(e, k_tick_dense<true, 0, 16, true, 256, DN_ROWS, true>, grid, dim3(DN_ROWS * 16), lds, P, t);
        else if (rows32) emit_dense(e, k_tick_dense<true, 0, 8, true, DN_TAB, 32, true>, grid, dim3(32 * 8), lds, P, t);
        else if (S.dense_lpr == 8) emit_dense(e, k_tick_dense<true, 0, 8, true, DN_TAB, DN_ROWS, true>, grid, dim3(DN_ROWS * 8), lds, P, t);
        else emit_dense(e, k_tick_dense<true, 0, 16, true, DN_TAB, DN_ROWS, true>, grid, dim3(DN_ROWS * 16), lds, P, t);
        return;
    }
    if (rows32) {
        emit_dense(e, k_tick_dense<true, 0, 8, true, DN_TAB, 32>, grid, dim3(32 * 8), lds, P, t);
        return;
    }
    if (t256) {
        if (S.pull) emit_dense_256<true>(e, S, P, t, grid, lds);
        else emit_dense_256<false>(e, S, P, t, grid, lds);
        return;
    }
    if (S.pull) {
        if (S.dense_lpr == 8) emit_dense_lpr<8, true>(e, S, P, t, grid, lds);
        else emit_dense_lpr<16, true>(e, S, P, t, grid, lds);
    } else {
        if (S.dense_lpr == 8) emit_dense_lpr<8, false>(e, S, P, t, grid, lds);
        else emit_dense_lpr<16, false>(e, S, P, t, grid, lds);
    }
}

}
```

vehicles_dispatch_simulator_amd/env.py:

```python
from __future__ import annotations

import ctypes as C
from typing import Dict, Optional, Sequence

import numpy as np

from . import _lib

PICKUP_REJECT_THRESHOLD = 600_000_000_000
PLANE_OUTCOMES = 32
OUTCOME_NAMES = ("served", "rejected", "wait_sum", "value_sum")


def _p(a: Optional[np.ndarray]):
    return None if a is None else a.ctypes.data_as(C.c_void_p)


def _i32(a) -> np.ndarray:
    return np.ascontiguousarray(a, dtype=np.int32)


def neighbors_to_csr(neighbors: Sequence[Sequence[int]]):
    off = np.zeros(len(neighbors) + 1, dtype=np.int32)
    off[1:] = np.cumsum([len(x) for x in neighbors])
# ... 43 lines not shown
        if rc:
            raise Exception("libvds error %d: %s" % (rc, self._lib.vds_last_error(self._h).decode()))

    def close(self):
        if getattr(self, "_h", None) is not None and self._h.value:
            bad = self._lib.vds_debug_check_guards(self._h) if hasattr(self._lib, "vds_debug_check_guards") else 0
            msg = self._lib.vds_last_error(self._h).decode() if bad < 0 else ""
            self._lib.vds_destroy(self._h)
            self._h = C.c_void_p()
            if bad > 0:
                raise Exception("libvds guard zones damaged: %d table(s) written out of bounds (see stderr)" % bad)
            if bad < 0:
                raise Exception("libvds error %d while checking the guard zones: %s" % (bad, msg))

    def __del__(self):
        try:
            self.close()
        except Exception:
            pass

    def set_stream(self, stream):
        if stream == "legacy":
            stream = C.c_void_p(-1).value
        self._chk(self._lib.vds_set_stream(self._h, C.c_void_p(stream or 0)))

    def load_orders(self, release_min, pickup, delivery):
        r, p, d = _i32(release_min), _i32(pickup), _i32(delivery)
        self.O = r.size
        self._chk(self._lib.vds_load_orders(self._h, _p(r), _p(p), _p(d), self.O))
        t = C.c_int32()
        self._chk(self._lib.vds_num_ticks(self._h, C.byref(t)))
        self.T = t.value

    def load_order_days(self, days, replica_day=None):
        for i, d in enumerate(days):
            n = [np.asarray(x).size for x in d[:3]]
            if len(d) < 3 or n[0] != n[1] or n[0] != n[2]:
                raise Exception("load_order_days: day %d needs three arrays of equal length (release_min, pickup, delivery), got %s" % (i, n))
        rel = np.concatenate([_i32(d[0]).reshape(-1) for d in days])
        pk = np.concatenate([_i32(d[1]).reshape(-1) for d in days])
        dl = np.concatenate([_i32(d[2]).reshape(-1) for d in days])
        off = np.zeros(len(days) + 1, dtype=np.int64)
        off[1:] = np.cumsum([np.asarray(d[0]).size for d in days])
        rd = None if replica_day is None else _i32(replica_day)
        if rd is not None and rd.size != self.R:
            raise Exception("load_order_days: replica_day needs %d entries" % self.R)
        self._chk(self._lib.vds_load_order_days(self._h, len(days), _p(off), _p(rel), _p(pk), _p(dl), _p(rd)))
        self._after_load(int(np.diff(off).max()))

    def set_replica_days(self, replica_day):
        rd = _i32(replica_day)
        if rd.size != self.R:
            raise Exception("set_replica_days: replica_day needs %d entries" % self.R)
        self._chk(self._lib.vds_set_replica_days(self._h, _p(rd)))
        t = C.c_int32()
        self._chk(self._lib.vds_num_ticks(self._h, C.byref(t)))
        self.T = t.value

    def load_orders_strided(self, release_min, pickup, delivery, O: int, replica_stride: int):
        r, p, d = _i32(release_min).reshape(-1), _i32(pickup).reshape(-1), _i32(delivery).reshape(-1)
        need = int(O) if int(replica_stride) == 0 else (self.R - 1) * int(replica_stride) + int(O)
        if not (r.size == p.size == d.size) or r.size < need:
            raise Exception("load_orders_strided: the three arrays need %d elements each ((R - 1) * replica_stride + O), got %d / %d / %d"
                            % (need, r.size, p.size, d.size))
        self._chk(self._lib.vds_load_orders_strided(self._h, _p(r), _p(p), _p(d), int(O), int(replica_stride)))
        self._after_load(int(O))

    def _after_load(self, omax: int):
        self.O = omax
        t = C.c_int32()
        self._chk(self._lib.vds_num_ticks(self._h, C.byref(t)))
        self.T = t.value

    def replica_ticks(self, replica: int):
        t, n = C.c_int32(), C.c_int32()
        self._chk(self._lib.vds_replica_ticks(self._h, int(replica), C.byref(t), C.byref(n)))
        return t.value, n.value

    def set_idle_cap(self, cap: int):
        self._chk(self._lib.vds_set_idle_cap(self._h, int(cap)))

    @property
    def idle_cap(self) -> int:
        return int(self._lib.vds_idle_cap(self._h))

    def reset(self, veh_init_node):
        v = _i32(veh_init_node).reshape(-1)
        if v.size != self.R * self.V:
            raise Exception("reset: expected %d start nodes, got %d" % (self.R * self.V, v.size))
        self._chk(self._lib.vds_reset(self._h, _p(v)))

    def reset_random(self, seeds):
        s = np.ascontiguousarray(np.asarray(seeds, dtype=np.uint64).reshape(-1))
        if s.size != self.R:
            raise Exception("reset_random: expected %d seeds, got %d" % (self.R, s.size))
        self._chk(self._lib.vds_reset_random(self._h, _p(s)))

    def reset_again(self):
        self._chk(self._lib.vds_reset_again(self._h))

    def step(self):
        self._chk(self._lib.vds_step(self._h))

    def apply_dispatch(self, replica, from_cluster, idle_pos, target_node, arrive_min=None, counted=None):
        a = [_i32(x).reshape(-1) for x in (replica, from_cluster, idle_pos, target_node)]
        if arrive_min is None and counted is None:
            self._chk(self._lib.vds_apply_dispatch(self._h, a[0].size, *[_p(x) for x in a]))
            return
        am = None if arrive_min is None else _i32(arrive_min).reshape(-1)
        ct = None if counted is None else _i32(counted).reshape(-1)
        self._chk(self._lib.vds_apply_dispatch_ex(self._h, a[0].size, *[_p(x) for x in a], _p(am), _p(ct)))

    def apply_dispatch_torch(self, actions):
        if tuple(actions.shape[:1]) != (self.R,) or actions.dim() != 3 or actions.shape[2] != 3:
            raise Exception("apply_dispatch_torch: expected an int32 tensor [R, K, 3]")
        if str(actions.dtype) != "torch.int32" or not actions.is_cuda or not actions.is_contiguous():
            raise Exception("apply_dispatch_torch: expected a contiguous int32 CUDA tensor")
        self._chk(self._lib.vds_apply_dispatch_device(self._h, int(actions.shape[1]), C.c_void_p(actions.data_ptr())))

    def advance(self):
        self._chk(self._lib.vds_advance(self._h))

    def run(self, n_ticks: int):
        self._chk(self._lib.vds_run(self._h, int(n_ticks)))

    def run_hooked(self, n_ticks: int, actions=None, policy_graph=None, idle_pre=True, idle_now=True, supply=True, cl_orders=True, inflight=False,
                   outcomes=False):
        planes = (1 if idle_pre else 0) | (2 if idle_now else 0) | (4 if supply else 0) | (8 if cl_orders else 0) | (16 if inflight else 0)
        planes |= PLANE_OUTCOMES if outcomes else 0
        K, ptr = 0, None
        if actions is not None:
            if tuple(actions.shape[:1]) != (self.R,) or actions.dim() != 3 or actions.shape[2] != 3:
                raise Exception("run_hooked: expected an int32 tensor [R, K, 3]")
            if str(actions.dtype) != "torch.int32" or not actions.is_cuda or not actions.is_contiguous():
                raise Exception("run_hooked: expected a contiguous int32 CUDA tensor")
            K, ptr = int(actions.shape[1]), C.c_void_p(actions.data_ptr())
        raw = None
        if policy_graph is not None:
            raw = policy_graph if isinstance(policy_graph, int) else int(policy_graph.raw_cuda_graph())
        self._chk(self._lib.vds_run_hooked(self._h, int(n_ticks), planes, K, ptr, C.c_void_p(raw) if raw is not None else None))

    def run_hooked_invalidate(self):
        self._chk(self._lib.vds_run_hooked_invalidate(self._h))

    def set_run_groups(self, groups: int = 0, stagger: int = -1):
        self._chk(self._lib.vds_set_run_groups(self._h, int(groups), int(stagger)))

    def tick_forms(self) -> np.ndarray:
        out = np.zeros(max(self.T, 1), dtype=np.uint8)
        n = C.c_int32()
        self._chk(self._lib.vds_debug_tick_forms(self._h, _p(out), int(out.size), C.byref(n)))
        return out[:n.value].copy()

    def run_groups(self) -> int:
        return int(self._lib.vds_get_run_groups(self._h))

    def sync(self):
        self._chk(self._lib.vds_sync(self._h))

    @property
    def clock(self):
        s, n = C.c_int32(), C.c_int32()
        self._chk(self._lib.vds_clock(self._h, C.byref(s), C.byref(n)))
        return s.value, n.value

    def obs(self) -> Dict[str, np.ndarray]:
        names = ("idle_pre", "idle_now", "supply", "cl_orders", "inflight")
        arrs = [np.empty((self.R, self.C), dtype=np.int32) for _ in names]
        self._chk(self._lib.vds_read_obs(self._h, *[_p(a) for a in arrs]))
        return dict(zip(names, arrs))

    def obs_device_ptr(self, planes: int = 31) -> int:
        p = C.c_void_p()
        self._chk(self._lib.vds_obs_device_planes(self._h, int(planes), C.byref(p)))
        return p.value

    def obs_torch(self, inflight: bool = True, idle_pre: bool = True, idle_now: bool = True, supply: bool = True, cl_orders: bool = True):
        import torch

        class _Block:
            pass

        blk = _Block()
        blk.__cuda_array_interface__ = {"shape": (5, self.R, self.C), "typestr": "<i4", "data": (self.obs_device_ptr((1 if idle_pre else 0) | (2 if idle_now else 0) | (4 if supply else 0) | (8 if cl_orders else 0) | (16 if inflight else 0)), False),
                                        "version": 2, "strides": None}
        return torch.as_tensor(blk, device=torch.device("cuda", self.device))

    def obs_inplace_torch(self):
        import torch

        out = {}
        for name, k in (("idle_pre", 0), ("idle_now", 1), ("cl_orders", 3)):
            p, sr, sc = C.c_void_p(), C.c_int64(), C.c_int64()
            self._chk(self._lib.vds_obs_inplace(self._h, k, C.byref(p), C.byref(sr), C.byref(sc)))

            class _Block:
                pass

            blk = _Block()
            blk.__cuda_array_interface__ = {"shape": (self.R, self.C), "typestr": "<i4", "data": (p.value, False), "version": 2,
                                            "strides": (4 * sr.value, 4 * sc.value)}
            out[name] = torch.as_tensor(blk, device=torch.device("cuda", self.device))
        return out

    def supply_inplace_torch(self):
        import torch

        ring, slot, planes = C.c_void_p(), C.c_void_p(), C.c_int32()
        sp, sr, sc = C.c_int64(), C.c_int64(), C.c_int64()
        self._chk(self._lib.vds_supply_inplace(self._h, C.byref(ring), C.byref(sp), C.byref(sr), C.byref(sc), C.byref(slot), C.byref(planes)))

        class _Block:
            pass

        blk = _Block()
        blk.__cuda_array_interface__ = {"shape": (planes.value, self.R, self.C), "typestr": "<i4", "data": (ring.value, False), "version": 2,
                                        "strides": (4 * sp.value, 4 * sr.value, 4 * sc.value)}
        sw = _Block()
        sw.__cuda_array_interface__ = {"shape": (1,), "typestr": "<i4", "data": (slot.value, False), "version": 2}
        dev = torch.device("cuda", self.device)
        return torch.as_tensor(blk, device=dev), torch.as_tensor(sw, device=dev)

    def counters_torch(self):
        import torch

        p = C.c_void_p()
        self._chk(self._lib.vds_counters_device(self._h, C.byref(p)))

        class _Block:
            pass

        blk = _Block()
        blk.__cuda_array_interface__ = {"shape": (self.R, 8), "typestr": "<i8", "data": (p.value, False), "version": 2, "strides": None}
        return torch.as_tensor(blk, device=torch.device("cuda", self.device))

    def outcomes_device_ptr(self) -> int:
        p = C.c_void_p()
        self._chk(self._lib.vds_outcomes_device(self._h, C.byref(p)))
        return p.value

    def outcomes_torch(self):
        import torch

        class _Block:
            pass

        blk = _Block()
        blk.__cuda_array_interface__ = {"shape": (4, self.R, self.C), "typestr": "<i8", "data": (self.outcomes_device_ptr(), False),
                                        "version": 2, "strides": None}
        return torch.as_tensor(blk, device=torch.device("cuda", self.device))

    def outcomes(self) -> Dict[str, np.ndarray]:
        arrs = [np.empty((self.R, self.C), dtype=np.int64) for _ in OUTCOME_NAMES]
        self._chk(self._lib.vds_read_outcomes(self._h, *[_p(a) for a in arrs]))
        return dict(zip(OUTCOME_NAMES, arrs))

    def counters(self) -> np.ndarray:
        out = np.zeros((self.R, _lib.NUM_COUNTERS), dtype=np.int64)
        self._chk(self._lib.vds_read_counters(self._h, _p(out)))
        return out

    def total_counters(self, want_device_ptr: bool = False):
        out = np.zeros(_lib.NUM_COUNTERS, dtype=np.int64)
        p = C.c_void_p()
        self._chk(self._lib.vds_reduce_counters(self._h, _p(out), C.byref(p)))
        return (out, p.value) if want_device_ptr else out

    def reduce_counters_into(self, dev_ptr: int):
        self._chk(self._lib.vds_reduce_counters_into(self._h, C.c_void_p(dev_ptr)))

    def profile(self, on: bool):
        self._chk(self._lib.vds_profile_enable(self._h, int(bool(on))))

    def main_kernel(self) -> str:
        return (self._lib.vds_main_kernel(self._h) or b"").decode()

    def profile_read(self, cap: int = 4096) -> np.ndarray:
        ms = np.zeros(cap, dtype=np.float32)
        n = C.c_int32()
        self._chk(self._lib.vds_profile_read(self._h, _p(ms), cap, C.byref(n)))
        return ms[:n.value].copy()

    def vehicles(self, replica: int) -> Dict[str, np.ndarray]:
        V = self.V
        st = np.zeros(V, dtype=np.uint8)
        arrs = [np.zeros(V, dtype=np.int32) for _ in range(4)]
        self._chk(self._lib.vds_read_vehicles(self._h, int(replica), _p(st), *[_p(a) for a in arrs]))
        return dict(state=st, node=arrs[0], cluster=arrs[1], arrive_min=arrs[2], order=arrs[3])

    def work(self) -> Dict[str, int]:
        out = np.zeros(8, dtype=np.int64)
        self._chk(self._lib.vds_read_work(self._h, _p(out)))
        return dict(zip(("ticks", "orders", "matches", "evals", "arrivals", "dispatches", "slow_path_buckets"), out.tolist()))

    def orders(self, r0: int = 0, nr: Optional[int] = None) -> Dict[str, np.ndarray]:
        nr = self.R - r0 if nr is None else nr
        st = np.zeros((nr, self.O), dtype=np.uint8)
        veh = np.zeros((nr, self.O), dtype=np.int32)
        wt = np.zeros((nr, self.O), dtype=np.int32)
        self._chk(self._lib.vds_read_orders(self._h, r0, nr, _p(st), _p(veh), _p(wt)))
        return dict(status=st, vehicle=veh, wait=wt)

    def lists(self, replica: int) -> Dict[str, np.ndarray]:
        V, Cn = self.V, self.C
        io, ao = np.zeros(Cn + 1, dtype=np.int32), np.zeros(Cn + 1, dtype=np.int32)
        arrs = [np.full(V, -1, dtype=np.int32) for _ in range(6)]
# ... 5 lines not shown
```

Measured before the change: 22.25 million.

## Choose dense tick kernel form per (slot, cluster) with mixed-form launch

The slow-bucket counter grows from one counter per tick slot to one per (slot, cluster). The adaptive pass now marks individual clusters for the 16-lane/256-entry table form instead of switching a whole slot. Slots that end up with both forms get a block map on the device and a single k_tick_dense_mixed launch, where each workgroup picks its own form. The goal is to keep most clusters on the cheaper 8-lane form while avoiding slow-path fallbacks in the clusters that need larger tables; the cost is more host bookkeeping, a device bmap upload, and LDS sized for the larger of the two forms.

```diff
diff --git a/include/vds_debug.h b/include/vds_debug.h
--- a/include/vds_debug.h
+++ b/include/vds_debug.h
@@ -25,6 +25,8 @@
 
 int vds_debug_tick_forms(vds_handle *h, uint8_t *out, int32_t cap, int32_t *n_out);
 
+int vds_debug_cluster_forms(vds_handle *h, uint8_t *out, int64_t cap, int32_t *n_out);
+
 int vds_selftest_dpp(vds_handle *h, const int32_t *in, int32_t *out_wave, int32_t *out_rowmin, int32_t *out_rowsum,
                      int32_t *out_rowscan, int32_t nwaves);
 
diff --git a/profiles/r07_cluster_forms/per_slot.py b/profiles/r07_cluster_forms/per_slot.py
--- /dev/null
+++ b/profiles/r07_cluster_forms/per_slot.py
@@ -0,0 +1,41 @@
+import sys
+sys.path.insert(0, ".")
+if sys.argv[1] == "run":
+    import numpy as np, torch
+    from vehicles_dispatch_simulator_amd import workloads
+    wl, arm, out = sys.argv[2], sys.argv[3], sys.argv[4]
+    w = workloads.didi_day("cfg2") if wl == "cfg2" else (workloads.didi_day("cfg4", neighbor=True, service_m=2000.0) if wl == "cfg4" else workloads.stress())
+    R = 128 if wl == "cfg5" else 1024
+    env = w.make_env(R, stream=torch.cuda.current_stream().cuda_stream)
+    env.reset(w.vehicle_nodes(R))
+    for _ in range(6):
+        env.reset_again(); env.run(env.T); env.sync()
+    try:
+        plane = env.cluster_forms()
+    except AttributeError:
+        plane = np.repeat(env.tick_forms()[:, None], env.C, axis=1)
+    np.save("%s/plane_%s_%s.npy" % (out, arm, wl), plane)
+else:
+    import csv, glob
+    import numpy as np
+    def last_day(d, T):
+        f = glob.glob(d + "/**/*kernel_trace.csv", recursive=True)[0]
+        rows = [r for r in csv.DictReader(open(f)) if "k_tick_dense" in r["Kernel_Name"]]
+        rows.sort(key=lambda r: int(r["Start_Timestamp"]))
+        rows = rows[-T:]
+        return [(int(r["End_Timestamp"]) - int(r["Start_Timestamp"])) / 1000 for r in rows], [r["Kernel_Name"] for r in rows]
+    da, db, wl, out = sys.argv[2], sys.argv[3], sys.argv[4], sys.argv[5]
+    pa = np.load("%s/plane_parent_%s.npy" % (out, wl)); pb = np.load("%s/plane_new_%s.npy" % (out, wl))
+    T, C = pb.shape
+    (a, ka), (b, kb) = last_day(da, T), last_day(db, T)
+    print("%s: last day, k_tick_dense %.2f ms (parent) -> %.2f ms (forms per (slot, cluster)); %d slots x %d clusters" % (wl, sum(a) / 1e3, sum(b) / 1e3, T, C))
+    print("parent: %d slots in the 16-lane form; this build: %d (slot, cluster) pairs in the 16-lane form, %d slots with both forms (k_tick_dense_mixed)"
+          % (int(pa[:, 0].sum()), int(pb.sum()), sum("mixed" in k for k in kb)))
+    print("per slot: us parent (form: 8 / 16 lanes) / us this build (16-lane clusters of the slot; M: one launch with both forms)")
+    for t0 in range(0, T, 6):
+        cells = []
+        for t in range(t0, min(t0 + 6, T)):
+            fa = "16" if pa[t, 0] else " 8"
+            fb = ("M" if "mixed" in kb[t] else " ") + "%3d" % int(pb[t].sum())
+            cells.append("%4.0f/%s %4.0f/%s" % (a[t], fa, b[t], fb))
+        print("%3d  " % t0 + "  ".join(cells))
diff --git a/vehicles_dispatch_simulator_amd/_lib.py b/vehicles_dispatch_simulator_amd/_lib.py
--- a/vehicles_dispatch_simulator_amd/_lib.py
+++ b/vehicles_dispatch_simulator_amd/_lib.py
@@ -88,7 +88,7 @@
     "vds_main_kernel": (C.c_char_p, [_VP]),
     "vds_dfs_sequences": (C.c_int, [_VP, _VP, _I32, _I32, _VP, _VP, C.c_int64]),
 }
-TEST_SYMBOLS = {"vds_debug_read_span": (C.c_int, [_VP, _VP, _I32]), "vds_debug_read_err": (C.c_int, [_VP, _VP]), "vds_debug_graph_pool_size": (C.c_int, []), "vds_debug_tick_forms": (C.c_int, [_VP, _VP, _I32, _VP]), "vds_debug_check_guards": (C.c_int, [_VP]), "vds_debug_poke_guard": (C.c_int, [_VP]), "vds_debug_dense": (C.c_int, [_VP, _I32, _I32, _I32, _I32]), "vds_debug_ablate": (C.c_int, [_VP, _I32]), "vds_debug_read_prof": (C.c_int, [_VP, _VP]), "vds_selftest_dpp": (C.c_int, [_VP, _VP, _VP, _VP, _VP, _VP, _I32])}
+TEST_SYMBOLS = {"vds_debug_read_span": (C.c_int, [_VP, _VP, _I32]), "vds_debug_read_err": (C.c_int, [_VP, _VP]), "vds_debug_graph_pool_size": (C.c_int, []), "vds_debug_tick_forms": (C.c_int, [_VP, _VP, _I32, _VP]), "vds_debug_cluster_forms": (C.c_int, [_VP, _VP, C.c_int64, _VP]), "vds_debug_check_guards": (C.c_int, [_VP]), "vds_debug_poke_guard": (C.c_int, [_VP]), "vds_debug_dense": (C.c_int, [_VP, _I32, _I32, _I32, _I32]), "vds_debug_ablate": (C.c_int, [_VP, _I32]), "vds_debug_read_prof": (C.c_int, [_VP, _VP]), "vds_selftest_dpp": (C.c_int, [_VP, _VP, _VP, _VP, _VP, _VP, _I32])}
 
 _lib = None
 
diff --git a/vehicles_dispatch_simulator_amd/csrc/vds_api.hip b/vehicles_dispatch_simulator_amd/csrc/vds_api.hip
--- a/vehicles_dispatch_simulator_amd/csrc/vds_api.hip
+++ b/vehicles_dispatch_simulator_amd/csrc/vds_api.hip
@@ -54,6 +54,8 @@
 void read_prof_dense(unsigned long long *, hipStream_t);
 void read_span_dense(unsigned long long *, int, hipStream_t);
 void emit_tick_dense(const Emit &, const Static &, const State &, int, int, int);
+void emit_tick_dense_mixed(const Emit &, const Static &, const State &, int, const int2 *, int);
+bool dense_mixed_ok(const Static &, int);
 void emit_dense_flush(const Emit &, const Static &, const State &, int, int);
 void emit_pack_obs(const Emit &, const Static &, const State &, int, int, int, int *, int, int);
 void emit_dispatch_dense(const Emit &, const Static &, const State &, int, int, const int *, int, int, int);
@@ -224,11 +226,16 @@
     int *pin_slow = nullptr;
     hipEvent_t pin_ev = nullptr;
     long long pin_bucket_ticks = 0;
-    int *pin_slow_tick = nullptr; int pin_slow_cap = 0;
+    int *pin_slow_tick = nullptr; size_t pin_slow_cap = 0;
     bool pin_ticks_valid = false;
-    int slow_tick_cap = 1;
-    int tick_mode = 1, tick_lim = -1;
+    int slow_tick_cap = 1, slow_tick_C = 1;
+    int tick_mode = 3, tick_lim = -1, cluster_lim = -1, cluster_seed = 0;
     std::vector<unsigned char> tick_form;
+    std::vector<unsigned char> cluster_form;
+    std::vector<int> bmap_off;
+    std::vector<int> bmap_n;
+    std::vector<int2> bmap_host;
+    int2 *d_bmap = nullptr; size_t bmap_cap = 0;
     Static S_alt;
     int dense_adapt = 0;
     unsigned tables_gen = 0;
@@ -345,11 +352,24 @@
 
 #define RUN_GROUPS_MAX 16
 
+static bool slot_mixed(const vds_handle *h, int t) { return t >= 0 && (size_t)t < h->bmap_off.size() && h->bmap_off[t] >= 0; }
 extern "C" int vds_debug_tick_forms(vds_handle *h, uint8_t *out, int32_t cap, int32_t *n_out) {
     if (!h || !out || !n_out || cap < 0) return VDS_EINVAL;
     const int n = (int)std::min<size_t>(h->tick_form.size(), (size_t)cap);
-    for (int i = 0; i < n; ++i) out[i] = h->tick_form[i];
+    for (int i = 0; i < n; ++i) out[i] = (h->tick_form[i] || slot_mixed(h, i)) ? 1 : 0;
     *n_out = n;
+    return VDS_OK;
+}
+extern "C" int vds_debug_cluster_forms(vds_handle *h, uint8_t *out, int64_t cap, int32_t *n_out) {
+    if (!h || !out || !n_out || cap < 0) return VDS_EINVAL;
+    const int C = h->S.C, T = (int)h->tick_form.size();
+    if ((long long)T * C > cap) return VDS_EINVAL;
+    for (int t = 0; t < T; ++t)
+        for (int c = 0; c < C; ++c) {
+            const size_t i = (size_t)t * C + c;
+            out[i] = slot_mixed(h, t) ? h->cluster_form[i] : h->tick_form[t];
+        }
+    *n_out = T;
     return VDS_OK;
 }
 extern "C" int vds_debug_graph_pool_size() {
@@ -838,6 +858,12 @@
     return VDS_OK;
 }
 
+static int slow_tick_slots(const vds_handle *h) {
+    int tcap = std::max(h->S.T, 1);
+    for (const auto &d : h->days) tcap = std::max(tcap, d.T);
+    return tcap;
+}
+
 static int alloc_state(vds_handle *h, int O) {
     Static &S = h->S;
     State &D = h->D;
@@ -855,7 +881,8 @@
     if (ring_cap > 65520) return fail(h, VDS_EINVAL, "ring_cap=%d > 65520 unsupported", ring_cap);
     int far_cap = h->cfg.far_cap > 0 ? round_up(h->cfg.far_cap, 64) : std::min(round_up(std::max(V, 1), 64), 256);
     if (S.dense && H > 32) { S.dense = 0; S.pull = 0; }
-    if (!h->state_allocs.empty() && S.idle_cap >= idle_cap && S.fl_cap == far_cap && S.H == H && S.ring_cap >= ring_cap && h->alloc_dense == S.dense && h->alloc_st == S.dense_st && h->alloc_R == R)
+    if (!h->state_allocs.empty() && S.idle_cap >= idle_cap && S.fl_cap == far_cap && S.H == H && S.ring_cap >= ring_cap && h->alloc_dense == S.dense && h->alloc_st == S.dense_st && h->alloc_R == R &&
+        h->slow_tick_cap >= slow_tick_slots(h) && h->slow_tick_C == C)
         return VDS_OK;
     for (void *p : h->state_allocs) dev_free(p);
     h->state_allocs.clear();
@@ -881,12 +908,12 @@
         h->alloc_sink = keep;
         if (rc) return rc;
     }
-    D.slow_tick = nullptr;
+    D.slow_tick = nullptr; D.slow_T = 0;
     {
-        int tcap = std::max(S.T, 1);
-        for (const auto &d : h->days) tcap = std::max(tcap, d.T);
-        h->slow_tick_cap = tcap;
-        if (S.dense && (rc = dev_alloc(h, &D.slow_tick, (size_t)tcap))) return rc;
+        const int tcap = slow_tick_slots(h);
+        h->slow_tick_cap = tcap; h->slow_tick_C = C;
+        if (S.dense && (rc = dev_alloc(h, &D.slow_tick, (size_t)tcap * C))) return rc;
+        if (S.dense) D.slow_T = tcap;
     }
     D.dry = nullptr;
     if (S.dense_st && (rc = dev_alloc(h, &D.dry, (size_t)R))) return rc;
@@ -1239,8 +1266,14 @@
         S.dense_lpr = (lpr == 8 || lpr == 16) ? lpr : DENSE_LPR_DEFAULT;
         const int tab_max = (S.dense_lpr == 16 && S.blk8s != nullptr && env_int("VDS_DENSE_TAB256", 1) != 0) ? 256 : 128;
         h->dense_adapt = (h->dbg_dense_lpr > 0 || h->dbg_dense_tab > 0 || getenv("VDS_DENSE_LPR") || env_int("VDS_DENSE_ADAPT", 1) == 0) ? -1 : 0;
-        h->pin_bucket_ticks = 0; h->pin_ticks_valid = false; h->tick_form.clear();
-        { const char *v = getenv("VDS_DENSE_TICK_FORMS"); h->tick_mode = !v || !*v ? 1 : (*v == '0' ? 0 : (*v == 'a' ? 2 : 1)); h->tick_lim = env_int("VDS_DENSE_TICK_LIM", -1); }
+        h->pin_bucket_ticks = 0; h->pin_ticks_valid = false; h->tick_form.clear(); h->cluster_form.clear(); h->bmap_off.clear(); h->bmap_n.clear();
+        {
+            const char *v = getenv("VDS_DENSE_TICK_FORMS");
+            h->tick_lim = env_int("VDS_DENSE_TICK_LIM", -1);
+            h->cluster_lim = env_int("VDS_DENSE_CLUSTER_LIM", -1);
+            h->cluster_seed = env_int("VDS_DENSE_CLUSTER_SEED", 0);
+            h->tick_mode = !v || !*v ? (h->tick_lim >= 0 ? 1 : 3) : (*v == '0' ? 0 : (*v == 'a' ? 2 : (*v == 's' ? 1 : 3)));
+        }
         S.dense_tab = h->dbg_dense_tab > 0 ? std::min(h->dbg_dense_tab, tab_max) : tab_max;
         S.dense_keys = h->dbg_dense_keys > 0 ? std::min(h->dbg_dense_keys, 64) : 64;
         S.dense_force_slow = h->dbg_dense_slow & 1;
@@ -1443,11 +1476,66 @@
 #ifndef DENSE_TICK_RATE
 #define DENSE_TICK_RATE 0.00025
 #endif
+#ifndef DENSE_CLUSTER_LIM
+#define DENSE_CLUSTER_LIM 0
+#endif
 static const Static &tick_static(vds_handle *h, int t) {
     if (t < 0 || (size_t)t >= h->tick_form.size() || !h->tick_form[t]) return h->S;
     h->S_alt = h->S;
     h->S_alt.dense_lpr = 16; h->S_alt.dense_tab = 256;
     return h->S_alt;
+}
+static void emit_tick(vds_handle *h, const Emit &e, int t, int r_lo, int r_n) {
+    if (slot_mixed(h, t)) {
+        if (r_lo == 0 && (r_n <= 0 || r_n == h->S.R)) { emit_tick_dense_mixed(e, h->S, h->D, t, h->d_bmap + h->bmap_off[t], h->bmap_n[t]); return; }
+        h->S_alt = h->S;
+        h->S_alt.dense_lpr = 16; h->S_alt.dense_tab = 256;
+        emit_tick_dense(e, h->S_alt, h->D, t, r_lo, r_n);
+        return;
+    }
+    emit_tick_dense(e, tick_static(h, t), h->D, t, r_lo, r_n);
+}
+static size_t set_cluster_forms(vds_handle *h) {
+    const Static &S = h->S;
+    const int T = S.T, C = S.C, R = S.R;
+    if (!h->bmap_host.empty()) (void)hipStreamSynchronize(h->stream);
+    h->tick_form.assign((size_t)T, 0);
+    h->bmap_off.assign((size_t)T, -1); h->bmap_n.assign((size_t)T, 0);
+    h->bmap_host.clear();
+    size_t n16 = 0;
+    for (int t = 0; t < T; ++t) {
+        const unsigned char *f = h->cluster_form.data() + (size_t)t * C;
+        int k = 0;
+        for (int c = 0; c < C; ++c) k += f[c] ? 1 : 0;
+        n16 += (size_t)k;
+        if (k == C) h->tick_form[t] = 1;
+        if (k == 0 || k == C) continue;
+        h->bmap_off[t] = (int)h->bmap_host.size();
+        for (int ci = 0; ci < C; ++ci) {
+            const int form = f[h->corder_host[ci]] ? 1 : 0, rows = form ? 16 : 32;
+            for (int r0 = 0; r0 < R; r0 += rows) h->bmap_host.push_back(make_int2(ci, (r0 << 1) | form));
+        }
+        h->bmap_n[t] = (int)h->bmap_host.size() - h->bmap_off[t];
+    }
+    if (!h->bmap_host.empty()) {
+        bool ok = true;
+        if (h->bmap_cap < h->bmap_host.size()) {
+            (void)hipStreamSynchronize(h->stream);
+            if (h->d_bmap) { h->dev_allocs.erase(std::remove(h->dev_allocs.begin(), h->dev_allocs.end(), (void *)h->d_bmap), h->dev_allocs.end()); dev_free(h->d_bmap); }
+            h->d_bmap = nullptr; h->bmap_cap = 0;
+            std::vector<void *> *sink = h->alloc_sink; h->alloc_sink = nullptr;
+            ok = dev_alloc(h, &h->d_bmap, h->bmap_host.size()) == VDS_OK;
+            h->alloc_sink = sink;
+            if (ok) h->bmap_cap = h->bmap_host.size();
+        }
+        ok = ok && hipMemcpyAsync(h->d_bmap, h->bmap_host.data(), h->bmap_host.size() * sizeof(int2), hipMemcpyHostToDevice, h->stream) == hipSuccess;
+        if (!ok) {
+            (void)hipGetLastError();
+            for (int t = 0; t < T; ++t) if (h->bmap_off[t] >= 0) { h->tick_form[t] = 1; h->bmap_off[t] = -1; }
+        }
+    }
+    h->run_stale = true; h->tables_gen++;
+    return n16;
 }
 static void adapt_dense(vds_handle *h) {
     Static &S = h->S;
@@ -1460,6 +1548,19 @@
         }
         return;
     }
+    if (h->cluster_seed != 0 && S.dense_lpr == 8 && dense_mixed_ok(S, S.R) && (int)h->corder_host.size() == S.C) {
+        if (h->cluster_form.empty()) {
+            h->cluster_form.assign((size_t)S.T * S.C, 0);
+            unsigned long long x = 0x9E3779B97F4A7C15ull * (unsigned long long)(unsigned)h->cluster_seed + 1;
+            for (int t = 0; t < S.T; ++t)
+                for (int c = 0; c < S.C; ++c) {
+                    x ^= x << 13; x ^= x >> 7; x ^= x << 17;
+                    h->cluster_form[(size_t)t * S.C + c] = (unsigned char)(S.C > 1 ? (c == t % S.C ? 1 : (c == (t + 1) % S.C ? 0 : (x >> 32) & 1)) : 0);
+                }
+            set_cluster_forms(h);
+        }
+        return;
+    }
     if (h->dense_adapt != 0) return;
     if (!h->pin_slow) {
         if (hipHostMalloc((void **)&h->pin_slow, sizeof(int)) != hipSuccess || hipEventCreateWithFlags(&h->pin_ev, hipEventDisableTiming) != hipSuccess) {
@@ -1468,11 +1569,25 @@
         *h->pin_slow = 0;
     }
     if (h->pin_bucket_ticks > 0 && hipEventQuery(h->pin_ev) == hipSuccess) {
-        if (h->tick_mode == 1 && h->pin_ticks_valid && S.dense_lpr == 8) {
+        if (h->tick_mode == 3 && h->pin_ticks_valid && S.dense_lpr == 8 && dense_mixed_ok(S, S.R) && (int)h->corder_host.size() == S.C) {
+            const int lim = h->cluster_lim >= 0 ? h->cluster_lim : DENSE_CLUSTER_LIM;
+            h->cluster_form.assign((size_t)S.T * S.C, 0);
+            size_t n16 = 0;
+            for (size_t i = 0; i < h->cluster_form.size(); ++i) if (h->pin_slow_tick[i] > lim) { h->cluster_form[i] = 1; ++n16; }
+            h->dense_adapt = 1;
+            if (n16 > 0) set_cluster_forms(h);
+            else h->cluster_form.clear();
+            return;
+        }
+        if ((h->tick_mode == 1 || h->tick_mode == 3) && h->pin_ticks_valid && S.dense_lpr == 8) {
             const double lim = h->tick_lim >= 0 ? (double)h->tick_lim : DENSE_TICK_RATE * (double)S.R * (double)S.C;
             size_t n16 = 0;
             h->tick_form.assign((size_t)S.T, 0);
-            for (int t = 0; t < S.T; ++t) if ((double)h->pin_slow_tick[t] > lim) { h->tick_form[t] = 1; ++n16; }
+            for (int t = 0; t < S.T; ++t) {
+                long long sum = 0;
+                for (int c = 0; c < S.C; ++c) sum += h->pin_slow_tick[(size_t)t * S.C + c];
+                if ((double)sum > lim) { h->tick_form[t] = 1; ++n16; }
+            }
             h->dense_adapt = 1;
             if (n16 * 100 >= (size_t)S.T * 85) { std::fill(h->tick_form.begin(), h->tick_form.end(), (unsigned char)1); n16 = (size_t)S.T; }
             if (n16 > 0) { h->run_stale = true; h->tables_gen++; }
@@ -1491,13 +1606,14 @@
     if (h->have_reset && h->t > 0) {
         h->pin_ticks_valid = false;
         bool ok = hipMemcpyAsync(h->pin_slow, h->D.err + 2, sizeof(int), hipMemcpyDeviceToHost, h->stream) == hipSuccess;
-        if (ok && h->tick_mode == 1 && h->D.slow_tick && h->t == S.T && S.T > 0) {
-            if (h->pin_slow_cap < S.T) {
+        if (ok && (h->tick_mode == 1 || h->tick_mode == 3) && h->D.slow_tick && h->t == S.T && S.T > 0 && S.T <= h->slow_tick_cap && S.C == h->slow_tick_C) {
+            const size_t words = (size_t)S.T * S.C;
+            if (h->pin_slow_cap < words) {
                 if (h->pin_slow_tick) { (void)hipStreamSynchronize(h->stream); (void)hipHostFree(h->pin_slow_tick); h->pin_slow_tick = nullptr; h->pin_slow_cap = 0; }
-                if (hipHostMalloc((void **)&h->pin_slow_tick, (size_t)S.T * sizeof(int)) == hipSuccess) h->pin_slow_cap = S.T;
+                if (hipHostMalloc((void **)&h->pin_slow_tick, words * sizeof(int)) == hipSuccess) h->pin_slow_cap = words;
                 else { (void)hipGetLastError(); h->pin_slow_tick = nullptr; }
             }
-            if (h->pin_slow_tick && hipMemcpyAsync(h->pin_slow_tick, h->D.slow_tick, (size_t)S.T * sizeof(int), hipMemcpyDeviceToHost, h->stream) == hipSuccess)
+            if (h->pin_slow_tick && hipMemcpyAsync(h->pin_slow_tick, h->D.slow_tick, words * sizeof(int), hipMemcpyDeviceToHost, h->stream) == hipSuccess)
                 h->pin_ticks_valid = true;
         }
         if (ok && hipEventRecord(h->pin_ev, h->stream) == hipSuccess)
@@ -1511,7 +1627,7 @@
     const Static &S = h->S;
     HIPCHK(h, hipMemsetAsync(h->D.err, 0, 16 * sizeof(int), h->stream));
     HIPCHK(h, hipMemsetAsync(h->D.work, 0, 2 * sizeof(int), h->stream));
-    if (h->D.slow_tick) HIPCHK(h, hipMemsetAsync(h->D.slow_tick, 0, (size_t)h->slow_tick_cap * sizeof(int), h->stream));
+    if (h->D.slow_tick) HIPCHK(h, hipMemsetAsync(h->D.slow_tick, 0, (size_t)h->slow_tick_cap * h->slow_tick_C * sizeof(int), h->stream));
     HIPCHK(h, hipMemsetAsync(h->D.ring_cnt, 0, (size_t)S.H * S.C * S.R * sizeof(int), h->stream));
     if (h->D.sup) {
         HIPCHK(h, hipMemsetAsync(h->D.sup, 0, (size_t)VDS_SUP_PLANES * S.C * S.R * sizeof(int), h->stream));
@@ -1727,7 +1843,7 @@
         if (h->S.dense) {
             const int rcs = dev_copy_sync(h);
             if (rcs) return rcs;
-            Emit e; e.st = h->stream; emit_tick_dense(e, tick_static(h, h->t), h->D, h->t, 0, 0);
+            Emit e; e.st = h->stream; emit_tick(h, e, h->t, 0, 0);
         }
         else launch_tick_main(h->S, h->D, h->t, h->lds_ints, h->stream);
         if (h->profiling) HIPCHK(h, hipEventRecord(b, h->stream));
@@ -1743,7 +1859,7 @@
             const int rcs = dev_copy_sync(h);
             if (rcs) return rcs;
             Emit e; e.st = h->stream;
-            emit_tick_dense(e, tick_static(h, h->t), h->D, h->t, 0, 0);
+            emit_tick(h, e, h->t, 0, 0);
             emit_hybrid_walk(e, h->S, h->D, h->t, 0, 0);
             if (flush) emit_dense_flush(e, h->S, h->D, 0, 0);
         }
@@ -1827,13 +1943,13 @@
             Emit e;
             e.graph = g; e.deps = prev ? &prev : nullptr; e.ndeps = prev ? 1 : 0; e.node = &node; e.err = &err;
             if (!h->dfs_mode) {
-                if (h->S.dense) emit_tick_dense(e, tick_static(h, t), h->D, t, r_lo, r_n);
+                if (h->S.dense) emit_tick(h, e, t, r_lo, r_n);
                 else emit_tick_rows(e, h->S, h->D, t, h->lds_ints, r_lo, r_n);
                 if (err != hipSuccess) break;
                 prev = node;
                 continue;
             }
-            if (h->S.dense_st) emit_tick_dense(e, tick_static(h, t), h->D, t, r_lo, r_n);
+            if (h->S.dense_st) emit_tick(h, e, t, r_lo, r_n);
             else emit_hybrid_rows(e, h->S, h->D, t, h->lds_ints, r_lo, r_n);
             if (err != hipSuccess) break;
             prev = node;
@@ -1974,10 +2090,10 @@
                 Emit e;
                 e.graph = g; e.deps = chain ? &chain : nullptr; e.ndeps = chain ? 1 : 0; e.node = &n1; e.err = &err;
                 if (!h->dfs_mode) {
-                    if (h->S.dense) emit_tick_dense(e, tick_static(h, t), h->D, t, r_lo, r_n);
+                    if (h->S.dense) emit_tick(h, e, t, r_lo, r_n);
                     else emit_tick_rows(e, h->S, h->D, t, h->lds_ints, r_lo, r_n);
                 } else {
-                    if (h->S.dense_st) emit_tick_dense(e, tick_static(h, t), h->D, t, r_lo, r_n);
+                    if (h->S.dense_st) emit_tick(h, e, t, r_lo, r_n);
                     else emit_hybrid_rows(e, h->S, h->D, t, h->lds_ints, r_lo, r_n);
                     if (err != hipSuccess) break;
                     e.deps = &n1; e.ndeps = 1; e.node = &n2;
diff --git a/vehicles_dispatch_simulator_amd/csrc/vds_device.h b/vehicles_dispatch_simulator_amd/csrc/vds_device.h
--- a/vehicles_dispatch_simulator_amd/csrc/vds_device.h
+++ b/vehicles_dispatch_simulator_amd/csrc/vds_device.h
@@ -139,6 +139,7 @@
     unsigned *arr;
     unsigned short *stamp;
     int *slow_tick;
+    int slow_T;
     int *dry;
     int *sup;
     int *sup_slot;
diff --git a/vehicles_dispatch_simulator_amd/csrc/vds_tick_dense.hip b/vehicles_dispatch_simulator_amd/csrc/vds_tick_dense.hip
--- a/vehicles_dispatch_simulator_amd/csrc/vds_tick_dense.hip
+++ b/vehicles_dispatch_simulator_amd/csrc/vds_tick_dense.hip
@@ -48,6 +48,8 @@
     unsigned *arr; const int *so_slot; const int2 *d_rec; const int *d_first; const int4 *replica_desc2; int pull_W;
     const int4 *tdesc;
     unsigned short *stamp; int *dry; int *slow_tick; const int *so_rank;
+    int slow_T;
+    const int2 *bmap;
     int *sup, *sup_slot;
     const Static *Sdev; const State *Ddev;
 };
@@ -955,8 +957,8 @@
 
 #define DN_CAND 128
 
-template <bool U8, int DM, int LPR, bool PULL, int TABMAX = DN_TAB, int ROWS = DN_ROWS, bool ST = false>
-__global__ __launch_bounds__(ROWS * LPR, TABMAX > 128 ? DN_MIN_WAVES256 : (LPR == 16 ? DN_MIN_WAVES16 : (LPR == 8 ? DN_MIN_WAVES8 : DN_MIN_WAVES4))) void k_tick_dense(DenseArgs P, int t) {
+template <bool U8, int DM, int LPR, bool PULL, int TABMAX, int ROWS, bool ST>
+__device__ __forceinline__ void tick_dense_wg(const DenseArgs &P, int t, int ci, int row0, int tabl) {
     static_assert(TABMAX == 128 || (TABMAX == 256 && LPR == 16 && U8), "256-entry tables: 16 lanes per replica, byte costs");
     static_assert(!ST || (U8 && DM == 0 && PULL), "stamp form: byte costs, one shared day, static arrival slots");
     static_assert(ROWS == DN_ROWS || (ROWS == 32 && DM == 0 && LPR == 8) || ((ROWS == 8 || ROWS == 4) && DM == 1 && LPR == 16),
@@ -979,14 +981,12 @@
     int2 *lds_drec = reinterpret_cast<int2 *>(lds_rank + (ST ? DN_ORDERS : 0));
     unsigned *tab_all = reinterpret_cast<unsigned *>(lds_drec + (PULL ? DN_CAND : 0));
     CT *lds_blk = reinterpret_cast<CT *>(tab_all + ROWS * (TABMAX + DN_TPAD));
-    const int nchunks = gridDim.x / S.C;
     int4 cd, td0 = make_int4(0, 0, 0, 0);
     if (DM == 0) {
-        const int4 *tp = S.tdesc + 2 * ((size_t)t * S.C + blockIdx.x / nchunks);
+        const int4 *tp = S.tdesc + 2 * ((size_t)t * S.C + ci);
         td0 = tp[0]; cd = tp[1];
-    } else cd = S.cdesc_dense[blockIdx.x / nchunks];
+    } else cd = S.cdesc_dense[ci];
     const int c = cd.z, nc = cd.x;
-    const int row0 = S.r_lo + (int)(blockIdx.x % nchunks) * ROWS;
     const int wave = __builtin_amdgcn_readfirstlane((int)(threadIdx.x >> 6));
     const int lane = lane_id();
     const int g = lane / LPR, lg = lane & (LPR - 1);
@@ -1141,11 +1141,11 @@
     __syncthreads();
     PROF_STAMP_NW(1);
     const int mnew0 = ST ? max(m + A, m_raw) : m + A;
-    const bool bad = rowvalid && (!wg_ok || far != 0 || Aring > S.dense_keys || Aring > S.ring_cap || A > DN_TAB || mnew0 > min(S.dense_tab, TABMAX) || mnew0 > S.idle_cap || S.dense_force_slow ||
+    const bool bad = rowvalid && (!wg_ok || far != 0 || Aring > S.dense_keys || Aring > S.ring_cap || A > DN_TAB || mnew0 > min(tabl, TABMAX) || mnew0 > S.idle_cap || S.dense_force_slow ||
                                   (PULL && (A - Aring > S.dense_keys * 2 || A > DN_TH)));
 #ifdef VDS_PROF
     if (bad && lg == 0) {
-        const int why = k > DN_ORDERS ? 4 : (n > DN_CAND ? 5 : (far != 0 ? 6 : ((Aring > S.dense_keys || Aring > S.ring_cap) ? 7 : (A > DN_TAB ? 8 : ((mnew0 > min(S.dense_tab, TABMAX) || mnew0 > S.idle_cap) ? 9 :
+        const int why = k > DN_ORDERS ? 4 : (n > DN_CAND ? 5 : (far != 0 ? 6 : ((Aring > S.dense_keys || Aring > S.ring_cap) ? 7 : (A > DN_TAB ? 8 : ((mnew0 > min(tabl, TABMAX) || mnew0 > S.idle_cap) ? 9 :
                         ((PULL && A - Aring > S.dense_keys * 2) ? 10 : 11))))));
         atomicAdd(&D.err[why], 1);
     }
@@ -1153,7 +1153,7 @@
     const unsigned long long badrows = ballot(bad && lg == 0);
     if (badrows != 0ull && lane == 0) {
         atomicAdd(&D.err[2], popc64(badrows));
-        if (D.slow_tick != nullptr) atomicAdd(&D.slow_tick[t], popc64(badrows));
+        if (D.slow_tick != nullptr && t < D.slow_T) atomicAdd(&D.slow_tick[(size_t)t * S.C + c], popc64(badrows));
     }
     if (bad) { rowvalid = false; m = 0; A = 0; Aring = 0; }
     if (!rowvalid) m_raw = 0;
@@ -1175,6 +1175,22 @@
         const int l0 = __ffsll((long long)rest) - 1;
         dense_bucket_slow<CT, ST>(*P.Sdev, *P.Ddev, c, rdlane(r, l0), t, reinterpret_cast<const CT *>(blk_g), nc, (DM == 2 || k > 0) ? lds_blk : (const CT *)nullptr);
     }
+}
+
+template <bool U8, int DM, int LPR, bool PULL, int TABMAX = DN_TAB, int ROWS = DN_ROWS, bool ST = false>
+__global__ __launch_bounds__(ROWS * LPR, TABMAX > 128 ? DN_MIN_WAVES256 : (LPR == 16 ? DN_MIN_WAVES16 : (LPR == 8 ? DN_MIN_WAVES8 : DN_MIN_WAVES4))) void k_tick_dense(DenseArgs P, int t) {
+    const int nchunks = gridDim.x / P.C;
+    tick_dense_wg<U8, DM, LPR, PULL, TABMAX, ROWS, ST>(P, t, (int)(blockIdx.x / nchunks), P.r_lo + (int)(blockIdx.x % nchunks) * ROWS, P.dense_tab);
+}
+
+#ifndef DN_MIN_WAVES_MIX
+#define DN_MIN_WAVES_MIX DN_MIN_WAVES8
+#endif
+template <bool ST>
+__global__ __launch_bounds__(256, DN_MIN_WAVES_MIX) void k_tick_dense_mixed(DenseArgs P, int t) {
+    const int2 e = P.bmap[blockIdx.x];
+    if (e.y & 1) tick_dense_wg<true, 0, 16, true, 256, DN_ROWS, ST>(P, t, e.x, P.r_lo + (e.y >> 1), 256);
+    else tick_dense_wg<true, 0, 8, true, DN_TAB, 32, ST>(P, t, e.x, P.r_lo + (e.y >> 1), P.dense_tab);
 }
 
 __global__ __launch_bounds__(256) void k_dense_flush(int *hdr, unsigned *idle_all, unsigned short *stamp_all, int R, int C, int idle_cap, int r_lo, int r_n) {
@@ -1255,7 +1271,7 @@
     else emit_dense(e, dm == 2 ? k_tick_dense<false, 2, LPR, PULL> : (dm ? k_tick_dense<false, 1, LPR, PULL> : k_tick_dense<false, 0, LPR, PULL>), grid, block, lds, P, t);
 }
 
-void emit_tick_dense(const Emit &e, const Static &S, const State &D, int t, int r_lo, int r_n) {
+static DenseArgs dense_args(const Static &S, const State &D, int r_lo, int r_n) {
     DenseArgs P;
     P.hdr = D.hdr; P.cnt = D.cnt; P.idle = reinterpret_cast<unsigned *>(D.idle); P.ring = reinterpret_cast<uint2 *>(D.ring);
     P.ring_cnt = D.ring_cnt; P.inbox = D.inbox; P.out = D.out; P.err = D.err;
@@ -1268,6 +1284,30 @@
     P.tdesc = S.tdesc;
     P.stamp = D.stamp; P.dry = D.dry; P.slow_tick = D.slow_tick; P.so_rank = S.so_rank; P.sup = D.sup; P.sup_slot = D.sup_slot;
     P.arr = D.arr; P.so_slot = S.so_slot; P.d_rec = S.d_rec; P.d_first = S.d_first; P.replica_desc2 = S.replica_desc2; P.pull_W = S.pull_W;
+    P.slow_T = D.slow_T; P.bmap = nullptr;
+    return P;
+}
+
+static size_t dense_lds(const Static &S, int rows, int tab) {
+    const int bb = (S.max_nc * (S.max_nc + 1) * (S.blk8s ? 1 : 4) + 15) / 16 * 16;
+    return (S.n_days > 1 && !S.chunk_days ? DN_ROWS * DN_ORDERS * 2 : DN_ORDERS * 16) + (S.pull ? DN_ORDERS * 8 + DN_CAND * 8 : 0) + (S.dense_st ? DN_ORDERS * 4 : 0) +
+           (size_t)rows * (tab + DN_TPAD) * 4 + bb;
+}
+
+bool dense_mixed_ok(const Static &S, int slots) {
+    return S.dense && S.n_days <= 1 && S.blk8s != nullptr && S.pull && S.tdesc != nullptr && slots >= 64 && DN_ROWS32;
+}
+
+void emit_tick_dense_mixed(const Emit &e, const Static &S, const State &D, int t, const int2 *bmap, int nblk) {
+    DenseArgs P = dense_args(S, D, 0, 0);
+    P.bmap = bmap;
+    const size_t lds = std::max(dense_lds(S, 32, DN_TAB), dense_lds(S, DN_ROWS, 256));
+    if (S.dense_st) emit_dense(e, k_tick_dense_mixed<true>, dim3(nblk), dim3(256), lds, P, t);
+    else emit_dense(e, k_tick_dense_mixed<false>, dim3(nblk), dim3(256), lds, P, t);
+}
+
+void emit_tick_dense(const Emit &e, const Static &S, const State &D, int t, int r_lo, int r_n) {
+    const DenseArgs P = dense_args(S, D, r_lo, r_n);
     const int slots = r_n > 0 ? r_n : (S.rperm != nullptr ? S.rslots : S.R) - r_lo;
     const bool t256 = dense_tab256(S);
     const bool rows32 = S.n_days <= 1 && S.dense_lpr == 8 && !t256 && S.blk8s != nullptr && S.pull && slots >= 64 && DN_ROWS32;
@@ -1275,9 +1315,7 @@
     const int rows = rows32 ? 32 : (rows8 ? S.row_gran : DN_ROWS);
     const int rchunks = (slots + rows - 1) / rows;
     const dim3 grid(S.C * rchunks);
-    const int bb = (S.max_nc * (S.max_nc + 1) * (S.blk8s ? 1 : 4) + 15) / 16 * 16;
-    const size_t lds = (S.n_days > 1 && !S.chunk_days ? DN_ROWS * DN_ORDERS * 2 : DN_ORDERS * 16) + (S.pull ? DN_ORDERS * 8 + DN_CAND * 8 : 0) + (S.dense_st ? DN_ORDERS * 4 : 0) +
-                       rows * ((t256 ? 256 : DN_TAB) + DN_TPAD) * 4 + bb;
+    const size_t lds = dense_lds(S, rows, t256 ? 256 : DN_TAB);
     if (S.dense_st) {
         if (t256) emit_dense(e, k_tick_dense<true, 0, 16, true, 256, DN_ROWS, true>, grid, dim3(DN_ROWS * 16), lds, P, t);
         else if (rows32) emit_dense(e, k_tick_dense<true, 0, 8, true, DN_TAB, 32, true>, grid, dim3(32 * 8), lds, P, t);
diff --git a/vehicles_dispatch_simulator_amd/env.py b/vehicles_dispatch_simulator_amd/env.py
--- a/vehicles_dispatch_simulator_amd/env.py
+++ b/vehicles_dispatch_simulator_amd/env.py
@@ -219,6 +219,12 @@
         self._chk(self._lib.vds_debug_tick_forms(self._h, _p(out), int(out.size), C.byref(n)))
         return out[:n.value].copy()
 
+    def cluster_forms(self) -> np.ndarray:
+        out = np.zeros((max(self.T, 1), self.C), dtype=np.uint8)
+        n = C.c_int32()
+        self._chk(self._lib.vds_debug_cluster_forms(self._h, _p(out), C.c_int64(out.size), C.byref(n)))
+        return out[:n.value].copy()
+
     def run_groups(self) -> int:
         return int(self._lib.vds_get_run_groups(self._h))
 
```

New measurement: 23.82 million (median of 6 runs). 1.07x the previous value.
